# quitedob/yolo-sod

Measured on AMD Instinct MI355X. Metric: images/sec @640×640 bs=32, 1→8 MI355X; mAP@0.5:0.95 parity vs CPU ref, higher is better.
Workload: dtype f32

## Files before the change

include/yolosod_hip.h:

```cpp
#ifndef YOLOSOD_HIP_H
#define YOLOSOD_HIP_H
#include <stddef.h>
#include <stdint.h>

#ifdef __cplusplus
extern "C" {
#endif

int yolosod_abi_version(void);
const char* yolosod_last_error(void);
int yolosod_init(int device);

size_t yolosod_se_workspace(int B, int C, int H, int W);
int yolosod_se_forward(const float* x, float* y, int B, int C, int H, int W, const float* fc1_w, const float* fc1_b,
                       const float* fc2_w, const float* fc2_b, int hidden, void* workspace, size_t workspace_bytes,
                       void* stream);

size_t yolosod_cbam_workspace(int B, int C, int H, int W);
int yolosod_cbam_forward(const float* x, float* y, int B, int C, int H, int W, const float* fc0_w,
                         const float* fc2_w, int hidden, const float* sa_w, void* workspace, size_t workspace_bytes,
                         void* stream);

size_t yolosod_ca_workspace(int B, int C, int H, int W);
int yolosod_ca_forward(const float* x, float* y, int B, int C, int H, int W, const float* conv1_w,
// ... 29 lines not shown
                         size_t workspace_bytes, void* stream);
size_t yolosod_swin_prep_bytes(int C, int num_heads, int mlp_hidden);
size_t yolosod_swin_prepared_workspace(int B, int C, int H, int W, int num_heads, int window, int mlp_hidden);
int yolosod_swin_prepare(int C, int num_heads, int mlp_hidden, const float* ln1_w, const float* ln1_b,
                         const float* in_proj_w, const float* in_proj_b, const float* out_proj_w, const float* ln2_w,
                         const float* ln2_b, const float* mlp1_w, const float* mlp1_b, const float* mlp2_w,
                         const float* pw_w, const float* bn_w, const float* bn_b, const float* bn_mean,
                         const float* bn_var, float bn_eps, void* prep, size_t prep_bytes, void* stream);
int yolosod_swin_forward_prepared(const float* x, float* y, int B, int C, int H, int W, int num_heads, int window,
                                  const float* dw_w, float ln1_eps, const float* out_proj_b, float ln2_eps,
                                  int mlp_hidden, const float* mlp2_b, const void* prep, size_t prep_bytes,
                                  void* workspace, size_t workspace_bytes, void* stream);

int yolosod_plane_parts(long HW, long* seg);
int yolosod_bias_act_stats(const float* y, long y_bstride, float* out, long out_bstride, const float* bias,
                           const float* res, long res_bstride, int B, int C, long HW, int act, int parts, long seg,
                           float* psum, float* pmax, void* stream);
int yolosod_se_forward_pre(const float* x, float* y, int B, int C, int H, int W, const float* fc1_w,
                           const float* fc1_b, const float* fc2_w, const float* fc2_b, int hidden, const float* psum,
                           void* workspace, size_t workspace_bytes, void* stream);
int yolosod_cbam_forward_pre(const float* x, float* y, int B, int C, int H, int W, const float* fc0_w,
                             const float* fc2_w, int hidden, const float* sa_w, const float* psum, const float* pmax,
                             void* workspace, size_t workspace_bytes, void* stream);
int yolosod_bias_act_capool(const float* y, long y_bstride, float* out, long out_bstride, const float* bias,
                            const float* res, long res_bstride, int B, int C, int H, int W, int act, float* yin,
                            void* stream);
int yolosod_upsample2x(const void* x, void* out, long out_bstride, int B, int C, int h, int w, int elem_bytes,
                       void* stream);
size_t yolosod_stem_workspace(int B, int Cout, int H, int W);
int yolosod_stem_conv(const float* x, const float* w, const float* bias, float* out, int B, int Cout, int H, int W,
                      int parts, long seg, float* psum, void* workspace, size_t workspace_bytes, void* stream);
int yolosod_ca_forward_pre(const float* x, float* y, int B, int C, int H, int W, const float* conv1_w,
                           const float* conv1_b, int mip, const float* bn_w, const float* bn_b, const float* bn_mean,
                           const float* bn_var, float bn_eps, const float* convh_w, const float* convh_b,
                           const float* convw_w, const float* convw_b, const float* yin, void* workspace,
                           size_t workspace_bytes, void* stream);

size_t yolosod_mamba_glu_workspace(int B, int C, int H, int W, int ch, int reduction);
int yolosod_mamba_glu_forward(const float* x, float* y, int B, int C, int H, int W, int ch, int reduction,
                              const float* in_w, const float* in_bn_w, const float* in_bn_b, const float* in_bn_mean,
                              const float* in_bn_var, float in_bn_eps, const float* pw1_w, const float* dw_w,
                              const float* bn_w, const float* bn_b, const float* bn_mean, const float* bn_var,
                              float bn_eps, const float* pw2_w, const float* out_w, const float* out_bn_w,
                              const float* out_bn_b, const float* out_bn_mean, const float* out_bn_var,
                              float out_bn_eps, void* workspace, size_t workspace_bytes, void* stream);

int yolosod_detect_decode(int nl, const float* const* maps, const int* heights, const int* widths,
                          const float* strides, int B, int nc, int reg_max, float* y, void* stream);

int yolosod_detect_head(int nl, const float* const* box_feat, const float* const* cls_feat, int c2, int c3,
                        const float* const* box_w, const float* const* box_b, const float* const* cls_w,
                        const float* const* cls_b, const int* heights, const int* widths, const float* strides, int B,
                        int nc, int reg_max, float* y, void* stream);

size_t yolosod_nms_workspace(int B, int nc, int A, int multi_label);
size_t yolosod_nms_workspace_v2(int B, int nc, int A, int multi_label, int max_det);
int yolosod_nms(float* pred, int B, int nc, int A, float conf_thres, double iou_thres, const int* classes,
                int n_classes, int agnostic, int multi_label, int max_det, int max_nms, float max_wh, int in_place,
                float* out, int* counts, int* out_index, void* workspace, size_t workspace_bytes, void* stream);
int yolosod_nms_merged(float* pred, int B, int nc, int A, float conf_thres, double iou_thres, const int* classes,
                       int n_classes, int agnostic, int multi_label, int max_det, int max_nms, float max_wh,
                       int in_place, float* out, int* counts, int* out_index, int* n_merged, void* workspace,
                       size_t workspace_bytes, void* stream);

int yolosod_letterbox_ingest(const int64_t* desc, int B, void* out, long out_bstride, int out_h, int out_w,
                             int out_bf16, int pad_value, void* stream);
int yolosod_scale_boxes(float* det, const int* counts, int B, int D, const float* geom, void* stream);
int yolosod_tile_merge(const float* y, int n, int nc, int A, const int32_t* desc, int rows, float* merged, int F,
                       int S, float cut_margin, void* stream);
int yolosod_tta_views(const void* x, int B, int C, int H, int W, int bf16, const int64_t* desc, int V, int max_ph,
                      int max_pw, void* stream);
int yolosod_tta_merge(const float* y, int B, int nc, int A, int src_lo, int n, float* cat, int A_tot, int dst,
                      float scale, int flip, float img_w, float img_h, void* stream);
int yolosod_tile_merge_tta(const float* y, int n, int nc, int A, int src_lo, int n_k, const int32_t* desc, int rows,
                           float* merged, int F, int S, int A_tot, int dst, float scale, int flip, float img_w,
                           float img_h, float cut_margin, void* stream);
int yolosod_match_predictions(const float* det, const int* counts, int B, int D, const float* labels,
                              const int* label_off, const float* iouv, int T, uint8_t* tp, void* stream);

int yolosod_bias_act(const float* y, long y_bstride, float* out, long out_bstride, const float* bias,
                     const float* res, long res_bstride, int B, int C, long HW, int act, void* stream);

int yolosod_bias_act_dual(const float* y, long y_bstride, float* out, long out_bstride, const float* bias,
                          const float* res, long res_bstride, float* out2, long out2_bstride, int c2lo, int B, int C,
                          long HW, int act, void* stream);

size_t yolosod_conv3x3_prep_bytes(int cin);
int yolosod_conv3x3_prepare(const float* w, int cin, void* prep, size_t prep_bytes, void* stream);
int yolosod_conv3x3_silu(const float* x, float* y, int B, int cin, int H, int W, const float* bias, const void* prep,
                         size_t prep_bytes, void* stream);
size_t yolosod_conv3x3_prep_bytes_ex(int cin, int cout);
int yolosod_conv3x3_prepare_ex(const float* w, int cin, int cout, void* prep, size_t prep_bytes, void* stream);
int yolosod_conv3x3_silu_ex(const float* x, float* y, long y_bstride, const float* res, long res_bstride, int B,
                            int cin, int cout, int H, int W, const float* bias, const void* prep, size_t prep_bytes,
                            void* stream);
int yolosod_conv3x3_silu_xs(const float* x, long x_bstride, float* y, long y_bstride, const float* res, long res_bstride,
                            int B, int cin, int cout, int H, int W, const float* bias, const void* prep,
                            size_t prep_bytes, void* stream);
int yolosod_bottleneck3x3_silu_xs(const float* x, long x_bstride, float* y, long y_bstride, const float* res,
                                  long res_bstride, int B, int H, int W, const float* bias1, const void* prep1,
                                  size_t prep1_bytes, const float* bias2, const void* prep2, size_t prep2_bytes,
                                  void* stream);

int yolosod_conv3x3_head_xs(const float* x, long x_bstride, int B, int H, int W, const float* bias, const void* prep,
                            size_t prep_bytes, const void* head_prep, const float* head_bias, int mode, int nc,
                            float stride, float* y, int A, int a_off, void* stream);
size_t yolosod_detect_head_prep_bytes(int rows);
int yolosod_detect_head_prepare(const float* w, int rows, void* prep, size_t prep_bytes, void* stream);

int yolosod_conv1x1_thin(const float* x, long x_bs, const float* w, const float* bias, float* out, long out_bs,
                         const float* res, long res_bs, float* out2, long out2_bs, int c2lo, int B, int Cin, int Cout,
                         long HW, void* stream);

int yolosod_sppf_pool(float* z, long z_bstride, int B, int C, int H, int W, void* stream);

int yolosod_conv1x1_thin_cat(const float* x, long x_bs, const float* x2, long x2_bs, int k1, const float* w,
                             const float* bias, float* out, long out_bs, float* out2, long out2_bs, int c2lo, int B,
                             int Cin, int Cout, long HW, int up_w, void* stream);

int yolosod_conv1x1_thin_stats(const float* x, long x_bs, const float* w, const float* bias, float* out, long out_bs,
                               int B, int Cin, int Cout, long HW, int parts, float* psum, float* pmax, float* tile_ws,
                               void* stream);

int yolosod_conv1x1(const float* x, long x_bs, const float* w, const float* bias, float* out, long out_bs,
                    const float* res, long res_bs, int B, int Cin, int Cout, long HW, int act, void* stream);

int yolosod_gemm_f32(const float* A, long a_bs, int lda, const float* B, long b_bs, int ldb, int b_kcontig, float* C,
                     long c_bs, int ldc, int M, int N, int K, int batch, const float* bias, int bias_mode, int act,
                     const float* res, void* stream);
int yolosod_layernorm(const float* x, float* y, long rows, int C, const float* w, const float* b, float eps,
                      void* stream);
int yolosod_attention(const float* qkv, float* out, long n_seq, int L, int C, int heads, void* stream);

void yolosod_debug_set_swin_fused(int on);
int yolosod_debug_set_swin_x3(int on);
int yolosod_debug_set_a2_pool_px(int px);
int yolosod_debug_set_head_x2(int on);
int yolosod_debug_set_a2_x2(int on);
int yolosod_debug_set_a2_fused(int on);
int yolosod_debug_set_a2_pool_wide(int on);
int yolosod_se_gate(const float* x, int B, int C, int H, int W, const float* fc1_w, const float* fc1_b,
                    const float* fc2_w, const float* fc2_b, int hidden, const float* psum, float* gate, void* workspace,
                    size_t workspace_bytes, void* stream);
int yolosod_cbam_gates(const float* x, int B, int C, int H, int W, const float* fc0_w, const float* fc2_w, int hidden,
                       const float* sa_w, const float* psum, const float* pmax, float* ca, float* sa, void* workspace,
                       size_t workspace_bytes, void* stream);
size_t yolosod_conv3x3s2_prep_bytes(int cin, int cout);
int yolosod_conv3x3s2_prepare(const float* w, int cin, int cout, void* prep, size_t prep_bytes, void* stream);
int yolosod_conv3x3s2_silu(const float* x, float* y, int B, int cin, int cout, int H, int W, const float* bias,
                           const float* gc, const float* gp, const void* prep, size_t prep_bytes, void* stream);
int yolosod_conv3x3s2_silu_out(const float* x, float* y, long y_bstride, int B, int cin, int cout, int H, int W,
                               const float* bias, const float* gc, const float* gp, const void* prep,
                               size_t prep_bytes, void* stream);
size_t yolosod_conv1x1x2_prep_bytes(int cin, int cout);
int yolosod_conv1x1x2_prepare(const float* w, int cin, int cout, void* prep, size_t prep_bytes, void* stream);
int yolosod_conv1x1x2_silu(const float* x, long x_bstride, float* y, long y_bstride, float* y2, long y2_bstride,
                           int c2lo, int B, int cin, int cout, int HW, const float* bias, const void* prep,
                           size_t prep_bytes, void* stream);
int yolosod_conv1x1x2_silu_cat(const float* x, long x_bstride, const float* x2, long x2_bstride, int k1, float* y,
                               long y_bstride, float* y2, long y2_bstride, int c2lo, int B, int cin, int cout, int HW,
                               const float* bias, const void* prep, size_t prep_bytes, int up_w, void* stream);
int yolosod_conv1x1x2_silu_stats(const float* x, long x_bstride, float* y, long y_bstride, int B, int cin, int cout,
                                 int HW, const float* bias, const void* prep, size_t prep_bytes, int stats, int parts,
                                 float* psum, float* pmax, float* tile_ws, void* stream);
int yolosod_debug_set_conv1x1x2_form(int form);
int yolosod_debug_conv1x1x2_form(int B, int cout, int H, int W);
int yolosod_debug_set_conv3x3s2_form(int form);
int yolosod_debug_conv3x3s2_form(int B, int cout, int H, int W);
int yolosod_debug_set_conv3x3_form(int form);
int yolosod_debug_conv3x3_form(int B, int cout, int H, int W);
int yolosod_debug_conv3x3_form_ex(int B, int cin, int cout, int H, int W);
int yolosod_debug_bottleneck3x3_fused(int B, int H, int W);
int yolosod_debug_set_bottleneck3x3_fuse(int mode);
int yolosod_debug_conv3x3_head_fused(int B, int H, int W);
int yolosod_debug_set_conv3x3_head_fuse(int mode);
void yolosod_debug_set_gemm_x2(int on);
int yolosod_debug_set_swin_tokln(int on);
int yolosod_debug_split_f16(const float* v, uint32_t* h, uint32_t* l, long npair, void* stream);
int yolosod_split_range_flag(int reset, void* stream);

#include <stdint.h>

int yolosod_se_forward_bf16(const uint16_t* x, uint16_t* y, int B, int C, int H, int W, const float* fc1_w,
                            const float* fc1_b, const float* fc2_w, const float* fc2_b, int hidden, const float* psum,
                            void* workspace, size_t workspace_bytes, void* stream);
int yolosod_cbam_forward_bf16(const uint16_t* x, uint16_t* y, int B, int C, int H, int W, const float* fc0_w,
                              const float* fc2_w, int hidden, const float* sa_w, const float* psum, const float* pmax,
                              void* workspace, size_t workspace_bytes, void* stream);
int yolosod_ca_forward_bf16(const uint16_t* x, uint16_t* y, int B, int C, int H, int W, const float* conv1_w,
                            const float* conv1_b, int mip, const float* bn_w, const float* bn_b, const float* bn_mean,
                            const float* bn_var, float bn_eps, const float* convh_w, const float* convh_b,
                            const float* convw_w, const float* convw_b, const float* yin, void* workspace,
                            size_t workspace_bytes, void* stream);
size_t yolosod_swin_workspace_bf16(int B, int C, int H, int W, int num_heads, int window, int mlp_hidden);
int yolosod_swin_forward_bf16(const uint16_t* x, uint16_t* y, int B, int C, int H, int W, int num_heads, int window,
                              const float* dw_w, const float* ln1_w, const float* ln1_b, float ln1_eps,
                              const uint16_t* in_proj_w, const float* in_proj_b, const uint16_t* out_proj_w,
                              const float* out_proj_b, const float* ln2_w, const float* ln2_b, float ln2_eps,
                              const uint16_t* mlp1_w, const float* mlp1_b, int mlp_hidden, const uint16_t* mlp2_w,
                              const float* mlp2_b, const uint16_t* pw_w, const float* bn_w, const float* bn_b,
                              const float* bn_mean, const float* bn_var, float bn_eps, void* workspace,
                              size_t workspace_bytes, void* stream);
size_t yolosod_a2_workspace_bf16(int B, int C, int H, int W, int num_areas);
int yolosod_a2_forward_bf16(const uint16_t* x, uint16_t* y, int B, int C, int H, int W, int num_areas, int num_heads,
                            const uint16_t* proj_w, const float* proj_b, const float* ln_w, const float* ln_b,
                            float ln_eps, const uint16_t* in_proj_w, const float* in_proj_b, const uint16_t* oproj_w,
                            const float* oproj_b, void* workspace, size_t workspace_bytes, void* stream);
int yolosod_detect_head_levels(int nl, int l0, int l1, const void* const* box_feat, const void* const* cls_feat, int c2,
                               int c3, const float* const* box_w, const float* const* box_b, const float* const* cls_w,
                               const float* const* cls_b, const int* heights, const int* widths, const float* strides,
                               int B, int nc, int reg_max, float* y, int bf16, void* stream);
int yolosod_detect_head_bf16(int nl, const uint16_t* const* box_feat, const uint16_t* const* cls_feat, int c2, int c3,
                             const float* const* box_w, const float* const* box_b, const float* const* cls_w,
                             const float* const* cls_b, const int* heights, const int* widths, const float* strides,
                             int B, int nc, int reg_max, float* y, void* stream);
int yolosod_bias_act_bf16(const uint16_t* y, long y_bstride, uint16_t* out, long out_bstride, const float* bias,
                          const uint16_t* res, long res_bstride, uint16_t* out2, long out2_bstride, int c2lo, int B,
                          int C, long HW, int act, void* stream);
int yolosod_bias_act_stats_bf16(const uint16_t* y, long y_bstride, uint16_t* out, long out_bstride, const float* bias,
                                const uint16_t* res, long res_bstride, int B, int C, long HW, int act, int parts,
                                long seg, float* psum, float* pmax, void* stream);
int yolosod_bias_act_capool_bf16(const uint16_t* y, long y_bstride, uint16_t* out, long out_bstride,
                                 const float* bias, const uint16_t* res, long res_bstride, int B, int C, int H, int W,
                                 int act, float* yin, void* stream);
int yolosod_gemm_bf16(const uint16_t* A, long a_bs, int lda, const uint16_t* B, long b_bs, int ldb, int b_kcontig,
                      uint16_t* C, long c_bs, int ldc, int M, int N, int K, int batch, const float* bias,
                      int bias_mode, int act, const uint16_t* res, void* stream);
int yolosod_attention_bf16(const uint16_t* qkv, uint16_t* out, long n_seq, int L, int C, int heads, void* stream);

#ifdef __cplusplus
}
#endif
#endif
```

yolo-sod_amd/_hip.py:

```python
from __future__ import annotations

import ctypes
import os
from pathlib import Path

import torch

from .utils.metrics import IOU_THRESHOLDS

LIB_PATH = Path(__file__).resolve().parent / "lib" / "libyolosod_hip.so"

_c_float_p = ctypes.c_void_p
_vp = ctypes.c_void_p
_i = ctypes.c_int
_l = ctypes.c_long
_f = ctypes.c_float
_d = ctypes.c_double
_sz = ctypes.c_size_t

SIGNATURES = {
    "yolosod_abi_version": (_i, []),
    "yolosod_last_error": (ctypes.c_char_p, []),
    "yolosod_se_workspace": (_sz, [_i, _i, _i, _i]),
    "yolosod_se_forward": (_i, [_vp, _vp, _i, _i, _i, _i, _vp, _vp, _vp, _vp, _i, _vp, _sz, _vp]),
    "yolosod_cbam_workspace": (_sz, [_i, _i, _i, _i]),
    "yolosod_cbam_forward": (_i, [_vp, _vp, _i, _i, _i, _i, _vp, _vp, _i, _vp, _vp, _sz, _vp]),
    "yolosod_ca_workspace": (_sz, [_i, _i, _i, _i]),
    "yolosod_ca_forward": (_i, [_vp, _vp, _i, _i, _i, _i, _vp, _vp, _i, _vp, _vp, _vp, _vp, _f, _vp, _vp, _vp,
                                _vp, _vp, _sz, _vp]),
    "yolosod_a2_workspace": (_sz, [_i, _i, _i, _i, _i]),
    "yolosod_a2_forward": (_i, [_vp, _vp, _i, _i, _i, _i, _i, _i, _vp, _vp, _vp, _vp, _f, _vp, _vp, _vp, _vp, _vp,
                                _vp, _vp, _sz, _vp]),
    "yolosod_swin_workspace": (_sz, [_i, _i, _i, _i, _i, _i]),
    "yolosod_swin_workspace_v2": (_sz, [_i, _i, _i, _i, _i, _i, _i]),
    "yolosod_swin_forward": (_i, [_vp, _vp, _i, _i, _i, _i, _i, _i, _vp, _vp, _vp, _f, _vp, _vp, _vp, _vp, _vp, _vp,
                                  _f, _vp, _vp, _i, _vp, _vp, _vp, _vp, _vp, _vp, _vp, _f, _vp, _sz, _vp]),
    "yolosod_detect_decode": (_i, [_i, _vp, _vp, _vp, _vp, _i, _i, _i, _vp, _vp]),
    "yolosod_detect_head": (_i, [_i, _vp, _vp, _i, _i, _vp, _vp, _vp, _vp, _vp, _vp, _vp, _i, _i, _i, _vp, _vp]),
    "yolosod_nms_workspace": (_sz, [_i, _i, _i, _i]),
    "yolosod_nms_workspace_v2": (_sz, [_i, _i, _i, _i, _i]),
    "yolosod_nms": (_i, [_vp, _i, _i, _i, _f, _d, _vp, _i, _i, _i, _i, _i, _f, _i, _vp, _vp, _vp, _vp, _sz, _vp]),
    "yolosod_nms_merged": (_i, [_vp, _i, _i, _i, _f, _d, _vp, _i, _i, _i, _i, _i, _f, _i, _vp, _vp, _vp, _vp, _vp, _sz,
                                _vp]),
    "yolosod_gemm_f32": (_i, [_vp, _l, _i, _vp, _l, _i, _i, _vp, _l, _i, _i, _i, _i, _i, _vp, _i, _i, _vp, _vp]),
    "yolosod_layernorm": (_i, [_vp, _vp, _l, _i, _vp, _vp, _f, _vp]),
    "yolosod_attention": (_i, [_vp, _vp, _l, _i, _i, _i, _vp]),
    "yolosod_bias_act": (_i, [_vp, _l, _vp, _l, _vp, _vp, _l, _i, _i, _l, _i, _vp]),
    "yolosod_upsample2x": (_i, [_vp, _vp, _l, _i, _i, _i, _i, _i, _vp]),
    "yolosod_letterbox_ingest": (_i, [_vp, _i, _vp, _l, _i, _i, _i, _i, _vp]),
    "yolosod_scale_boxes": (_i, [_vp, _vp, _i, _i, _vp, _vp]),
    "yolosod_tile_merge": (_i, [_vp, _i, _i, _i, _vp, _i, _vp, _i, _i, _f, _vp]),
    "yolosod_tile_merge_tta": (_i, [_vp, _i, _i, _i, _i, _i, _vp, _i, _vp, _i, _i, _i, _i, _f, _i, _f, _f, _f, _vp]),
    "yolosod_match_predictions": (_i, [_vp, _vp, _i, _i, _vp, _vp, _vp, _i, _vp, _vp]),
    "yolosod_tta_views": (_i, [_vp, _i, _i, _i, _i, _i, _vp, _i, _i, _i, _vp]),
    "yolosod_tta_merge": (_i, [_vp, _i, _i, _i, _i, _i, _vp, _i, _i, _f, _i, _f, _f, _vp]),
    "yolosod_stem_workspace": (_sz, [_i, _i, _i, _i]),
    "yolosod_stem_conv": (_i, [_vp, _vp, _vp, _vp, _i, _i, _i, _i, _i, _l, _vp, _vp, _sz, _vp]),
    "yolosod_conv1x1_thin_stats": (_i, [_vp, _l, _vp, _vp, _vp, _l, _i, _i, _i, _l, _i, _vp, _vp, _vp, _vp]),
    "yolosod_conv1x1_thin": (_i, [_vp, _l, _vp, _vp, _vp, _l, _vp, _l, _vp, _l, _i, _i, _i, _i, _l, _vp]),
    "yolosod_bias_act_dual": (_i, [_vp, _l, _vp, _l, _vp, _vp, _l, _vp, _l, _i, _i, _i, _l, _i, _vp]),
    "yolosod_bias_act_capool": (_i, [_vp, ctypes.c_long, _vp, ctypes.c_long, _vp, _vp, ctypes.c_long, _i, _i, _i, _i,
                                     _i, _vp, _vp]),
    "yolosod_ca_forward_pre": (_i, [_vp, _vp, _i, _i, _i, _i, _vp, _vp, _i, _vp, _vp, _vp, _vp, _f, _vp, _vp, _vp, _vp,
                                    _vp, _vp, ctypes.c_size_t, _vp]),
    "yolosod_bias_act_stats": (_i, [_vp, _l, _vp, _l, _vp, _vp, _l, _i, _i, _l, _i, _i, _l, _vp, _vp, _vp]),
    "yolosod_plane_parts": (_i, [_l, ctypes.POINTER(ctypes.c_long)]),
    "yolosod_se_forward_pre": (_i, [_vp, _vp, _i, _i, _i, _i, _vp, _vp, _vp, _vp, _i, _vp, _vp, _sz, _vp]),
    "yolosod_cbam_forward_pre": (_i, [_vp, _vp, _i, _i, _i, _i, _vp, _vp, _i, _vp, _vp, _vp, _vp, _sz, _vp]),
    "yolosod_conv1x1": (_i, [_vp, _l, _vp, _vp, _vp, _l, _vp, _l, _i, _i, _i, _l, _i, _vp]),
    "yolosod_conv3x3_prep_bytes": (_sz, [_i]),
    "yolosod_conv3x3_prepare": (_i, [_vp, _i, _vp, _sz, _vp]),
    "yolosod_conv3x3_silu": (_i, [_vp, _vp, _i, _i, _i, _i, _vp, _vp, _sz, _vp]),
    "yolosod_conv1x1x2_prep_bytes": (_sz, [_i, _i]),
    "yolosod_conv1x1x2_prepare": (_i, [_vp, _i, _i, _vp, _sz, _vp]),
    "yolosod_conv1x1x2_silu": (_i, [_vp, _l, _vp, _l, _vp, _l, _i, _i, _i, _i, _i, _vp, _vp, _sz, _vp]),
    "yolosod_conv1x1x2_silu_cat": (_i, [_vp, _l, _vp, _l, _i, _vp, _l, _vp, _l, _i, _i, _i, _i, _i, _vp, _vp, _sz,
                                        _i, _vp]),
    "yolosod_conv1x1x2_silu_stats": (_i, [_vp, _l, _vp, _l, _i, _i, _i, _i, _vp, _vp, _sz, _i, _i, _vp, _vp, _vp, _vp]),
    "yolosod_sppf_pool": (_i, [_vp, _l, _i, _i, _i, _i, _vp]),
    "yolosod_conv1x1_thin_cat": (_i, [_vp, _l, _vp, _l, _i, _vp, _vp, _vp, _l, _vp, _l, _i, _i, _i, _i, _l, _i, _vp]),
    "yolosod_conv3x3_prep_bytes_ex": (_sz, [_i, _i]),
    "yolosod_conv3x3_prepare_ex": (_i, [_vp, _i, _i, _vp, _sz, _vp]),
    "yolosod_conv3x3_silu_ex": (_i, [_vp, _vp, _l, _vp, _l, _i, _i, _i, _i, _i, _vp, _vp, _sz, _vp]),
    "yolosod_conv3x3_silu_xs": (_i, [_vp, _l, _vp, _l, _vp, _l, _i, _i, _i, _i, _i, _vp, _vp, _sz, _vp]),
    "yolosod_debug_set_swin_fused": (None, [_i]),
    "yolosod_debug_set_swin_x3": (_i, [_i]),
    "yolosod_debug_set_head_x2": (_i, [_i]),
    "yolosod_debug_set_a2_x2": (_i, [_i]),
    "yolosod_debug_set_gemm_x2": (None, [_i]),
    "yolosod_debug_split_f16": (_i, [_vp, _vp, _vp, _l, _vp]),
    "yolosod_swin_prep_bytes": (_sz, [_i, _i, _i]),
    "yolosod_split_range_flag": (_i, [_i, _vp]),
    "yolosod_swin_prepare": (_i, [_i, _i, _i] + [_vp] * 15 + [_f, _vp, _sz, _vp]),
    "yolosod_swin_forward_prepared": (_i, [_vp, _vp, _i, _i, _i, _i, _i, _i, _vp, _f, _vp, _f, _i, _vp, _vp, _sz,
                                           _vp, _sz, _vp]),
    "yolosod_swin_prepared_workspace": (_sz, [_i, _i, _i, _i, _i, _i, _i]),
    "yolosod_a2_prep_bytes": (_sz, [_i, _i, _i, _i]),
    "yolosod_a2_prepare": (_i, [_i, _vp, _vp, _vp, _vp, _vp, _vp, _sz, _vp]),
    "yolosod_a2_forward_prepared": (_i, [_vp, _vp, _i, _i, _i, _i, _i, _i, _vp, _vp, _vp, _vp, _f, _vp, _vp, _vp,
                                         _vp, _vp, _sz, _vp, _sz, _vp]),
    "yolosod_init": (_i, [_i]),
    "yolosod_debug_set_a2_fused": (_i, [_i]),
    "yolosod_debug_set_a2_pool_wide": (_i, [_i]),
    "yolosod_debug_set_conv3x3_form": (_i, [_i]),
    "yolosod_debug_conv3x3_form": (_i, [_i, _i, _i, _i]),
    "yolosod_debug_conv3x3_form_ex": (_i, [_i, _i, _i, _i, _i]),
    "yolosod_bottleneck3x3_silu_xs": (_i, [_vp, _l, _vp, _l, _vp, _l, _i, _i, _i, _vp, _vp, _sz, _vp, _vp, _sz, _vp]),
    "yolosod_conv3x3_head_xs": (_i, [_vp, _l, _i, _i, _i, _vp, _vp, _sz, _vp, _vp, _i, _i, _f, _vp, _i, _i, _vp]),
    "yolosod_detect_head_prep_bytes": (_sz, [_i]),
    "yolosod_detect_head_prepare": (_i, [_vp, _i, _vp, _sz, _vp]),
    "yolosod_debug_conv3x3_head_fused": (_i, [_i, _i, _i]),
    "yolosod_debug_set_conv3x3_head_fuse": (_i, [_i]),
    "yolosod_debug_bottleneck3x3_fused": (_i, [_i, _i, _i]),
    "yolosod_debug_set_bottleneck3x3_fuse": (_i, [_i]),
    "yolosod_debug_set_conv1x1x2_form": (_i, [_i]),
    "yolosod_debug_conv1x1x2_form": (_i, [_i, _i, _i, _i]),
    "yolosod_debug_set_conv3x3s2_form": (_i, [_i]),
    "yolosod_debug_conv3x3s2_form": (_i, [_i, _i, _i, _i]),
    "yolosod_se_gate": (_i, [_vp, _i, _i, _i, _i, _vp, _vp, _vp, _vp, _i, _vp, _vp, _vp, _sz, _vp]),
    "yolosod_cbam_gates": (_i, [_vp, _i, _i, _i, _i, _vp, _vp, _i, _vp, _vp, _vp, _vp, _vp, _vp, _sz, _vp]),
    "yolosod_conv3x3s2_prep_bytes": (_sz, [_i, _i]),
    "yolosod_conv3x3s2_prepare": (_i, [_vp, _i, _i, _vp, _sz, _vp]),
    "yolosod_conv3x3s2_silu": (_i, [_vp, _vp, _i, _i, _i, _i, _i, _vp, _vp, _vp, _vp, _sz, _vp]),
    "yolosod_conv3x3s2_silu_out": (_i, [_vp, _vp, _l, _i, _i, _i, _i, _i, _vp, _vp, _vp, _vp, _sz, _vp]),
    "yolosod_debug_set_swin_tokln": (_i, [_i]),
    "yolosod_debug_set_a2_pool_px": (_i, [_i]),
    "yolosod_mamba_glu_workspace": (_sz, [_i, _i, _i, _i, _i, _i]),
    "yolosod_mamba_glu_forward": (_i, [_vp, _vp, _i, _i, _i, _i, _i, _i, _vp, _vp, _vp, _vp, _vp, _f, _vp, _vp,
                                       _vp, _vp, _vp, _vp, _f, _vp, _vp, _vp, _vp, _vp, _vp, _f, _vp, _sz, _vp]),
    "yolosod_se_forward_bf16": (_i, [_vp, _vp, _i, _i, _i, _i, _vp, _vp, _vp, _vp, _i, _vp, _vp, _sz, _vp]),
    "yolosod_cbam_forward_bf16": (_i, [_vp, _vp, _i, _i, _i, _i, _vp, _vp, _i, _vp, _vp, _vp, _vp, _sz, _vp]),
    "yolosod_ca_forward_bf16": (_i, [_vp, _vp, _i, _i, _i, _i, _vp, _vp, _i, _vp, _vp, _vp, _vp, _f, _vp, _vp, _vp,
                                     _vp, _vp, _vp, _sz, _vp]),
    "yolosod_bias_act_bf16": (_i, [_vp, _l, _vp, _l, _vp, _vp, _l, _vp, _l, _i, _i, _i, _l, _i, _vp]),
    "yolosod_bias_act_stats_bf16": (_i, [_vp, _l, _vp, _l, _vp, _vp, _l, _i, _i, _l, _i, _i, _l, _vp, _vp, _vp]),
    "yolosod_bias_act_capool_bf16": (_i, [_vp, _l, _vp, _l, _vp, _vp, _l, _i, _i, _i, _i, _i, _vp, _vp]),
    "yolosod_swin_workspace_bf16": (_sz, [_i, _i, _i, _i, _i, _i, _i]),
    "yolosod_swin_forward_bf16": (_i, [_vp, _vp, _i, _i, _i, _i, _i, _i, _vp, _vp, _vp, _f, _vp, _vp, _vp, _vp, _vp,
                                       _vp, _f, _vp, _vp, _i, _vp, _vp, _vp, _vp, _vp, _vp, _vp, _f, _vp, _sz, _vp]),
    "yolosod_a2_workspace_bf16": (_sz, [_i, _i, _i, _i, _i]),
    "yolosod_a2_forward_bf16": (_i, [_vp, _vp, _i, _i, _i, _i, _i, _i, _vp, _vp, _vp, _vp, _f, _vp, _vp, _vp, _vp,
                                     _vp, _sz, _vp]),
    "yolosod_detect_head_bf16": (_i, [_i, _vp, _vp, _i, _i, _vp, _vp, _vp, _vp, _vp, _vp, _vp, _i, _i, _i, _vp,
                                      _vp]),
    "yolosod_detect_head_levels": (_i, [_i, _i, _i, _vp, _vp, _i, _i, _vp, _vp, _vp, _vp, _vp, _vp, _vp, _i, _i,
                                        _i, _vp, _i, _vp]),
    "yolosod_gemm_bf16": (_i, [_vp, _l, _i, _vp, _l, _i, _i, _vp, _l, _i, _i, _i, _i, _i, _vp, _i, _i, _vp, _vp]),
    "yolosod_attention_bf16": (_i, [_vp, _vp, _l, _i, _i, _i, _vp]),
}

_LIB = None


def load_library() -> ctypes.CDLL:
    global _LIB
    if _LIB is None:
        if not LIB_PATH.exists():
            raise RuntimeError(
                f"yolosod_amd: HIP library {LIB_PATH} is missing - run __graft_entry__.build() "
                "(or python yolo-sod_amd/build.py). There is no CPU fallback.")
        path = os.environ.get("YOLOSOD_LIB_AB") or str(LIB_PATH)
        lib = ctypes.CDLL(path)
        for name, (res, args) in SIGNATURES.items():
            if path != str(LIB_PATH) and name.startswith("yolosod_debug_") and not hasattr(lib, name):
                continue
            fn = getattr(lib, name)
            fn.restype = res
            fn.argtypes = args
        _LIB = lib
    return _LIB


OPS_LIB_PATH = LIB_PATH.parent / "yolosod_torch_ops.so"
_OPS = None


def ops():
    global _OPS
    if _OPS is None:
        load_library()
        if not OPS_LIB_PATH.exists():
            raise RuntimeError(f"yolosod_amd: torch-op library {OPS_LIB_PATH} is missing - run "
                               "__graft_entry__.build() (or python yolo-sod_amd/build.py). There is no CPU fallback.")
        if not hasattr(torch.ops.yolosod, "se_fwd"):
            torch.ops.load_library(str(OPS_LIB_PATH))
        _OPS = torch.ops.yolosod
    return _OPS


class _OpTimer:

    def __init__(self, select=None):
        self.records = []
        self.select = select

    def durations_ms(self):
        torch.cuda.synchronize()
        out = []
        for key, e0, e1 in self.records:
            out.append((key, e0.elapsed_time(e1)))
        return out


_TIMER: _OpTimer | None = None


class op_timer:

    def __init__(self, select=None):
        self.select = select

    def __enter__(self):
        global _TIMER
        self.t = _OpTimer(self.select)
        _TIMER = self.t
        return self.t

    def __exit__(self, *exc):
        global _TIMER
        _TIMER = None
        return False


_INIT_DEVS = set()


def _init_device(dev) -> None:
    idx = torch.device(dev).index
    idx = torch.cuda.current_device() if idx is None else idx
    if idx not in _INIT_DEVS:
        _check(load_library().yolosod_init(int(idx)), "init")
        _INIT_DEVS.add(idx)


def _launch(key, dev, fn, *args):
    _init_device(dev)
    with torch.cuda.device(dev):
        t = _TIMER
        if t is None or (t.select is not None and not t.select(key)):
            return fn(*args)
        e0 = torch.cuda.Event(enable_timing=True)
        e1 = torch.cuda.Event(enable_timing=True)
        e0.record()
        rc = fn(*args)
        e1.record()
        t.records.append((key, e0, e1))
        return rc


def _check(rc: int, what: str) -> None:
    if rc != 0:
        msg = load_library().yolosod_last_error().decode(errors="replace")
        raise RuntimeError(f"yolosod_amd.{what} failed (rc={rc}): {msg}")


def _dev(t: torch.Tensor, name: str, dtype=torch.float32) -> int:
    if not isinstance(t, torch.Tensor):
        raise TypeError(f"{name}: expected a tensor")
    if t.device.type != "cuda":
        raise RuntimeError(f"{name}: HIP kernel requires a GPU tensor (got device {t.device}); no CPU fallback")
    if t.dtype != dtype:
        raise RuntimeError(f"{name}: expected {dtype}, got {t.dtype}")
    if not t.is_contiguous():
        raise RuntimeError(f"{name}: expected a contiguous tensor")
    return t.data_ptr()


def _p(t: torch.Tensor, name: str, numel: int | None = None, dtype=torch.float32) -> int:
    if numel is not None and t.numel() != numel:
        raise RuntimeError(f"{name}: expected {numel} elements, got {t.numel()}")
    return _dev(t, name, dtype)


_BF16 = torch.bfloat16


def _act_dtype(x: torch.Tensor) -> bool:
# ... 637 lines not shown
def bottleneck3x3_fused(B, H, W) -> bool:
    return bool(load_library().yolosod_debug_bottleneck3x3_fused(int(B), int(H), int(W)))


def bottleneck3x3_silu(x, bias1, prep1, bias2, prep2, out=None, res=None, op="bottleneck3x3"):
    lib = load_library()
    B, C, H, W = x.shape
    if C != 32:
        raise RuntimeError(f"bottleneck3x3: {C} channels (32 only)")
    if out is None:
        y = torch.empty((B, 32, H, W), dtype=torch.float32, device=x.device)
    else:
        _img_view(out, (B, 32, H, W), "bottleneck3x3: out")
        y = out
    if res is not None:
        _img_view(res, (B, 32, H, W), "bottleneck3x3: res")
    b1 = bias1.detach().float().contiguous()
    b2 = bias2.detach().float().contiguous()

    def run():
        blk1, blk2 = prep1(), prep2()
        _img_view(x, (B, 32, H, W), "bottleneck3x3: x")
        return lib.yolosod_bottleneck3x3_silu_xs(x.data_ptr(), x.stride(0), y.data_ptr(), y.stride(0),
                                                 None if res is None else res.data_ptr(),
                                                 0 if res is None else res.stride(0), B, H, W, _dev(b1, "bias1"),
                                                 blk1.data_ptr(), blk1.numel(), _dev(b2, "bias2"), blk2.data_ptr(),
                                                 blk2.numel(), _stream(x.device))

    _check(_launch((op, tuple(x.shape), 32 if res is None else (32, "res")), x.device, run), "bottleneck3x3")
    return y


class CatView:

    def __init__(self, parts, up0=False):
        a, b = parts
        sp = (2 * a.shape[2], 2 * a.shape[3]) if up0 else tuple(a.shape[2:])
        if a.shape[0] != b.shape[0] or sp != tuple(b.shape[2:]) or a.dtype != b.dtype or a.device != b.device:
            raise ValueError("CatView: parts must agree in batch, spatial size, dtype and device")
        self.parts = (a, b)
        self.up0 = bool(up0)
        self.shape = torch.Size((a.shape[0], a.shape[1] + b.shape[1], b.shape[2], b.shape[3]))
        self.device, self.dtype = a.device, a.dtype

    def dim(self):
        return 4

    def materialize(self):
        a, b = self.parts
        if self.up0:
            a = torch.nn.functional.interpolate(a, scale_factor=2, mode="nearest")
        return torch.cat((a, b), 1)


def sppf_pool(z, c):
    B, C4, H, W = z.shape
    if (C4 != 4 * c or z.dtype != torch.float32 or z.device.type != "cuda"
            or z.stride()[1:] != (H * W, W, 1)):
        raise RuntimeError("sppf_pool: z must be a [B, 4c, H, W] fp32 GPU tensor with contiguous images")
    lib = load_library()
    _check(_launch(("sppf_pool", (B, c, H, W), None), z.device, lib.yolosod_sppf_pool, z.data_ptr(), z.stride(0), B,
                   int(c), H, W, _stream(z.device)), "sppf_pool")
    return z


def _imgs_contig(t) -> bool:
    B, C, H, W = t.shape
    return t.stride()[1:] == (H * W, W, 1) and t.stride(0) % 4 == 0 and t.data_ptr() % 16 == 0


def conv1x1x2_ok(x, conv) -> bool:
    if isinstance(x, CatView):
        if not (all(_imgs_contig(t) for t in x.parts) and x.parts[0].shape[1] % 128 == 0):
            return False
    elif not (x.dim() == 4 and _imgs_contig(x)):
        return False
    return (x.device.type == "cuda" and x.dtype == torch.float32
            and conv.kernel_size == (1, 1) and conv.stride == (1, 1) and conv.padding == (0, 0) and conv.groups == 1
            and x.shape[1] == conv.in_channels and (x.shape[2] * x.shape[3]) % 4 == 0
            and int(load_library().yolosod_conv1x1x2_prep_bytes(int(conv.in_channels), int(conv.out_channels))) > 0)


def conv1x1x2_prepare(w):
    lib = load_library()
    return _split_prepare("conv1x1x2", lib.yolosod_conv1x1x2_prep_bytes, lib.yolosod_conv1x1x2_prepare,
                          w.reshape(int(w.shape[0]), int(w.shape[1])))


def conv1x1x2_silu(x, bias, prep, cout, out=None, out2=None, c2lo=0, op="conv1x1x2", stats=None):
    lib = load_library()
    B, Cin, H, W = x.shape
    if stats is not None and (stats not in ("sum", "summax", "capool") or out2 is not None or isinstance(x, CatView)):
        raise RuntimeError(f"conv1x1x2: stats={stats!r} takes one input tensor, no out2")
    if out is None:
        y = torch.empty((B, cout, H, W), dtype=torch.float32, device=x.device)
    else:
        _img_view(out, (B, cout, H, W), "conv1x1x2: out")
        y = out
    if out2 is not None:
        _img_view(out2, (B, cout - c2lo, H, W), "conv1x1x2: out2")
    b = bias.detach().float().contiguous()
    if stats in ("sum", "summax"):
        HW = H * W
        parts, _ = plane_parts(HW)
        psum = torch.empty(B * cout * parts, dtype=torch.float32, device=x.device)
        pmax = torch.empty_like(psum) if stats == "summax" else None
        tws = torch.empty(2 * B * cout * ((HW + 63) // 64), dtype=torch.float32, device=x.device)

        def run_stats():
            blk = prep()
            return lib.yolosod_conv1x1x2_silu_stats(x.data_ptr(), x.stride(0), y.data_ptr(), y.stride(0), B, Cin, cout,
                                                    HW, _dev(b, "bias"), blk.data_ptr(), blk.numel(),
                                                    2 if stats == "summax" else 1, parts, psum.data_ptr(),
                                                    None if pmax is None else pmax.data_ptr(), tws.data_ptr(),
                                                    _stream(x.device))

        _check(_launch(("conv1x1x2_stats", tuple(x.shape), (cout, stats)), x.device, run_stats), "conv1x1x2_stats")
        y._ys_plane_stats = PlaneStats(psum, pmax, parts, y.shape)
        return y

    x0, x1 = x.parts if isinstance(x, CatView) else (x, None)

    def run():
        blk = prep()
        return lib.yolosod_conv1x1x2_silu_cat(x0.data_ptr(), x0.stride(0), None if x1 is None else x1.data_ptr(),
                                              0 if x1 is None else x1.stride(0), int(x0.shape[1]), y.data_ptr(),
                                              y.stride(0), None if out2 is None else out2.data_ptr(),
                                              0 if out2 is None else out2.stride(0), int(c2lo), B, Cin, cout, H * W,
                                              _dev(b, "bias"), blk.data_ptr(), blk.numel(),
                                              W if x1 is not None and x.up0 else 0, _stream(x.device))

    extra = (cout, out2 is not None) + (("cat",) if x1 is not None else ())
    if stats == "capool":
        op, extra = "conv1x1x2_stats", (cout, stats)
    _check(_launch((op, tuple(x.shape), extra), x.device, run), "conv1x1x2")
    return y


def conv3x3s2_ok(x, conv) -> bool:
    return (x.device.type == "cuda" and x.dtype == torch.float32 and x.is_contiguous() and x.dim() == 4
            and conv.kernel_size == (3, 3) and conv.stride == (2, 2) and conv.padding == (1, 1)
            and conv.dilation == (1, 1) and conv.groups == 1
            and (conv.out_channels == 64 or (conv.out_channels % 128 == 0 and conv.out_channels <= 512))
            and conv.in_channels % 32 == 0 and x.shape[1] == conv.in_channels and ((x.shape[3] + 1) // 2) % 4 == 0
            and x.numel() * 4 < 2 ** 32
            and int(load_library().yolosod_conv3x3s2_prep_bytes(int(conv.in_channels), int(conv.out_channels))) > 0)


def conv3x3s2_prepare(w):
    lib = load_library()
    return _split_prepare("conv3x3s2", lib.yolosod_conv3x3s2_prep_bytes, lib.yolosod_conv3x3s2_prepare, w)


def conv3x3s2_silu(x, bias, prep, cout, gate_c=None, gate_p=None, key=None, out=None):
    lib = load_library()
    B, Cin, H, W = x.shape
    Ho, Wo = (H + 1) // 2, (W + 1) // 2
    if out is None:
        y = torch.empty((B, cout, Ho, Wo), dtype=torch.float32, device=x.device)
    else:
        y = out
        if (tuple(y.shape) != (B, cout, Ho, Wo) or y.dtype != torch.float32 or y.device != x.device
                or y.stride()[1:] != (Ho * Wo, Wo, 1) or y.data_ptr() % 16 or y.stride(0) % 4):
            raise RuntimeError(f"conv3x3s2: out {tuple(y.shape)} / {y.stride()} is not a [{B}, {cout}, {Ho}, {Wo}] "
                               "fp32 view with contiguous 16-byte aligned images")
    b = bias.detach().float().contiguous()
    gc = None if gate_c is None else gate_c.float().contiguous()
    gp = None if gate_p is None else gate_p.float().contiguous()
    if gc is not None and (tuple(gc.shape) != (B, Cin) or gc.data_ptr() % 16):
        raise RuntimeError(f"conv3x3s2: channel gate {tuple(gc.shape)} (16-byte aligned [{B}, {Cin}] expected)")
    if gp is not None and gp.numel() != B * H * W:
        raise RuntimeError(f"conv3x3s2: spatial gate of {gp.numel()} values ({B * H * W} expected)")

    def run():
        blk = prep()
        return lib.yolosod_conv3x3s2_silu_out(_dev(x, "x"), y.data_ptr(), y.stride(0), B, Cin, cout, H, W,
                                              _dev(b, "bias"), None if gc is None else _dev(gc, "gate_c"),
                                              None if gp is None else _dev(gp, "gate_p"), blk.data_ptr(), blk.numel(),
                                              _stream(x.device))

    if key is None:
        key = ("conv3x3s2", tuple(x.shape), (cout, gc is not None, gp is not None))
    _check(_launch(key, x.device, run), "conv3x3s2")
    return y


INGEST_MAX_DIM = 16384


def letterbox_ingest(images, out_shape, geoms, dtype=torch.float32, out=None, pad_value=114):
    lib = load_library()
    B = len(images)
    out_h, out_w = int(out_shape[0]), int(out_shape[1])
    if B < 1 or len(geoms) != B:
        raise RuntimeError(f"letterbox_ingest: {B} frames with {len(geoms)} geometries")
    if dtype not in (torch.float32, _BF16):
        raise RuntimeError(f"letterbox_ingest: output dtype must be float32 or bfloat16, got {dtype}")
    if out_w % 4 or not (0 < out_h <= INGEST_MAX_DIM and 0 < out_w <= INGEST_MAX_DIM):
        raise RuntimeError(f"letterbox_ingest: canvas {out_h}x{out_w} unsupported (width % 4 == 0, <= {INGEST_MAX_DIM})")
    rows = []
    dev = None
    for i, (t, g) in enumerate(zip(images, geoms)):
        if not isinstance(t, torch.Tensor):
            raise TypeError(f"letterbox_ingest: frame {i}: expected a tensor")
        if t.dtype != torch.uint8:
            raise RuntimeError(f"letterbox_ingest: frame {i}: expected uint8, got {t.dtype}")
        if t.dim() != 3 or t.shape[2] != 3:
            raise RuntimeError(f"letterbox_ingest: frame {i}: expected [h, w, 3] (BGR), got {tuple(t.shape)}")
        h, w = int(t.shape[0]), int(t.shape[1])
        if not (0 < h <= INGEST_MAX_DIM and 0 < w <= INGEST_MAX_DIM):
            raise RuntimeError(f"letterbox_ingest: frame {i}: {h}x{w} outside 1..{INGEST_MAX_DIM}")
        if t.stride(2) != 1:
            raise RuntimeError(f"letterbox_ingest: frame {i}: channel stride {t.stride(2)} (1 expected)")
        if w > 1 and t.stride(1) != 3:
            raise RuntimeError(f"letterbox_ingest: frame {i}: pixel stride {t.stride(1)} (3 expected)")
        pitch = int(t.stride(0)) if h > 1 else 3 * w
        if pitch < 3 * w:
            raise RuntimeError(f"letterbox_ingest: frame {i}: row pitch {pitch} < 3 * {w}")
        if t.device.type != "cuda":
            raise RuntimeError(f"letterbox_ingest: frame {i}: HIP kernel requires a GPU tensor (got device "
                               f"{t.device}); no CPU fallback")
        if dev is None:
            dev = t.device
        elif t.device != dev:
            raise RuntimeError(f"letterbox_ingest: frame {i} on {t.device}, frame 0 on {dev}")
        nh, nw, top, left = (int(v) for v in g[:4])
        if nh < 1 or nw < 1 or top < 0 or left < 0 or top + nh > out_h or left + nw > out_w:
            raise RuntimeError(f"letterbox_ingest: frame {i}: geometry {tuple(g)} leaves the {out_h}x{out_w} canvas")
        rows.append([t.data_ptr(), h, w, pitch, nh, nw, top, left])
    if out is None:
        out = torch.empty((B, 3, out_h, out_w), dtype=dtype, device=dev)
    elif (out.dtype != dtype or out.device != dev or tuple(out.shape) != (B, 3, out_h, out_w)
          or out.stride()[1:] != (out_h * out_w, out_w, 1) or out.stride(0) % 4 or out.stride(0) < 3 * out_h * out_w
          or out.data_ptr() % 16):
        raise RuntimeError(f"letterbox_ingest: out must be a {dtype} [{B}, 3, {out_h}, {out_w}] tensor on {dev} with "
                           "contiguous 16-byte aligned images and a batch stride that is a multiple of 4")
    desc = torch.tensor(rows, dtype=torch.int64).pin_memory().to(dev, non_blocking=True)
    key = ("ingest", (B, 3, out_h, out_w), 2 if dtype == _BF16 else None)
    _check(_launch(key, dev, lib.yolosod_letterbox_ingest, desc.data_ptr(), B, out.data_ptr(), out.stride(0) if B > 1
                   else 3 * out_h * out_w, out_h, out_w, int(dtype == _BF16), int(pad_value), _stream(dev)),
           "letterbox_ingest")
    return out


def scale_boxes_padded(out, counts, geom):
    lib = load_library()
    if out.dim() != 3 or out.shape[2] != 6:
        raise RuntimeError(f"scale_boxes_padded: out must be [B, D, 6], got {tuple(out.shape)}")
    B, D = int(out.shape[0]), int(out.shape[1])
    if tuple(counts.shape) != (B,) or tuple(geom.shape) != (B, 5):
        raise RuntimeError(f"scale_boxes_padded: counts {tuple(counts.shape)} / geom {tuple(geom.shape)} do not match "
                           f"{B} images")
    _check(_launch(("scale_boxes", (B, D, 6), None), out.device, lib.yolosod_scale_boxes, _dev(out, "out"),
                   _dev(counts, "counts", torch.int32), B, D, _dev(geom, "geom"), _stream(out.device)),
           "scale_boxes")
    return out


TILE_MERGE_MAX_NC = 64


def tile_merge(y, rows, merged, A, cut_margin=None):
    lib = load_library()
    for t, name in ((y, "y"), (merged, "merged")):
        if not isinstance(t, torch.Tensor):
            raise TypeError(f"tile_merge: {name}: expected a tensor")
        if t.device.type != "cuda":
            raise RuntimeError(f"tile_merge: {name}: HIP kernel requires a GPU tensor (got device {t.device}); "
                               "no CPU fallback")
        if t.dtype != torch.float32:
            raise RuntimeError(f"tile_merge: {name}: expected float32, got {t.dtype}")
        if t.dim() != 3:
            raise RuntimeError(f"tile_merge: {name}: expected 3 dimensions, got shape {tuple(t.shape)}")
        if not t.is_contiguous():
            raise RuntimeError(f"tile_merge: {name}: expected a contiguous tensor")
    if merged.device != y.device:
        raise RuntimeError(f"tile_merge: y on {y.device}, merged on {merged.device}")
    n, no, A = int(y.shape[0]), int(y.shape[1]), int(A)
    nc = no - 4
    if A < 1 or int(y.shape[2]) != A:
        raise RuntimeError(f"tile_merge: y has {int(y.shape[2])} anchors, A = {A}")
    if n < 1 or not 1 <= nc <= TILE_MERGE_MAX_NC:
        raise RuntimeError(f"tile_merge: y {tuple(y.shape)} unsupported (n >= 1, 1..{TILE_MERGE_MAX_NC} classes)")
    F, SA = int(merged.shape[0]), int(merged.shape[2])
    if F < 1 or int(merged.shape[1]) != no or SA < A or SA % A:
        raise RuntimeError(f"tile_merge: merged {tuple(merged.shape)} is not [F, {no}, S * {A}]")
    S = SA // A
    if S * A * nc >= 1 << 32:
        raise RuntimeError(f"tile_merge: S * A * nc = {S} * {A} * {nc} >= 2^32")
    desc = _tile_merge_desc("tile_merge", rows, n, F, S)
    cm = -1.0 if cut_margin is None else float(cut_margin)
    if cm != cm:
        raise RuntimeError("tile_merge: cut_margin is NaN")
    dev = y.device
    d = torch.from_numpy(desc).pin_memory().to(dev, non_blocking=True)
    _check(_launch(("tile_merge", (n, no, A), (F, S)), dev, lib.yolosod_tile_merge, y.data_ptr(), n, nc, A,
                   d.data_ptr(), len(desc), merged.data_ptr(), F, S, cm, _stream(dev)), "tile_merge")
    return merged


def _tile_merge_desc(who, rows, n, F, S):
    import numpy as np
    rows = list(rows)
    if not 1 <= len(rows) <= 65535:
        raise RuntimeError(f"{who}: {len(rows)} descriptor rows (1..65535)")
    desc = np.zeros((len(rows), 16), dtype=np.int32)
    fl = desc.view(np.float32)
    named = set()
    for i, r in enumerate(rows):
        if len(r) != 11 or len(r[10]) != 4:
            raise RuntimeError(f"{who}: row {i}: expected (src, frame, slot, gain, pad_x, pad_y, off_x, off_y, "
                               "tile_w, tile_h, (left, right, top, bottom))")
        src, frame, slot = int(r[0]), int(r[1]), int(r[2])
        if not -1 <= src < n:
            raise RuntimeError(f"{who}: row {i}: src {src} outside [-1, {n})")
        if not 0 <= frame < F:
            raise RuntimeError(f"{who}: row {i}: frame {frame} outside [0, {F})")
        if not 0 <= slot < S:
            raise RuntimeError(f"{who}: row {i}: slot {slot} outside [0, {S})")
        if (frame, slot) in named:
            raise RuntimeError(f"{who}: row {i}: slot {slot} of frame {frame} is named twice")
        named.add((frame, slot))
        gain = float(r[3])
        if src >= 0 and not (gain > 0.0 and gain < float("inf")):
            raise RuntimeError(f"{who}: row {i}: gain {gain}")
        desc[i, :3] = (src, frame, slot)
        desc[i, 3] = sum(1 << k for k in range(4) if r[10][k])
        fl[i, 4:11] = [float(v) for v in r[3:10]]
    return desc


def tile_merge_tta(y, rows, merged, A_tot, branch, canvas_hw, cut_margin=None):
    lib = load_library()
    for t, name in ((y, "y"), (merged, "merged")):
        if not isinstance(t, torch.Tensor):
# ... 254 lines not shown
```

yolo-sod_amd/csrc/conv3x3s2.hip:

```cpp
#include "split_conv.h"

namespace ys {
namespace c3s2 {

constexpr float WSC = SPLIT_WSC;
constexpr int TH = 4, TW = 32;
constexpr int HC = 2 * TW + 1;
constexpr int PS = 32 + 8;

struct Args {
  const float* x;
  const h16_t* wp;
  const float* bias;
  const float* gc;
  const float* gp;
  float* y;
  long ybs;
  int B, cin, H, W, Ho, Wo, tiles_x, tiles_y, ntiles;
  int ncb_all;
  unsigned* range_flag;
  const unsigned* prep_flag;
};

constexpr int ES = TW + 4;
template <int GATE, int THk, int NTk>
__global__ __launch_bounds__(NTk, 512 / NTk) void conv3x3s2_rw_kernel(Args p) {
  constexpr int HRk = 2 * THk + 1, NPXk = HRk * HC, PLk = NPXk * PS, NQUADk = NPXk * 8;
  constexpr int NITk = (NQUADk + NTk - 1) / NTk, NGPk = (NPXk + NTk - 1) / NTk;
  static_assert(NITk <= 32, "okb bits");
  __shared__ __attribute__((aligned(16))) h16_t Pl[2 * PLk];
  __shared__ __attribute__((aligned(16))) float Ep[THk * 64 * ES];
  __shared__ __attribute__((aligned(16))) float gcs[32];
  __shared__ float gps[(GATE & 2) ? NPXk : 1];
  const int tid = threadIdx.x, lane = tid & 63, wid = __builtin_amdgcn_readfirstlane(tid >> 6);
  const int l15 = lane & 15, g = lane >> 4;
  const int H = p.H, W = p.W, HWi = H * W;
  const int rp = wid >> 2, cb = wid & 3;
  float rng = 0.f;

  const int nj = gridDim.x >> 3, j = blockIdx.x >> 3, xcd = blockIdx.x & 7;
  const int per = (p.ntiles + 7) >> 3;
  const int t_beg = xcd * per + j, t_end = min((xcd + 1) * per, p.ntiles);
  if (t_beg >= t_end) return;
  const int n_it = (t_end - t_beg + nj - 1) / nj;

  auto rsrc = [&](const void* base, unsigned bytes) {
    const unsigned long long a = (unsigned long long)base;
    return __builtin_amdgcn_make_buffer_rsrc(
        (void*)(((unsigned long long)__builtin_amdgcn_readfirstlane((unsigned)(a >> 32)) << 32) |
                (unsigned)__builtin_amdgcn_readfirstlane((unsigned)a)),
        (short)0, __builtin_amdgcn_readfirstlane(bytes), 0x00020000);
  };
  const __amdgpu_buffer_rsrc_t rx = rsrc(p.x, 0xffffffffu);
  const __amdgpu_buffer_rsrc_t rw = rsrc(p.wp, (unsigned)(9L * 4 * 2 * 1024));

  f16x8_t wr[9][2];
#pragma unroll
  for (int t = 0; t < 9; ++t)
#pragma unroll
    for (int pl = 0; pl < 2; ++pl)
      wr[t][pl] = __builtin_bit_cast(
          f16x8_t, __builtin_amdgcn_raw_buffer_load_b128(rw, (unsigned)(lane * 16), ((t * 4 + cb) * 2 + pl) * 1024, 0));
  int pk[NITk], el0[NITk];
#pragma unroll
  for (int i = 0; i < NITk; ++i) {
    const int e = min(tid + NTk * i, NQUADk - 1);
    const int quad = e / NPXk, px = e - quad * NPXk;
    const int hy = px / HC, hx = px - hy * HC;
    pk[i] = (quad << 16) | (hy << 8) | hx;
    el0[i] = 4 * quad * HWi + hy * W + hx;
  }
  struct Tile {
    int b, ty, tx;
  };
  auto tile_of = [&](int it) __attribute__((always_inline)) {
    const int t = t_beg + it * nj;
    Tile tl;
    tl.tx = t % p.tiles_x;
    tl.ty = (t / p.tiles_x) % p.tiles_y;
    tl.b = t / (p.tiles_x * p.tiles_y);
    return tl;
  };
  f32x4 sv[NITk];
  float gcv = 0.f, gpv[NGPk];
  unsigned okb_ld = 0;
  auto load_tile = [&](const Tile& tl) __attribute__((always_inline)) {
    const int iy0 = 2 * THk * tl.ty - 1, ix0 = 2 * TW * tl.tx - 1;
    const __amdgpu_buffer_rsrc_t ri = rsrc(p.x + (long)tl.b * 32 * HWi, (unsigned)(32 * HWi * 4));
    const int toff = iy0 * W + ix0;
    const bool interior = iy0 >= 0 && ix0 >= 0 && iy0 + HRk <= H && ix0 + HC <= W;
    unsigned okb = 0xffffffffu;
    if (!interior) {
      okb = 0;
#pragma unroll
      for (int i = 0; i < NITk; ++i) {
        const int hy = (pk[i] >> 8) & 255, hx = pk[i] & 255;
        okb |= ((unsigned)(iy0 + hy) < (unsigned)H && (unsigned)(ix0 + hx) < (unsigned)W) ? (1u << i) : 0u;
      }
    }
#pragma unroll
    for (int i = 0; i < NITk; ++i) {
      const unsigned vo = (unsigned)((el0[i] + toff) * 4);
#pragma unroll
      for (int c = 0; c < 4; ++c)
        sv[i][c] = __builtin_bit_cast(float, __builtin_amdgcn_raw_buffer_load_b32(ri, vo + c * HWi * 4, 0, 0));
    }
    okb_ld = okb;
    if constexpr ((GATE & 1) != 0) gcv = p.gc[tl.b * 32 + (tid & 31)];
    if constexpr ((GATE & 2) != 0) {
#pragma unroll
      for (int k = 0; k < NGPk; ++k) {
        const int px = min(tid + NTk * k, NPXk - 1);
        const int hy = px / HC, hx = px - hy * HC;
        gpv[k] = p.gp[(long)tl.b * HWi + min(max(iy0 + hy, 0), H - 1) * W + min(max(ix0 + hx, 0), W - 1)];
      }
    }
  };
  int bpx[4];
#pragma unroll
  for (int k = 0; k < 4; ++k) bpx[k] = 2 * (2 * rp + (k >> 1)) * HC + 2 * ((k & 1) * 16 + l15);
  const int nw = __builtin_amdgcn_readfirstlane(p.Wo);
  const float bo = p.bias[16 * cb + l15];
  auto store_tile = [&](const Tile& tl) __attribute__((always_inline)) {
#pragma unroll
    for (int m = 0; m < THk * 512 / NTk; ++m) {
      const int idx = tid + NTk * m;
      const int r = idx >> 9, ch = (idx >> 3) & 63, px4 = idx & 7;
      const int ox = tl.tx * TW + 4 * px4, oy = tl.ty * THk + r;
      const f32x4 v = *reinterpret_cast<const f32x4*>(Ep + (r * 64 + ch) * ES + 4 * px4);
      if (oy < p.Ho && ox < nw)
        __builtin_nontemporal_store(v, reinterpret_cast<f32x4*>(p.y + (long)tl.b * p.ybs + ((long)ch * p.Ho + oy) * nw + ox));
    }
  };

  Tile cur = tile_of(0), prev = cur;
  load_tile(cur);
  for (int it = 0; it < n_it; ++it) {
    const unsigned okb = okb_ld;
    __syncthreads();
    if constexpr (GATE != 0) {
      if constexpr ((GATE & 1) != 0)
        if (tid < 32) gcs[tid] = gcv;
      if constexpr ((GATE & 2) != 0) {
#pragma unroll
        for (int k = 0; k < NGPk; ++k)
          if (tid + NTk * k < NPXk) gps[tid + NTk * k] = gpv[k];
      }
      __syncthreads();
    }
#pragma unroll
    for (int i = 0; i < NITk; ++i) {
      const int e = tid + NTk * i;
      if (e < NQUADk) {
        const int quad = pk[i] >> 16, px = e - quad * NPXk;
        f32x4 v = sv[i];
        if constexpr ((GATE & 1) != 0) v = v * *reinterpret_cast<const f32x4*>(gcs + 4 * quad);
        if constexpr ((GATE & 2) != 0) v = v * gps[px];
        if (!((okb >> i) & 1u)) v = f32x4{0.f, 0.f, 0.f, 0.f};
        uint2 hh, ll;
        split4x(v, hh, ll);
        rng = range_acc(rng, v);
        h16_t* d = Pl + px * PS + 4 * quad;
        *reinterpret_cast<uint2*>(d) = hh;
        *reinterpret_cast<uint2*>(d + PLk) = ll;
      }
    }
    if (it > 0) store_tile(prev);
    __syncthreads();
    prev = cur;
    if (it + 1 < n_it) cur = tile_of(it + 1);
    load_tile(cur);
    __builtin_amdgcn_sched_barrier(0);
    f32x4 acc[4];
#pragma unroll
    for (int k = 0; k < 4; ++k) acc[k] = f32x4{0.f, 0.f, 0.f, 0.f};
#pragma unroll
    for (int t = 0; t < 9; ++t) {
      const int toff = (t / 3) * HC + (t % 3);
#pragma unroll
      for (int k = 0; k < 4; ++k) {
        const h16_t* src = Pl + (bpx[k] + toff) * PS + 8 * g;
        const f16x8_t xh = *reinterpret_cast<const f16x8_t*>(src);
        const f16x8_t xl = *reinterpret_cast<const f16x8_t*>(src + PLk);
        f32x4 c = __builtin_amdgcn_mfma_f32_16x16x32_f16(xh, wr[t][1], acc[k], 0, 0, 0);
        c = __builtin_amdgcn_mfma_f32_16x16x32_f16(xl, wr[t][0], c, 0, 0, 0);
        acc[k] = __builtin_amdgcn_mfma_f32_16x16x32_f16(xh, wr[t][0], c, 0, 0, 0);
      }
    }
#pragma unroll
    for (int k = 0; k < 4; ++k) {
      f32x4 v;
#pragma unroll
      for (int e = 0; e < 4; ++e) v[e] = silu_fast_(acc[k][e] * (1.0f / WSC) + bo);
      *reinterpret_cast<f32x4*>(Ep + ((2 * rp + (k >> 1)) * 64 + 16 * cb + l15) * ES + 16 * (k & 1) + 4 * g) = v;
    }
  }
  __syncthreads();
  store_tile(prev);
  range_report(p.range_flag, rng);
  if (p.prep_flag && p.range_flag && blockIdx.x == 0 && threadIdx.x == 0 && *p.prep_flag) *p.range_flag = 1u;
}

template <int G>
struct Geo;
template <>
struct Geo<0> {
  static constexpr int BW = 16, TBX = 2, TBY = 2, RS = 65;
};
template <>
struct Geo<1> {
  static constexpr int BW = 8, TBX = 5, TBY = 1, RS = 88;
};
template <>
struct Geo<2> {
  static constexpr int BW = 4, TBX = 5, TBY = 1, RS = 44;
};
template <int G>
struct GeoD : Geo<G> {
  using B = Geo<G>;
  static constexpr int BH = 16 / B::BW, NBLK = B::TBX * B::TBY;
  static constexpr int TW = B::TBX * B::BW, TH = B::TBY * BH, HC = 2 * TW + 1, HR = 2 * TH + 1, NPX = HR * HC;
  static constexpr int PL = HR * B::RS * PS;
  static constexpr int NQUAD = NPX * 8, NIT = (NQUAD + 255) / 256;
  static_assert(B::RS >= HC && NIT <= 32 && HC < 256 && HR < 256, "conv3x3s2 geometry");
};

#ifndef YS_S2_READ_AHEAD
#define YS_S2_READ_AHEAD 1
#endif

template <int NCB, int GATE, int G>
__global__ __launch_bounds__(256, (NCB == 8 || G != 0) ? 2 : 3) void conv3x3s2_t2_kernel(Args p) {
  using Ge = GeoD<G>;
  constexpr int BW = Ge::BW, BH = Ge::BH, TBX = Ge::TBX, NBLK = Ge::NBLK, RS = Ge::RS;
  constexpr int THk = Ge::TH, TW = Ge::TW, HC = Ge::HC;
  constexpr int NTk = 256, HRk = Ge::HR, NPXk = Ge::NPX, PLk = Ge::PL, NQUADk = Ge::NQUAD;
  constexpr int NITk = Ge::NIT, NGPk = (NPXk + NTk - 1) / NTk, CBW = NCB / 4;
  static_assert(NCB == 4 || NCB == 8, "Cout 64 or 128");
  constexpr bool RA = YS_S2_READ_AHEAD != 0 && !(NCB == 4 && G == 0);
  __shared__ __attribute__((aligned(16))) h16_t Pl[2 * PLk];
  __shared__ __attribute__((aligned(16))) float gcs[32];
  __shared__ float gps[(GATE & 2) ? NPXk : 1];
  __shared__ float bsh[512];
  const int tid = threadIdx.x, lane = tid & 63, wid = __builtin_amdgcn_readfirstlane(tid >> 6);
  const int l15 = lane & 15, g = lane >> 4;
  const int H = p.H, W = p.W, HWi = H * W, nq = p.cin >> 5;
  float rng = 0.f;
  for (int o = tid; o < 16 * p.ncb_all; o += 256) bsh[o] = p.bias[o];

  const int nj = gridDim.x >> 3, j = blockIdx.x >> 3, xcd = blockIdx.x & 7;
  const int ngrp = p.ncb_all / NCB;
  const int nitems = p.ntiles * ngrp;
  const int per = (nitems + 7) >> 3;
  const int t_beg = xcd * per + j, t_end = min((xcd + 1) * per, nitems);
  if (t_beg >= t_end) return;
  const int n_it = ((t_end - t_beg + nj - 1) / nj) * nq;

  auto rsrc = [&](const void* base, unsigned bytes) {
    const unsigned long long a = (unsigned long long)base;
    return __builtin_amdgcn_make_buffer_rsrc(
        (void*)(((unsigned long long)__builtin_amdgcn_readfirstlane((unsigned)(a >> 32)) << 32) |
                (unsigned)__builtin_amdgcn_readfirstlane((unsigned)a)),
        (short)0, __builtin_amdgcn_readfirstlane(bytes), 0x00020000);
  };
  const __amdgpu_buffer_rsrc_t rw = rsrc(p.wp, (unsigned)(9L * nq * p.ncb_all * 2 * 1024));
  int pk[NITk], el0[NITk];
#pragma unroll
  for (int i = 0; i < NITk; ++i) {
    const int e = min(tid + NTk * i, NQUADk - 1);
    const int quad = e / NPXk, px = e - quad * NPXk;
    const int hy = px / HC, hx = px - hy * HC;
    pk[i] = (quad << 16) | (hy << 8) | hx;
    el0[i] = 4 * quad * HWi + hy * W + hx;
  }
  struct It {
    int b, ty, tx, q, grp;
  };
  auto it_of = [&](int it) __attribute__((always_inline)) {
    const int tg = t_beg + (it / nq) * nj;
    const int t = tg / ngrp;
    It r;
    r.grp = tg - t * ngrp;
    r.q = it - (it / nq) * nq;
    r.tx = t % p.tiles_x;
    r.ty = (t / p.tiles_x) % p.tiles_y;
    r.b = t / (p.tiles_x * p.tiles_y);
    return r;
  };
  f32x4 sv[NITk];
  float gcv = 0.f, gpv[NGPk];
  unsigned okb_ld = 0;
  auto load_part = [&](const It& r, int k0, int k1) __attribute__((always_inline)) {
    const int iy0 = 2 * THk * r.ty - 1, ix0 = 2 * TW * r.tx - 1;
    const __amdgpu_buffer_rsrc_t ri =
        rsrc(p.x + ((long)r.b * p.cin + 32 * r.q) * HWi, (unsigned)((p.cin - 32 * r.q) * HWi * 4));
    const int toff = iy0 * W + ix0;
    if (k0 == 0) {
      const bool interior = iy0 >= 0 && ix0 >= 0 && iy0 + HRk <= H && ix0 + HC <= W;
      unsigned okb = 0xffffffffu;
      if (!interior) {
        okb = 0;
#pragma unroll
        for (int i = 0; i < NITk; ++i) {
          const int hy = (pk[i] >> 8) & 255, hx = pk[i] & 255;
          okb |= ((unsigned)(iy0 + hy) < (unsigned)H && (unsigned)(ix0 + hx) < (unsigned)W) ? (1u << i) : 0u;
        }
      }
      okb_ld = okb;
    }
#pragma unroll
    for (int i = 0; i < NITk; ++i) {
      if (4 * i + 3 < k0 || 4 * i >= k1) continue;
      const unsigned vo = (unsigned)((el0[i] + toff) * 4);
#pragma unroll
      for (int c = 0; c < 4; ++c)
        if (4 * i + c >= k0 && 4 * i + c < k1)
          sv[i][c] = __builtin_bit_cast(float, __builtin_amdgcn_raw_buffer_load_b32(ri, vo + c * HWi * 4, 0, 0));
    }
  };
  auto load_gates = [&](const It& r) __attribute__((always_inline)) {
    if constexpr ((GATE & 1) != 0) gcv = p.gc[r.b * p.cin + 32 * r.q + (tid & 31)];
    if constexpr ((GATE & 2) != 0) {
      const int iy0 = 2 * THk * r.ty - 1, ix0 = 2 * TW * r.tx - 1;
#pragma unroll
      for (int k = 0; k < NGPk; ++k) {
        const int px = min(tid + NTk * k, NPXk - 1);
        const int hy = px / HC, hx = px - hy * HC;
        gpv[k] = p.gp[(long)r.b * HWi + min(max(iy0 + hy, 0), H - 1) * W + min(max(ix0 + hx, 0), W - 1)];
      }
    }
  };
  auto wfrag = [&](int t, int q, int cb, int pl) __attribute__((always_inline)) {
    const int st = __builtin_amdgcn_readfirstlane((((t * nq + q) * p.ncb_all + cb) * 2 + pl) * 1024);
    return __builtin_bit_cast(f16x8_t, __builtin_amdgcn_raw_buffer_load_b128(rw, (unsigned)(lane * 16), st, 0));
  };
  int bpx[NBLK];
#pragma unroll
  for (int k = 0; k < NBLK; ++k) bpx[k] = 2 * ((k / TBX) * BH + l15 / BW) * RS + 2 * ((k % TBX) * BW + l15 % BW);
  f32x4 acc[NBLK][CBW];
#pragma unroll
  for (int k = 0; k < NBLK; ++k)
#pragma unroll
    for (int u = 0; u < CBW; ++u) acc[k][u] = f32x4{0.f, 0.f, 0.f, 0.f};
  const int nw = __builtin_amdgcn_readfirstlane(p.Wo);
  constexpr int NLD = 4 * NITk;
  constexpr int PER_TAP = (NLD + 7) / 8;

// ... 13 lines not shown
          if (tid + NTk * k < NPXk) gps[tid + NTk * k] = gpv[k];
      }
      __syncthreads();
    }
#pragma unroll
    for (int i = 0; i < NITk; ++i) {
      const int e = tid + NTk * i;
      if (e < NQUADk) {
        const int quad = pk[i] >> 16, px = e - quad * NPXk;
        f32x4 v = sv[i];
        if constexpr ((GATE & 1) != 0) v = v * *reinterpret_cast<const f32x4*>(gcs + 4 * quad);
        if constexpr ((GATE & 2) != 0) v = v * gps[px];
        if (!((okb >> i) & 1u)) v = f32x4{0.f, 0.f, 0.f, 0.f};
        uint2 hh, ll;
        split4x(v, hh, ll);
        rng = range_acc(rng, v);
        const int pxl = RS == HC ? px : ((pk[i] >> 8) & 255) * RS + (pk[i] & 255);
        h16_t* d = Pl + pxl * PS + 4 * quad;
        *reinterpret_cast<uint2*>(d) = hh;
        *reinterpret_cast<uint2*>(d + PLk) = ll;
      }
    }
    __syncthreads();
    if (it + 1 < n_it) cur = it_of(it + 1);
    const int cb0 = r.grp * NCB + CBW * wid;
    f16x8_t wa[CBW][2], wn[CBW][2];
#pragma unroll
    for (int u = 0; u < CBW; ++u) {
      wa[u][0] = wfrag(0, r.q, cb0 + u, 0);
      wa[u][1] = wfrag(0, r.q, cb0 + u, 1);
    }
    auto rd = [&](int t, int k, f16x8_t& h, f16x8_t& l) __attribute__((always_inline)) {
      const h16_t* src = Pl + (bpx[k] + (t / 3) * RS + (t % 3)) * PS + 8 * g;
      h = *reinterpret_cast<const f16x8_t*>(src);
      l = *reinterpret_cast<const f16x8_t*>(src + PLk);
    };
    f16x8_t nh, nl;
    if constexpr (RA) rd(0, 0, nh, nl);
    __builtin_amdgcn_sched_barrier(0);
#pragma unroll
    for (int t = 0; t < 9; ++t) {
      const int tn = t + 1 < 9 ? t + 1 : t;
#pragma unroll
      for (int u = 0; u < CBW; ++u) {
        wn[u][0] = wfrag(tn, r.q, cb0 + u, 0);
        wn[u][1] = wfrag(tn, r.q, cb0 + u, 1);
      }
      if (t < 8) load_part(cur, PER_TAP * t, min(PER_TAP * t + PER_TAP, NLD));
      else load_gates(cur);
      __builtin_amdgcn_sched_barrier(0);
#pragma unroll
      for (int k = 0; k < NBLK; ++k) {
        f16x8_t xh, xl;
        if constexpr (RA) {
          xh = nh, xl = nl;
          if (k < NBLK - 1) rd(t, k + 1, nh, nl);
          else if (t < 8) rd(t + 1, 0, nh, nl);
        } else {
          rd(t, k, xh, xl);
        }
#pragma unroll
        for (int u = 0; u < CBW; ++u) {
          f32x4 c = __builtin_amdgcn_mfma_f32_16x16x32_f16(xh, wa[u][1], acc[k][u], 0, 0, 0);
          c = __builtin_amdgcn_mfma_f32_16x16x32_f16(xl, wa[u][0], c, 0, 0, 0);
          acc[k][u] = __builtin_amdgcn_mfma_f32_16x16x32_f16(xh, wa[u][0], c, 0, 0, 0);
        }
      }
      if constexpr (RA) {
#pragma unroll
        for (int k = 0; k < NBLK; ++k) {
          if (k < NBLK - 1 || t < 8) __builtin_amdgcn_sched_group_barrier(0x100, 2, 0);
          __builtin_amdgcn_sched_group_barrier(0x008, 3 * CBW, 0);
        }
      }
#pragma unroll
      for (int u = 0; u < CBW; ++u) {
        wa[u][0] = wn[u][0];
        wa[u][1] = wn[u][1];
      }
    }
    if (r.q == nq - 1) {
      float bo[CBW];
#pragma unroll
      for (int u = 0; u < CBW; ++u) bo[u] = bsh[16 * (cb0 + u) + l15];
      f32x4 v[NBLK][CBW];
#pragma unroll
      for (int k = 0; k < NBLK; ++k)
#pragma unroll
        for (int u = 0; u < CBW; ++u)
#pragma unroll
          for (int e = 0; e < 4; ++e) v[k][u][e] = silu_fast_(acc[k][u][e] * (1.0f / WSC) + bo[u]);
#pragma unroll
      for (int k = 0; k < NBLK; ++k) {
        const int oy = r.ty * THk + (k / TBX) * BH + (4 * g) / BW, ox = r.tx * TW + (k % TBX) * BW + (4 * g) % BW;
#pragma unroll
        for (int u = 0; u < CBW; ++u) {
          const int o = 16 * (cb0 + u) + l15;
          if (oy < p.Ho && ox < nw)
            __builtin_nontemporal_store(
                v[k][u], reinterpret_cast<f32x4*>(p.y + (long)r.b * p.ybs + ((long)o * p.Ho + oy) * nw + ox));
          acc[k][u] = f32x4{0.f, 0.f, 0.f, 0.f};
        }
      }
    }
  }
  range_report(p.range_flag, rng);
  if (p.prep_flag && p.range_flag && blockIdx.x == 0 && threadIdx.x == 0 && *p.prep_flag) *p.range_flag = 1u;
}

}
}

using namespace ys;

YS_EXPORT size_t yolosod_conv3x3s2_prep_bytes(int cin, int cout) {
  if (cin <= 0 || cin % 32 || cin > 2048 || !(cout == 64 || (cout % 128 == 0 && cout <= 512))) return 0;
  return split_prep_bytes((size_t)2 * cout * cin * 9);
}

static int g_s2_form = 0;
YS_EXPORT int yolosod_debug_set_conv3x3s2_form(int form) {
  const int old = g_s2_form;
  if (form >= 0 && form < 12) g_s2_form = form;
  return old;
}

static const int S2_GEO_TW[3] = {c3s2::GeoD<0>::TW, c3s2::GeoD<1>::TW, c3s2::GeoD<2>::TW};
static const int S2_GEO_TH[3] = {c3s2::GeoD<0>::TH, c3s2::GeoD<1>::TH, c3s2::GeoD<2>::TH};

static int s2_pick_geo(int Ho, int Wo) {
  static const int nblk[3] = {c3s2::GeoD<0>::NBLK, c3s2::GeoD<1>::NBLK, c3s2::GeoD<2>::NBLK};
  return pick_geo(Ho, Wo, S2_GEO_TW, S2_GEO_TH, nblk);
}

static int s2_form(int B, int cout, int Ho, int Wo) {
  const int fgeo = g_s2_form & 3, fgrp = (g_s2_form >> 2) & 3;
  const int geo = fgeo ? fgeo - 1 : s2_pick_geo(Ho, Wo);
  const bool g64 = cout == 64 || fgrp == 2;
  return geo + 1 + 4 * (g64 ? 2 : 1);
}

YS_EXPORT int yolosod_debug_conv3x3s2_form(int B, int cout, int H, int W) {
  if (B <= 0 || H <= 0 || W <= 0 || ((W + 1) / 2) % 4 || !(cout == 64 || (cout % 128 == 0 && cout <= 512))) return 0;
  return s2_form(B, cout, (H + 1) / 2, (W + 1) / 2);
}

YS_EXPORT int yolosod_conv3x3s2_prepare(const float* w, int cin, int cout, void* prep, size_t prep_bytes,
                                        void* stream) {
  YS_CHECK_ARG(yolosod_conv3x3s2_prep_bytes(cin, cout) > 0, "conv3x3s2_prepare: (cin=%d, cout=%d) unsupported", cin,
               cout);
  return split_prepare<9>("conv3x3s2_prepare", w, cin, cin, cout, prep, prep_bytes, stream);
}

YS_EXPORT int yolosod_conv3x3s2_silu_out(const float* x, float* y, long y_bstride, int B, int cin, int cout, int H,
                                         int W, const float* bias, const float* gc, const float* gp, const void* prep,
                                         size_t prep_bytes, void* stream) {
  YS_CHECK_ARG(x && y && bias && prep, "conv3x3s2: null pointer");
  YS_CHECK_ARG(B >= 0 && H > 0 && W > 0 && yolosod_conv3x3s2_prep_bytes(cin, cout) > 0, "conv3x3s2: bad shape");
  const int Ho = (H + 1) / 2, Wo = (W + 1) / 2;
  YS_CHECK_ARG(Wo % 4 == 0, "conv3x3s2: output width %d not a multiple of 4", Wo);
  YS_CHECK_ARG(y_bstride >= (long)cout * Ho * Wo, "conv3x3s2: output batch stride %ld < %ld", y_bstride,
               (long)cout * Ho * Wo);
  YS_CHECK_ARG(((uintptr_t)y & 15) == 0 && y_bstride % 4 == 0, "conv3x3s2: output not 16-byte aligned");
  YS_CHECK_ARG((long)B * cin * H * W * 4 < (1L << 32) && (long)cin * H * W < (1L << 31),
               "conv3x3s2: input too large for 32-bit buffer offsets");
  YS_CHECK_ARG(!gc || ((uintptr_t)gc & 15) == 0, "conv3x3s2: channel gate must be 16-byte aligned");
  if (B == 0) return 0;
  SplitPrep sp;
  YS_CHECK_ARG(split_prep_carve(prep, prep_bytes, (size_t)2 * cout * cin * 9, &sp),
               "conv3x3s2: prepared block too small");
  const int tx = (Wo + c3s2::TW - 1) / c3s2::TW, ty = (Ho + c3s2::TH - 1) / c3s2::TH;
  const long ntiles = (long)B * tx * ty;
  YS_CHECK_ARG(ntiles < (1L << 30), "conv3x3s2: too many tiles");
  c3s2::Args a{x, sp.wp, bias, gc, gp, y, y_bstride, B, cin, H, W, Ho, Wo, tx, ty, (int)ntiles, cout / 16,
               range_flag_dev(), sp.flag};
  const int gate = (gc ? 1 : 0) | (gp ? 2 : 0);
  hipStream_t st = (hipStream_t)stream;
  using KP = void (*)(c3s2::Args);
  if (cout == 64 && cin == 32) {
    a.tiles_y = (Ho + 1) / 2;
    const long nt2 = (long)B * a.tiles_y * tx;
    a.ntiles = (int)nt2;
    static const KP kp[4] = {c3s2::conv3x3s2_rw_kernel<0, 2, 256>, c3s2::conv3x3s2_rw_kernel<1, 2, 256>,
                             c3s2::conv3x3s2_rw_kernel<2, 2, 256>, c3s2::conv3x3s2_rw_kernel<3, 2, 256>};
    hipLaunchKernelGGL(kp[gate], dim3((unsigned)persistent_grid(2L * cu_count(), nt2)), dim3(256), 0, st, a);
  } else {
    const int form = s2_form(B, cout, Ho, Wo);
    const int geo = (form & 3) - 1;
    const bool g64 = (form >> 2) == 2;
    a.tiles_x = (Wo + S2_GEO_TW[geo] - 1) / S2_GEO_TW[geo];
    a.tiles_y = (Ho + S2_GEO_TH[geo] - 1) / S2_GEO_TH[geo];
    const long nt2 = (long)B * a.tiles_y * a.tiles_x;
    const long nitems = nt2 * (g64 ? cout / 64 : cout / 128);
    YS_CHECK_ARG(nitems < (1L << 30), "conv3x3s2: too many tiles");
    a.ntiles = (int)nt2;
    const long grid = persistent_grid((g64 && geo == 0 ? 3L : 2L) * cu_count(), nitems);
#define S2T2_GATES(NCB_, G_)                                                                        \
  {                                                                                                 \
    c3s2::conv3x3s2_t2_kernel<NCB_, 0, G_>, c3s2::conv3x3s2_t2_kernel<NCB_, 1, G_>,                 \
        c3s2::conv3x3s2_t2_kernel<NCB_, 2, G_>, c3s2::conv3x3s2_t2_kernel<NCB_, 3, G_>              \
  }
    static const KP kp[3][2][4] = {{S2T2_GATES(8, 0), S2T2_GATES(4, 0)},
                                   {S2T2_GATES(8, 1), S2T2_GATES(4, 1)},
                                   {S2T2_GATES(8, 2), S2T2_GATES(4, 2)}};
#undef S2T2_GATES
    hipLaunchKernelGGL(kp[geo][g64 ? 1 : 0][gate], dim3((unsigned)grid), dim3(256), 0, st, a);
  }
  YS_CHECK_LAUNCH("conv3x3s2");
  return 0;
}

YS_EXPORT int yolosod_conv3x3s2_silu(const float* x, float* y, int B, int cin, int cout, int H, int W,
                                     const float* bias, const float* gc, const float* gp, const void* prep,
                                     size_t prep_bytes, void* stream) {
  return yolosod_conv3x3s2_silu_out(x, y, (long)cout * ((H + 1) / 2) * ((W + 1) / 2), B, cin, cout, H, W, bias, gc, gp,
                                    prep, prep_bytes, stream);
}
```

yolo-sod_amd/csrc/conv_epilogue.hip:

```cpp
#include "common.h"
#include <math.h>

namespace ys {


template <int ACT, bool RES, bool DUAL = false, class T = float>
__global__ __launch_bounds__(256) void bias_act_kernel(const T* __restrict__ y, T* __restrict__ out,
                                                       const float* __restrict__ bias, const T* __restrict__ res,
                                                       int C, long HW4, long y_bs4, long o_bs4, long r_bs4,
                                                       long total4, int rev, T* __restrict__ out2 = nullptr,
                                                       int c2lo = 0, long o2_bs4 = 0) {
  for (long i0 = (long)blockIdx.x * 256 + threadIdx.x; i0 < total4; i0 += (long)gridDim.x * 256) {
    const long i = rev ? total4 - 1 - i0 : i0;
    const long b = i / ((long)C * HW4);
    const long rem = i - b * (long)C * HW4;
    const int c = (int)(rem / HW4);
    const float bc = bias[c];
    f32x4 v = ld4(y + 4 * (b * y_bs4 + rem));
    v += bc;
    if (ACT == 1) {
      v.x = silu_st<T>(v.x); v.y = silu_st<T>(v.y); v.z = silu_st<T>(v.z); v.w = silu_st<T>(v.w);
    }
    if (RES) v += ld4(res + 4 * (b * r_bs4 + rem));
    st4(out + 4 * (b * o_bs4 + rem), v);
    if (DUAL && c >= c2lo) st4(out2 + 4 * (b * o2_bs4 + rem - (long)c2lo * HW4), v);
  }
}

template <int ACT, bool RES, bool DUAL>
__global__ __launch_bounds__(256) void bias_act8_bf16_kernel(const bf16_t* __restrict__ y, bf16_t* __restrict__ out,
                                                             const float* __restrict__ bias,
                                                             const bf16_t* __restrict__ res, int C, long HW8,
                                                             long y_bs8, long o_bs8, long r_bs8, long total8, int rev,
                                                             bf16_t* __restrict__ out2, int c2lo, long o2_bs8) {
  for (long i0 = (long)blockIdx.x * 256 + threadIdx.x; i0 < total8; i0 += (long)gridDim.x * 256) {
    const long i = rev ? total8 - 1 - i0 : i0;
    const long b = i / ((long)C * HW8);
    const long rem = i - b * (long)C * HW8;
    const int c = (int)(rem / HW8);
    const float bc = bias[c];
    float f[8];
    unpack8(*reinterpret_cast<const uint4*>(y + 8 * (b * y_bs8 + rem)), f);
    float r[8];
    if (RES) unpack8(*reinterpret_cast<const uint4*>(res + 8 * (b * r_bs8 + rem)), r);
#pragma unroll
    for (int j = 0; j < 8; ++j) {
      float v = f[j] + bc;
      if (ACT == 1) v = silu_st<bf16_t>(v);
      if (RES) v += r[j];
      f[j] = v;
    }
    const uint4 o = pack8(f);
    *reinterpret_cast<uint4*>(out + 8 * (b * o_bs8 + rem)) = o;
    if (DUAL && c >= c2lo) *reinterpret_cast<uint4*>(out2 + 8 * (b * o2_bs8 + rem - (long)c2lo * HW8)) = o;
  }
}

template <int ACT, bool RES, bool MAX, class T = float, bool V8 = false>
__global__ __launch_bounds__(256) void bias_act_stats_kernel(const T* __restrict__ y, T* __restrict__ out,
                                                             const float* __restrict__ bias,
                                                             const T* __restrict__ res, int C, long HW,
                                                             long y_bs, long o_bs, long r_bs, int parts, long seg,
                                                             float* __restrict__ psum, float* __restrict__ pmax,
                                                             int rev) {
  const long bx = rev ? (long)gridDim.x - 1 - blockIdx.x : (long)blockIdx.x;
  const long plane = bx / parts;
  const int k = (int)(bx % parts);
  const long b = plane / C;
  const int c = (int)(plane - b * C);
  const long s0 = k * seg;
  const long s1 = (s0 + seg < HW) ? s0 + seg : HW;
  const float bc = bias[c];
  const T* y4 = y + b * y_bs + (long)c * HW + s0;
  const T* r4 = RES ? res + b * r_bs + (long)c * HW + s0 : nullptr;
  T* o4 = out + b * o_bs + (long)c * HW + s0;
  const long n4 = (s1 - s0) >> 2;
  const int tid = threadIdx.x;
  float s = 0.f, m = -INFINITY;
  if constexpr (V8 && sizeof(T) == 2) {
    const long n8 = (s1 - s0) >> 3;
    for (long i0 = tid; i0 < n8; i0 += 4 * 256) {
      uint4 v[4], r[4];
#pragma unroll
      for (int u = 0; u < 4; ++u) {
        const long i = i0 + u * 256;
        if (i < n8) {
          v[u] = *reinterpret_cast<const uint4*>(y4 + 8 * i);
          if (RES) r[u] = *reinterpret_cast<const uint4*>(r4 + 8 * i);
        }
      }
#pragma unroll
      for (int u = 0; u < 4; ++u) {
        const long i = i0 + u * 256;
        if (i >= n8) continue;
        float f[8], rr[8];
        unpack8(v[u], f);
        if (RES) unpack8(r[u], rr);
#pragma unroll
        for (int j = 0; j < 8; ++j) {
          float o = f[j] + bc;
          if (ACT == 1) o = silu_st<T>(o);
          if (RES) o += rr[j];
          f[j] = o;
        }
        const uint4 ob = pack8(f);
        *reinterpret_cast<uint4*>(o4 + 8 * i) = ob;
        unpack8(ob, f);
        s += ((f[0] + f[1]) + (f[2] + f[3])) + ((f[4] + f[5]) + (f[6] + f[7]));
        if (MAX)
          m = fmaxf(m, fmaxf(fmaxf(fmaxf(f[0], f[1]), fmaxf(f[2], f[3])), fmaxf(fmaxf(f[4], f[5]), fmaxf(f[6], f[7]))));
      }
    }
  } else
  for (long i0 = tid; i0 < n4; i0 += 4 * 256) {
    f32x4 v[4], r[4];
#pragma unroll
    for (int u = 0; u < 4; ++u) {
      const long i = i0 + u * 256;
      if (i < n4) {
        v[u] = ld4(y4 + 4 * i);
        if (RES) r[u] = ld4(r4 + 4 * i);
      }
    }
#pragma unroll
    for (int u = 0; u < 4; ++u) {
      const long i = i0 + u * 256;
      if (i >= n4) continue;
      f32x4 o = v[u] + bc;
      if (ACT == 1) {
        o.x = silu_st<T>(o.x); o.y = silu_st<T>(o.y); o.z = silu_st<T>(o.z); o.w = silu_st<T>(o.w);
      }
      if (RES) o += r[u];
      st4(o4 + 4 * i, o);
      if (sizeof(T) == 2) o = round_bf16(o);
      s += (o.x + o.y) + (o.z + o.w);
      if (MAX) m = fmaxf(m, fmaxf(fmaxf(o.x, o.y), fmaxf(o.z, o.w)));
    }
  }
  __shared__ float ss[4], sm[4];
  s = wave_sum(s);
  if (MAX) m = wave_max(m);
  const int w = tid >> 6;
  if ((tid & 63) == 0) {
    ss[w] = s;
    sm[w] = m;
  }
  __syncthreads();
  if (tid == 0) {
    psum[bx] = (ss[0] + ss[1]) + (ss[2] + ss[3]);
    if (MAX) pmax[bx] = fmaxf(fmaxf(sm[0], sm[1]), fmaxf(sm[2], sm[3]));
  }
}

template <int ACT, bool RES, class T = float>
__global__ __launch_bounds__(256) void bias_act_capool_kernel(const T* __restrict__ y, T* __restrict__ out,
                                                              const float* __restrict__ bias,
                                                              const T* __restrict__ res, int C, int H, int W,
                                                              int RB, long y_bs, long o_bs, long r_bs,
                                                              float* __restrict__ yin) {
  extern __shared__ __attribute__((aligned(16))) float band[];
  const long plane = blockIdx.x;
  const long b = plane / C;
  const int c = (int)(plane - b * C);
  const long HW = (long)H * W;
  const T* yp = y + b * y_bs + (long)c * HW;
  T* op = out + b * o_bs + (long)c * HW;
  const T* rp = RES ? res + b * r_bs + (long)c * HW : nullptr;
  float* o = yin + plane * (long)(H + W);
  const float bc = bias[c];
  const int tid = threadIdx.x;
  const int W4 = W >> 2, NG = 256 / W4;
  const int cq = tid % W4, rg = tid / W4;
  f32x4* band4 = reinterpret_cast<f32x4*>(band);
  f32x4 col = f32x4{0.f, 0.f, 0.f, 0.f};
  const float invW = 1.0f / (float)W;
  for (int h0 = 0; h0 < H; h0 += RB) {
    const int rb = (H - h0 < RB) ? H - h0 : RB;
    const int n4 = rb * W4;
    const long base = (long)h0 * W;
    f32x4 v[8], r[8];
#pragma unroll
    for (int u = 0; u < 8; ++u) {
      const int i = tid + 256 * u < n4 ? tid + 256 * u : n4 - 1;
      v[u] = ld4(yp + base + 4 * i);
      if (RES) r[u] = ld4(rp + base + 4 * i);
    }
#pragma unroll
    for (int u = 0; u < 8; ++u) {
      f32x4 t = v[u] + bc;
      if (ACT == 1) {
        t.x = silu_st<T>(t.x); t.y = silu_st<T>(t.y); t.z = silu_st<T>(t.z); t.w = silu_st<T>(t.w);
      }
      if (RES) t += r[u];
      v[u] = t;
    }
#pragma unroll
    for (int u = 0; u < 8; ++u) {
      const int i = tid + 256 * u;
      if (i < n4) {
        f32x4 t = v[u];
        st4(op + base + 4 * i, t);
        if (sizeof(T) == 2) t = round_bf16(t);
        band4[i] = t;
      }
    }
    __syncthreads();
    for (int rr = tid >> 2; rr < rb; rr += 64) {
      f32x4 s4 = f32x4{0.f, 0.f, 0.f, 0.f};
      for (int q = tid & 3; q < W4; q += 4) s4 += band4[rr * W4 + q];
      const float sm = quad_sum((s4.x + s4.y) + (s4.z + s4.w));
      if ((tid & 3) == 0) o[h0 + rr] = sm * invW;
    }
    if (rg < NG)
      for (int rr = rg; rr < rb; rr += NG) col += band4[rr * W4 + cq];
    __syncthreads();
  }
  float* cpart = band + (long)RB * W;
  if (rg < NG) reinterpret_cast<f32x4*>(cpart)[rg * W4 + cq] = col;
  __syncthreads();
  const float invH = 1.0f / (float)H;
  for (int w = tid; w < W; w += 256) {
    float s = 0.f;
    for (int g = 0; g < NG; ++g) s += cpart[g * W + w];
    o[H + w] = s * invH;
  }
}


template <int M, int K, bool RES, bool DUAL, bool STATS = false, bool UP = false>
__global__ __launch_bounds__(256, 2) void conv1x1_thin_kernel(const float* __restrict__ x, long x_bs,
                                                              const float* __restrict__ w,
                                                              const float* __restrict__ bias, float* __restrict__ out,
                                                              long o_bs, const float* __restrict__ res, long r_bs,
                                                              float* __restrict__ out2, long o2_bs, int c2lo, int HW,
                                                              int ntile, int rev, float* __restrict__ tsum = nullptr,
                                                              float* __restrict__ tmax = nullptr,
                                                              const float* __restrict__ x2 = nullptr, long x2_bs = 0,
                                                              int k1 = K, int up_w = 0) {
  constexpr int RB = M / 64;
  constexpr int KQ = K / 4;
  constexpr int XS = 68;
  __shared__ __attribute__((aligned(16))) float xs[K * XS];
  const int tid = threadIdx.x, lane = tid & 63, wid = tid >> 6;
  const int l15 = lane & 15, g = lane >> 4;
  const int b = rev ? gridDim.y - 1 - blockIdx.y : blockIdx.y;
  const float* xb = x + (long)b * x_bs;
  const float* xb2 = x2 ? x2 + (long)b * x2_bs - (long)k1 * HW : xb;
  float4 a[RB][KQ / 4];
#pragma unroll
  for (int rb = 0; rb < RB; ++rb) {
    const float* wr = w + (long)(wid * (M / 4) + rb * 16 + l15) * K + g * KQ;
#pragma unroll
    for (int t = 0; t < KQ / 4; ++t) a[rb][t] = *reinterpret_cast<const float4*>(wr + 4 * t);
  }
  float bv[RB][4];
#pragma unroll
  for (int rb = 0; rb < RB; ++rb)
#pragma unroll
    for (int r = 0; r < 4; ++r) bv[rb][r] = bias[wid * (M / 4) + rb * 16 + 4 * g + r];
  for (int tile = blockIdx.x; tile < ntile; tile += gridDim.x) {
    const int p0 = tile * 64;
    __syncthreads();
    if (UP) {
      const int pp = p0 + 4 * (tid & 15), yy = pp / up_w, xx = pp - yy * up_w;
      const float* xu = xb + (yy >> 1) * (up_w >> 1) + (xx >> 1);
      const int hw1 = HW >> 2;
#pragma unroll 4
      for (int e = tid; e < k1 * 16; e += 256) {
        const int row = e >> 4, c4 = e & 15;
        const float2 s2 = *reinterpret_cast<const float2*>(xu + (long)row * hw1);
        *reinterpret_cast<float4*>(xs + row * XS + 4 * c4) = make_float4(s2.x, s2.x, s2.y, s2.y);
      }
#pragma unroll 4
      for (int e = k1 * 16 + tid; e < K * 16; e += 256) {
        const int row = e >> 4, c4 = e & 15;
        *reinterpret_cast<float4*>(xs + row * XS + 4 * c4) =
            *reinterpret_cast<const float4*>(xb2 + (long)row * HW + p0 + 4 * c4);
      }
    } else {
#pragma unroll 4
      for (int e = tid; e < K * 16; e += 256) {
        const int row = e >> 4, c4 = e & 15;
        *reinterpret_cast<float4*>(xs + row * XS + 4 * c4) =
            *reinterpret_cast<const float4*>((row < k1 ? xb : xb2) + (long)row * HW + p0 + 4 * c4);
      }
    }
    __syncthreads();
    f32x4 acc[RB][4];
#pragma unroll
    for (int rb = 0; rb < RB; ++rb)
#pragma unroll
      for (int pb = 0; pb < 4; ++pb) acc[rb][pb] = f32x4{0.f, 0.f, 0.f, 0.f};
#pragma unroll
    for (int t4 = 0; t4 < KQ / 4; ++t4)
#pragma unroll
      for (int c = 0; c < 4; ++c) {
        const float* xr = xs + (g * KQ + 4 * t4 + c) * XS + l15;
        float bx[4];
#pragma unroll
        for (int pb = 0; pb < 4; ++pb) bx[pb] = xr[16 * pb];
#pragma unroll
        for (int rb = 0; rb < RB; ++rb) {
          const float av = c == 0 ? a[rb][t4].x : c == 1 ? a[rb][t4].y : c == 2 ? a[rb][t4].z : a[rb][t4].w;
#pragma unroll
          for (int pb = 0; pb < 4; ++pb) acc[rb][pb] = __builtin_amdgcn_mfma_f32_16x16x4f32(av, bx[pb], acc[rb][pb], 0, 0, 0);
        }
      }
#pragma unroll
    for (int rb = 0; rb < RB; ++rb)
#pragma unroll
      for (int r = 0; r < 4; ++r) {
        const int row = wid * (M / 4) + rb * 16 + 4 * g + r;
        float ts = 0.f, tm = -INFINITY;
#pragma unroll
        for (int pb = 0; pb < 4; ++pb) {
          const int p = p0 + pb * 16 + l15;
          float v = siluf_(acc[rb][pb][r] + bv[rb][r]);
          if (RES) v += res[(long)b * r_bs + (long)row * HW + p];
          out[(long)b * o_bs + (long)row * HW + p] = v;
          if (DUAL && row >= c2lo) out2[(long)b * o2_bs + (long)(row - c2lo) * HW + p] = v;
          if (STATS) {
            ts += v;
            tm = fmaxf(tm, v);
          }
        }
        if (STATS) {
#pragma unroll
          for (int o = 1; o < 16; o <<= 1) {
            ts += __shfl_xor(ts, o, 64);
            tm = fmaxf(tm, __shfl_xor(tm, o, 64));
          }
          if (l15 == 0) {
            const long ti = ((long)b * M + row) * ntile + tile;
            tsum[ti] = ts;
            tmax[ti] = tm;
          }
        }
      }
  }
}

__global__ __launch_bounds__(256) void thin_stats_reduce_kernel(const float* __restrict__ tsum,
                                                                const float* __restrict__ tmax, long planes, int ntile,
                                                                int parts, float* __restrict__ psum,
                                                                float* __restrict__ pmax) {
  const long plane = (long)blockIdx.x * 4 + (threadIdx.x >> 6);
  const int lane = threadIdx.x & 63;
  if (plane >= planes) return;
  float s = 0.f, m = -INFINITY;
  for (int t = lane; t < ntile; t += 64) {
    s += tsum[plane * ntile + t];
    if (tmax) m = fmaxf(m, tmax[plane * ntile + t]);
  }
  s = wave_sum(s);
  m = wave_max(m);
  for (int k = lane; k < parts; k += 64) {
    psum[plane * parts + k] = k == 0 ? s : 0.f;
    if (pmax) pmax[plane * parts + k] = k == 0 ? m : -INFINITY;
  }
}

void thin_stats_reduce_launch(const float* tsum, const float* tmax, long planes, int ntile, int parts, float* psum,
                              float* pmax, hipStream_t st) {
  hipLaunchKernelGGL(thin_stats_reduce_kernel, dim3((unsigned)((planes + 3) / 4)), dim3(256), 0, st, tsum, tmax, planes,
                     ntile, parts, psum, pmax);
}

template <class E>
__global__ __launch_bounds__(256) void upsample2x_kernel(const E* __restrict__ x, E* __restrict__ out, long ob, int C,
                                                         int h, int w, long quads) {
  const int wq = w >> 2;
  for (long q = (long)blockIdx.x * 256 + threadIdx.x; q < quads; q += (long)gridDim.x * 256) {
    const long row = q / wq;
    const int j = (int)(q - row * wq) * 4;
    const long plane = row / h;
    const int i = (int)(row - plane * h);
    const int b = (int)(plane / C), c = (int)(plane - (long)b * C);
    E* o = out + (long)b * ob + ((long)c * 2 * h + 2 * i) * (2L * w) + 2 * j;
    if (sizeof(E) == 4) {
      const uint4 v = *reinterpret_cast<const uint4*>(x + row * w + j);
      const uint4 lo = make_uint4(v.x, v.x, v.y, v.y), hi = make_uint4(v.z, v.z, v.w, v.w);
      uint4* o0 = reinterpret_cast<uint4*>(o);
      uint4* o1 = reinterpret_cast<uint4*>(o + 2L * w);
      o0[0] = lo; o0[1] = hi; o1[0] = lo; o1[1] = hi;
    } else {
      const uint2 v = *reinterpret_cast<const uint2*>(x + row * w + j);
      const uint32_t e0 = v.x & 0xffffu, e1 = v.x >> 16, e2 = v.y & 0xffffu, e3 = v.y >> 16;
      const uint4 d = make_uint4(e0 | (e0 << 16), e1 | (e1 << 16), e2 | (e2 << 16), e3 | (e3 << 16));
      *reinterpret_cast<uint4*>(o) = d;
      *reinterpret_cast<uint4*>(o + 2L * w) = d;
    }
  }
}

}

using namespace ys;

YS_EXPORT int yolosod_upsample2x(const void* x, void* out, long out_bstride, int B, int C, int h, int w, int elem_bytes,
                                 void* stream) {
  YS_CHECK_ARG(x && out, "upsample2x: null pointer");
  YS_CHECK_ARG(B >= 0 && C > 0 && h > 0 && w > 0 && (elem_bytes == 4 || elem_bytes == 2), "upsample2x: bad shape");
  YS_CHECK_ARG(w % 4 == 0 && ((uintptr_t)x & 15) == 0 && ((uintptr_t)out & 15) == 0 &&
                   (out_bstride * elem_bytes) % 16 == 0 && (4L * h * w * elem_bytes) % 16 == 0 &&
                   out_bstride >= 4L * C * h * w,
               "upsample2x: w %% 4, 16-byte alignment and a batch stride >= C*4*h*w required");
  if (B == 0) return 0;
  const long quads = (long)B * C * h * (w / 4);
  const unsigned grid = (unsigned)((quads + 255) / 256 < 8192 ? (quads + 255) / 256 : 8192);
  hipStream_t st = (hipStream_t)stream;
  if (elem_bytes == 4)
    hipLaunchKernelGGL(upsample2x_kernel<uint32_t>, dim3(grid), dim3(256), 0, st, (const uint32_t*)x, (uint32_t*)out,
                       out_bstride, C, h, w, quads);
  else
    hipLaunchKernelGGL(upsample2x_kernel<uint16_t>, dim3(grid), dim3(256), 0, st, (const uint16_t*)x, (uint16_t*)out,
                       out_bstride, C, h, w, quads);
  YS_CHECK_LAUNCH("upsample2x");
  return 0;
}

template <class T>
static int bias_act_stats_impl(const T* y, long y_bstride, T* out, long out_bstride, const float* bias, const T* res,
                               long res_bstride, int B, int C, long HW, int act, int parts, long seg, float* psum,
                               float* pmax, void* stream) {
  YS_CHECK_ARG(y && out && bias && psum, "bias_act_stats: null pointer");
  YS_CHECK_ARG(act == 0 || act == 1, "bias_act_stats: act=%d unsupported", act);
  YS_CHECK_ARG(HW % 4 == 0 && seg % 4 == 0 && y_bstride % 4 == 0 && out_bstride % 4 == 0 &&
                   (!res || res_bstride % 4 == 0),
               "bias_act_stats: HW, seg and batch strides must be multiples of 4");
  YS_CHECK_ARG(parts >= 1 && seg >= 1 && (long)parts * seg >= HW && (long)(parts - 1) * seg < HW,
               "bias_act_stats: plane plan (%d x %ld) does not cover HW=%ld", parts, seg, HW);
  YS_CHECK_ARG((((uintptr_t)y | (uintptr_t)out | (uintptr_t)(res ? res : y)) & (4 * sizeof(T) - 1)) == 0,
               "bias_act_stats: pointers must be aligned to 4 elements");
  const long blocks = (long)B * C * parts;
  if (blocks == 0) return 0;
  YS_CHECK_ARG(blocks < (1L << 31), "bias_act_stats: too many planes");
  hipStream_t st = (hipStream_t)stream;
  const bool v8 = sizeof(T) == 2 && HW % 8 == 0 && seg % 8 == 0 && y_bstride % 8 == 0 && out_bstride % 8 == 0 &&
                  (!res || res_bstride % 8 == 0) && (((uintptr_t)y | (uintptr_t)out | (uintptr_t)(res ? res : y)) & 15) == 0;
#define YS_BAS(A_, R_, M_)                                                                                         \
  do {                                                                                                             \
    if (v8)                                                                                                        \
      hipLaunchKernelGGL((bias_act_stats_kernel<A_, R_, M_, T, true>), dim3((unsigned)blocks), dim3(256), 0, st, y, \
                         out, bias, res, C, HW, y_bstride, out_bstride, res_bstride, parts, seg, psum, pmax,       \
                         mall_reverse());                                                                          \
    else                                                                                                           \
      hipLaunchKernelGGL((bias_act_stats_kernel<A_, R_, M_, T>), dim3((unsigned)blocks), dim3(256), 0, st, y, out,  \
                         bias, res, C, HW, y_bstride, out_bstride, res_bstride, parts, seg, psum, pmax,            \
                         mall_reverse());                                                                          \
  } while (0)
  const bool mx = pmax != nullptr;
  if (act == 1) {
    if (res) { if (mx) YS_BAS(1, true, true); else YS_BAS(1, true, false); }
    else { if (mx) YS_BAS(1, false, true); else YS_BAS(1, false, false); }
  } else {
    if (res) { if (mx) YS_BAS(0, true, true); else YS_BAS(0, true, false); }
    else { if (mx) YS_BAS(0, false, true); else YS_BAS(0, false, false); }
  }
#undef YS_BAS
  YS_CHECK_LAUNCH("bias_act_stats");
  return 0;
}

template <class T>
static int bias_act_impl(const T* y, long y_bstride, T* out, long out_bstride, const float* bias, const T* res,
                         long res_bstride, T* out2, long out2_bstride, int c2lo, int B, int C, long HW, int act,
                         void* stream) {
  YS_CHECK_ARG(y && out && bias, "bias_act: null pointer");
  YS_CHECK_ARG(act == 0 || act == 1, "bias_act: act=%d unsupported", act);
  YS_CHECK_ARG(!out2 || (c2lo >= 0 && c2lo < C), "bias_act_dual: c2lo=%d outside [0, C=%d)", c2lo, C);
// ... 237 lines not shown
```

yolo-sod_amd/nn/modules.py:

```python
from __future__ import annotations

import contextlib
import math
import os
from collections.abc import Sequence

import torch
import torch.nn as nn
import torch.nn.functional as F

from .. import _hip

__all__ = (
    "Conv", "DWConv", "Concat", "Bottleneck", "C2f", "SPPF", "DFL", "SE", "SE_Block", "CBAM_Block",
    "ChannelAttention", "SpatialAttention", "CA_Block", "h_sigmoid", "A2_Attn", "WindowAttention", "SwinBlock",
    "Conv1x1BN", "GLUBlock", "MambaBlock", "Detect",
)


def autopad(k, p=None, d=1):
    if d > 1:
        k = d * (k - 1) + 1 if isinstance(k, int) else [d * (x - 1) + 1 for x in k]
    if p is None:
        p = k // 2 if isinstance(k, int) else [x // 2 for x in k]
    return p


def _is_meta(x: torch.Tensor) -> bool:
    return x.device.type == "meta"


def _cached(mod: nn.Module, tag: str, srcs, make):
    key = tuple((id(t), t.data_ptr(), -1 if t.is_inference() else t._version, t.dtype, t.device) for t in srcs)
    cache = mod.__dict__.setdefault("_ys_cache", {})
    ent = cache.get(tag)
    if ent is None or ent[0] != key:
        val = make()
        dev = _cuda_device(val)
        ent = cache[tag] = (key, val, torch.cuda.current_stream(dev) if dev is not None else None)
    elif ent[2] is not None:
        cur = torch.cuda.current_stream(ent[2].device)
        if cur != ent[2]:
            _record_stream(ent[1], cur)
    return ent[1]


def _prep(conv: nn.Module, tag: str, make):
    return lambda: _cached(conv, tag, (conv.weight,), lambda: make(conv.weight))


def _cuda_device(v):
    if isinstance(v, torch.Tensor):
        return v.device if v.is_cuda else None
    if isinstance(v, (tuple, list)):
        for t in v:
            d = _cuda_device(t)
            if d is not None:
                return d
    return None


def _record_stream(v, stream):
    if isinstance(v, torch.Tensor):
        if v.is_cuda:
            v.record_stream(stream)
    elif isinstance(v, (tuple, list)):
        for t in v:
            _record_stream(t, stream)


def _f32(mod: nn.Module, tag: str, *ts):
    if all(t.dtype == torch.float32 and t.is_contiguous() for t in ts):
        return tuple(t.detach() for t in ts)
    return _cached(mod, tag, ts, lambda: tuple(t.detach().float().contiguous() for t in ts))


def _as(mod: nn.Module, tag: str, dtype, *ts):
    if all(t.dtype == dtype and t.is_contiguous() for t in ts):
        return tuple(t.detach() for t in ts)
    return _cached(mod, tag, ts, lambda: tuple(t.detach().to(dtype).contiguous() for t in ts))


def _act_code(act):
    if isinstance(act, nn.SiLU):
        return 1
    if isinstance(act, nn.Identity):
        return 0
    return None


THIN1X1 = os.environ.get("YOLOSOD_THIN1X1", "1") == "1"
CONV3X3 = os.environ.get("YOLOSOD_CONV3X3", "1")
S2_NECK = os.environ.get("YOLOSOD_S2_NECK", "1") != "0"
S1_BACKBONE_DEFAULT, S2_BACKBONE_DEFAULT = "1", "10"
S2_BACKBONE_LAYERS = (7, 10)


def _backbone_switch(value: str, layers=()):
    v = value.strip()
    if v in ("0", "1"):
        return v == "1"
    try:
        picked = frozenset(int(t) for t in v.split(","))
    except ValueError:
        picked = frozenset()
    if not picked or not picked <= frozenset(layers):
        raise ValueError(f"backbone switch {value!r}: expected 0, 1"
                         + (f" or layers out of {tuple(layers)}" if layers else ""))
    return True if picked == frozenset(layers) else picked


S2_BACKBONE = _backbone_switch(os.environ.get("YOLOSOD_S2_BACKBONE", S2_BACKBONE_DEFAULT), S2_BACKBONE_LAYERS)
S1_BACKBONE = _backbone_switch(os.environ.get("YOLOSOD_S1_BACKBONE", S1_BACKBONE_DEFAULT))
S1_NECK = os.environ.get("YOLOSOD_S1_NECK", "1") != "0"
N1_NECK = os.environ.get("YOLOSOD_N1_NECK", "1") != "0"
N1_BACKBONE_DEFAULT = "8,11,13"
N1_BACKBONE_LAYERS = (6, 8, 11, 13)
N1_BACKBONE = _backbone_switch(os.environ.get("YOLOSOD_N1_BACKBONE", N1_BACKBONE_DEFAULT), N1_BACKBONE_LAYERS)
N1_STATS_DEFAULT = "17,22,31"
N1_STATS_LAYERS = (17, 22, 31)
N1_STATS = _backbone_switch(os.environ.get("YOLOSOD_N1_STATS", N1_STATS_DEFAULT), N1_STATS_LAYERS)
C2F_SLICES = os.environ.get("YOLOSOD_C2F_SLICES", "1") != "0"
SPPF_HIP = os.environ.get("YOLOSOD_SPPF_HIP", "1") != "0"
STEM_HIP = os.environ.get("YOLOSOD_STEM_HIP", "1") != "0"


def _onoff_switch(name: str, value: str) -> bool:
    v = value.strip()
    if v not in ("0", "1"):
        raise ValueError(f"{name}={value!r}: expected 0 or 1")
    return v == "1"


BOTTLENECK_FUSE = _onoff_switch("YOLOSOD_BOTTLENECK_FUSE", os.environ.get("YOLOSOD_BOTTLENECK_FUSE", "1"))
HEAD_FUSE_DEFAULT = "1"
HEAD_FUSE = _onoff_switch("YOLOSOD_HEAD_FUSE", os.environ.get("YOLOSOD_HEAD_FUSE", HEAD_FUSE_DEFAULT))


def _s2_on(s2, layer=None):
    if not s2:
        return False
    if s2 != "backbone":
        return S2_NECK
    if layer is None or isinstance(S2_BACKBONE, bool):
        return S2_BACKBONE
    return layer in S2_BACKBONE


def _s1_on(s1) -> bool:
    return bool(s1) and (S1_BACKBONE if s1 == "backbone" else S1_NECK)


def _n1_on(n1, layer=None):
    if not n1:
        return False
    if n1 != "backbone":
        return N1_NECK
    if layer is None or isinstance(N1_BACKBONE, bool):
        return bool(N1_BACKBONE)
    return layer in N1_BACKBONE


def _n1_stats_on(stats_layer) -> bool:
    if stats_layer is None:
        return False
    if isinstance(N1_STATS, bool):
        return N1_STATS
    return stats_layer in N1_STATS


def _n1_run(conv, x, out, out2, c2lo, n1, stats=None):
    prep = _prep(conv, "c1prep", _hip.conv1x1x2_prepare)
    return _hip.conv1x1x2_silu(x, conv.bias, prep, conv.out_channels, out=out, out2=out2, c2lo=c2lo,
                               op="conv1x1x2_backbone" if n1 == "backbone" else "conv1x1x2", stats=stats)


def conv_epilogue(conv: nn.Conv2d, act_code, x, out=None, res=None, stats=None, out2=None, c2lo=0, tower=False,
                  s2=False, s1=False, n1=False, layer=None, stats_layer=None):
    if x.device.type != "cuda" or conv.bias is None or act_code is None or x.dtype not in (torch.float32,
                                                                                           torch.bfloat16):
        return None
    split = _hip.split_convs_enabled()
    if isinstance(x, _hip.CatView):
        if act_code == 1 and res is None and stats is None and conv.kernel_size == (1, 1):
            if split and _n1_on(n1, layer) and _hip.conv1x1x2_ok(x, conv) and (
                    out is None or _hip._imgs_contig(out)) and (out2 is None or _hip._imgs_contig(out2)):
                return _n1_run(conv, x, out, out2, c2lo, n1)
            if (THIN1X1 and conv.out_channels == 64 and conv.stride == (1, 1) and conv.groups == 1
                    and conv.padding == (0, 0) and _hip.conv1x1_thin_ok(x, conv.out_channels)
                    and (out is None or out.data_ptr() % 16 == 0)):
                return _hip.conv1x1_thin(x, conv.weight.detach().reshape(conv.out_channels, -1), conv.bias.detach(),
                                         out=out, out2=out2, c2lo=c2lo)
        x = x.materialize()
    if (split and act_code == 1 and out is None and res is None and stats is None and out2 is None and CONV3X3 != "0"
            and (CONV3X3 == "all" or tower) and _hip.conv3x3_ok(x, conv)):
        prep = _prep(conv, "c3prep", _hip.conv3x3_prepare)
        return _hip.conv3x3_silu(x, conv.bias, prep, conv.out_channels)
    if (split and _n1_on(n1, layer) and act_code == 1 and res is None
            and (stats is None or (n1 is True and out2 is None and stats in ("sum", "summax", "capool")
                                   and _n1_stats_on(stats_layer)))
            and _hip.conv1x1x2_ok(x, conv) and (out is None or _hip._imgs_contig(out))
            and (out2 is None or _hip._imgs_contig(out2))):
        return _n1_run(conv, x, out, out2, c2lo, n1, stats)
    if (split and _s1_on(s1) and act_code == 1 and stats is None and out2 is None and _hip.conv3x3_ok(x, conv)
            and x.shape[3] % 4 == 0 and (res is None or _hip._imgs_contig(res))):
        prep = _prep(conv, "c3prep", _hip.conv3x3_prepare)
        return _hip.conv3x3_silu(x, conv.bias, prep, conv.out_channels, out=out, res=res,
                                 op="conv3x3_backbone" if s1 == "backbone" else "conv3x3")
    if (split and _s2_on(s2, layer) and act_code == 1 and res is None and stats is None and out2 is None
            and _hip.conv3x3s2_ok(x, conv)):
        prep = _prep(conv, "c3s2prep", _hip.conv3x3s2_prepare)
        key = ("conv3x3s2_backbone", tuple(x.shape), (conv.out_channels, False, False)) if s2 == "backbone" else None
        return _hip.conv3x3s2_silu(x, conv.bias, prep, conv.out_channels, key=key, out=out)
    if (THIN1X1 and act_code == 1 and (stats is None or (stats in ("sum", "summax") and res is None and out2 is None))
            and conv.out_channels == 64 and conv.kernel_size == (1, 1) and conv.stride == (1, 1)
            and conv.groups == 1 and conv.padding == (0, 0) and _hip.conv1x1_thin_ok(x, conv.out_channels)
            and (out is None or out.data_ptr() % 16 == 0) and (res is None or res.data_ptr() % 16 == 0)):
        return _hip.conv1x1_thin(x, conv.weight.detach().reshape(conv.out_channels, -1), conv.bias.detach(),
                                 out=out, res=res, out2=out2, c2lo=c2lo, stats=stats)
    y = F.conv2d(x, conv.weight, None, conv.stride, conv.padding, conv.dilation, conv.groups)
    if (y.shape[2] * y.shape[3]) % 4 or y.dtype != x.dtype:
        y = y + conv.bias.view(1, -1, 1, 1)
        y = F.silu(y) if act_code == 1 else y
        if res is not None:
            y = y + res
        if out2 is not None:
            out2.copy_(y[:, c2lo:])
        if out is not None:
            out.copy_(y)
            return out
        return y
    (bias,) = _f32(conv, "bias", conv.bias)
    return _hip.bias_act(y, bias, act_code, out=out, res=res, stats=stats, out2=out2, c2lo=c2lo)


def catview_route(cv, c0, c1, H, W, dtype) -> bool:
    conv = cv.conv
    if (dtype != torch.float32 or not cv.is_fused() or conv.bias is None or _act_code(cv.act) != 1
            or cv.emit_stats is not None or conv.kernel_size != (1, 1) or conv.stride != (1, 1) or conv.groups != 1
            or conv.padding != (0, 0) or conv.in_channels != c0 + c1):
        return False
    if cv.n1 and N1_NECK and _hip.split_convs_enabled() and c0 % 128 == 0 and c1 % 32 == 0 and (H * W) % 4 == 0 and int(
            _hip.load_library().yolosod_conv1x1x2_prep_bytes(c0 + c1, conv.out_channels)) > 0:
        return True
    return (THIN1X1 and conv.out_channels == 64 and c0 + c1 in _hip.THIN1X1_CIN and (H * W) % 64 == 0
            and c0 % 4 == 0 and c1 % 4 == 0)


class Conv(nn.Module):

    default_act = nn.SiLU()
    emit_stats = None
    tower = False
    s2 = False
    s2_backbone = False
    layer = None
    s1 = False
    s1_backbone = False
    n1 = False
    n1_backbone = False
    n1_layer = None
    n1_stats_layer = None
    stem = False

    def __init__(self, c1, c2, k=1, s=1, p=None, g=1, d=1, act=True):
        super().__init__()
        self.conv = nn.Conv2d(c1, c2, k, s, autopad(k, p, d), groups=g, dilation=d, bias=False)
        self.bn = nn.BatchNorm2d(c2)
        self.act = self.default_act if act is True else act if isinstance(act, nn.Module) else nn.Identity()

    def forward(self, x):
        return self.act(self.bn(self.conv(x)))

    def gated_ok(self, x) -> bool:
        return (not hasattr(self, "bn") and self.conv.bias is not None and isinstance(self.act, nn.SiLU)
                and _hip.split_convs_enabled() and _hip.conv3x3s2_ok(x, self.conv))

    def forward_gated(self, x, gate_c, gate_p, key):
        cv = self.conv
        prep = _prep(cv, "c3s2prep", _hip.conv3x3s2_prepare)
        return _hip.conv3x3s2_silu(x, cv.bias, prep, cv.out_channels, gate_c, gate_p, key=key)

    def forward_fuse(self, x, out=None, res=None, out2=None, c2lo=0):
        if (self.stem and STEM_HIP and self.emit_stats == "sum" and out is None and res is None and out2 is None
                and isinstance(self.act, nn.SiLU) and _hip.stem_ok(x, self.conv)):
            return _hip.stem_conv(x, self.conv.weight.detach(), self.conv.bias.detach())
        y = conv_epilogue(self.conv, _act_code(self.act), x, out, res, self.emit_stats, out2, c2lo, self.tower,
                          "backbone" if self.s2_backbone else self.s2, self.s1_mark(),
                          "backbone" if self.n1_backbone else self.n1,
                          self.n1_layer if self.n1_backbone else self.layer, self.n1_stats_layer)
        if y is not None:
            return y
        if isinstance(x, _hip.CatView):
            x = x.materialize()
        y = self.act(self.conv(x))
        if res is not None:
            y = y + res
        if out2 is not None:
            out2.copy_(y[:, c2lo:])
        if out is not None:
            out.copy_(y)
            return out
        return y

    def is_fused(self):
        return not hasattr(self, "bn")

    def s1_mark(self):
        return "backbone" if self.s1_backbone else self.s1


class DWConv(Conv):

    def __init__(self, c1, c2, k=1, s=1, d=1, act=True):
        super().__init__(c1, c2, k, s, g=math.gcd(c1, c2), d=d, act=act)


class Concat(nn.Module):
    def __init__(self, dimension=1):
        super().__init__()
        self.d = dimension

    def forward(self, x):
        return torch.cat(x, self.d)


class Bottleneck(nn.Module):
    def __init__(self, c1, c2, shortcut=True, g=1, k=(3, 3), e=0.5):
        super().__init__()
        c_ = int(c2 * e)
        self.cv1 = Conv(c1, c_, k[0], 1)
        self.cv2 = Conv(c_, c2, k[1], 1, g=g)
        self.add = shortcut and c1 == c2

    def _one_launch(self, x, out, out2) -> bool:
        if not (BOTTLENECK_FUSE and out2 is None and x.device.type == "cuda" and x.dtype == torch.float32
                and _hip.split_convs_enabled() and x.dim() == 4 and x.shape[1] == 32 and x.shape[3] % 4 == 0):
            return False
        for cv in (self.cv1, self.cv2):
            c = cv.conv
            if not (cv.is_fused() and c.bias is not None and _act_code(cv.act) == 1 and cv.emit_stats is None
                    and _s1_on(cv.s1_mark()) and c.in_channels == 32 and c.out_channels == 32
                    and _hip.conv3x3_ok(x, c)):
                return False
        if not _hip._imgs_contig(x) or (out is not None and not _hip._imgs_contig(out)):
            return False
        return _hip.bottleneck3x3_fused(x.shape[0], x.shape[2], x.shape[3])

    def forward(self, x, out=None, out2=None):
        if self._one_launch(x, out, out2):
            c1, c2 = self.cv1.conv, self.cv2.conv
            prep1 = _prep(c1, "c3prep", _hip.conv3x3_prepare)
            prep2 = _prep(c2, "c3prep", _hip.conv3x3_prepare)
            backbone = self.cv2.s1_mark() == "backbone"
            return _hip.bottleneck3x3_silu(x, c1.bias, prep1, c2.bias, prep2, out=out, res=x if self.add else None,
                                           op="bottleneck3x3_backbone" if backbone else "bottleneck3x3")
        if self.cv2.is_fused():
            return self.cv2.forward_fuse(self.cv1(x), out=out, res=x if self.add else None, out2=out2)
        y = x + self.cv2(self.cv1(x)) if self.add else self.cv2(self.cv1(x))
        if out2 is not None:
            out2.copy_(y)
        if out is not None:
            out.copy_(y)
            return out
        return y


class C2f(nn.Module):
    def __init__(self, c1, c2, n=1, shortcut=False, g=1, e=0.5):
        super().__init__()
        self.c = int(c2 * e)
        self.cv1 = Conv(c1, 2 * self.c, 1, 1)
        self.cv2 = Conv((2 + n) * self.c, c2, 1)
        self.m = nn.ModuleList(Bottleneck(self.c, self.c, shortcut, g, k=((3, 3), (3, 3)), e=1.0) for _ in range(n))

    def forward(self, x):
        if isinstance(x, _hip.CatView) and not (x.device.type == "cuda" and self.cv1.is_fused()):
            x = x.materialize()
        if x.device.type == "cuda" and self.cv1.is_fused():
            B, _, H, W = x.shape
            n, c = len(self.m), self.c
            z = torch.empty((B, (2 + n) * c, H, W), dtype=x.dtype, device=x.device)
            if (n and _hip.split_convs_enabled() and x.dtype == torch.float32 and W % 4 == 0
                    and (C2F_SLICES or all(m.cv1.s1_backbone and m.cv2.s1_backbone for m in self.m))
                    and all(_s1_on(m.cv1.s1_mark()) and _s1_on(m.cv2.s1_mark()) and m.cv1.conv.kernel_size == (3, 3)
                            for m in self.m)):
                self.cv1.forward_fuse(x, out=z[:, : 2 * c])
                for i, m in enumerate(self.m):
                    m(z[:, (1 + i) * c:(2 + i) * c], out=z[:, (2 + i) * c:(3 + i) * c])
                return self.cv2(z)
            t = torch.empty((B, c, H, W), dtype=x.dtype, device=x.device) if n else None
            self.cv1.forward_fuse(x, out=z[:, : 2 * c], out2=t, c2lo=c)
            for i, m in enumerate(self.m):
                nxt = torch.empty_like(t) if i + 1 < n else None
                m(t, out=z[:, (2 + i) * c:(3 + i) * c], out2=nxt)
                t = nxt
            return self.cv2(z)
        y = list(self.cv1(x).chunk(2, 1))
        y.extend(m(y[-1]) for m in self.m)
        return self.cv2(torch.cat(y, 1))


class SPPF(nn.Module):
    def __init__(self, c1, c2, k=5):
        super().__init__()
        c_ = c1 // 2
        self.cv1 = Conv(c1, c_, 1, 1)
        self.cv2 = Conv(c_ * 4, c2, 1, 1)
        self.m = nn.MaxPool2d(kernel_size=k, stride=1, padding=k // 2)

    def forward(self, x):
        mp = self.m
        if (SPPF_HIP and x.device.type == "cuda" and x.dtype == torch.float32 and self.cv1.is_fused()
                and mp.kernel_size == 5 and mp.stride in (1, (1, 1)) and mp.padding == 2 and mp.dilation == 1
                and not mp.ceil_mode and x.shape[2] * x.shape[3] <= 4096):
            B, _, H, W = x.shape
            c = self.cv1.conv.out_channels
            z = torch.empty((B, 4 * c, H, W), dtype=x.dtype, device=x.device)
            self.cv1.forward_fuse(x, out=z[:, :c])
            _hip.sppf_pool(z, c)
            return self.cv2(z)
        y = [self.cv1(x)]
        y.extend(self.m(y[-1]) for _ in range(3))
        return self.cv2(torch.cat(y, 1))


class DFL(nn.Module):

    def __init__(self, c1=16):
        super().__init__()
        self.conv = nn.Conv2d(c1, 1, 1, bias=False).requires_grad_(False)
        x = torch.arange(c1, dtype=torch.float)
        self.conv.weight.data[:] = nn.Parameter(x.view(1, c1, 1, 1))
        self.c1 = c1


def fold_conv_bn(conv: nn.Conv2d, bn: nn.BatchNorm2d):
    w_conv = conv.weight.view(conv.out_channels, -1)
    w_bn = torch.diag(bn.weight.div(torch.sqrt(bn.eps + bn.running_var)))
    w = torch.mm(w_bn, w_conv).view(conv.weight.shape)
    b_conv = torch.zeros(conv.weight.shape[0], device=conv.weight.device) if conv.bias is None else conv.bias
    b_bn = bn.bias - bn.weight.mul(bn.running_mean).div(torch.sqrt(bn.running_var + bn.eps))
    b = torch.mm(w_bn, b_conv.reshape(-1, 1)).reshape(-1) + b_bn
    return w, b


def conv_weight_bias(m: Conv):
    if hasattr(m, "bn"):
        w, b = fold_conv_bn(m.conv, m.bn)
    else:
        w, b = m.conv.weight, m.conv.bias
    return w.detach().reshape(w.shape[0], -1).contiguous(), b.detach().contiguous()


class SE(nn.Module):

    def __init__(self, reduction: int = 16) -> None:
        super().__init__()
        self.reduction = reduction
        self.fc1: nn.Conv2d | None = None
        self.fc2: nn.Conv2d | None = None
        self.in_channels: int | None = None

    def _maybe_build(self, c: int, device):
        hidden = max(c // self.reduction, 4)
        if (self.fc1 is None) or (self.in_channels != c):
            self.fc1 = nn.Conv2d(c, hidden, 1, bias=True)
            self.fc2 = nn.Conv2d(hidden, c, 1, bias=True)
            self.in_channels = c
        if device is not None and torch.device(device).type != "meta":
            self.fc1.to(device=device)
            self.fc2.to(device=device)

    def forward(self, x: torch.Tensor) -> torch.Tensor:
        b, c, h, w = x.shape
        if _is_meta(x):
            if self.fc1 is None or self.in_channels != c:
                raise RuntimeError("SE: lazy weights must be materialised before a meta shape probe")
            return torch.empty_like(x)
        self._maybe_build(c, x.device)
        return _hip.se_forward(x, *_f32(self, "fc", self.fc1.weight, self.fc1.bias, self.fc2.weight, self.fc2.bias))

    def gate(self, x: torch.Tensor) -> torch.Tensor:
        self._maybe_build(x.shape[1], x.device)
        return _hip.se_gate(x, *_f32(self, "fc", self.fc1.weight, self.fc1.bias, self.fc2.weight, self.fc2.bias))


SE_Block = SE


class ChannelAttention(nn.Module):

    def __init__(self, in_planes, ratio=16):
        super().__init__()
        self.avg_pool = nn.AdaptiveAvgPool2d(1)
        self.max_pool = nn.AdaptiveMaxPool2d(1)
        self.fc = nn.Sequential(nn.Conv2d(in_planes, in_planes // ratio, 1, bias=False), nn.ReLU(),
                                nn.Conv2d(in_planes // ratio, in_planes, 1, bias=False))
        self.sigmoid = nn.Sigmoid()


class SpatialAttention(nn.Module):

    def __init__(self, kernel_size=7):
        super().__init__()
        self.conv1 = nn.Conv2d(2, 1, kernel_size, padding=kernel_size // 2, bias=False)
        self.sigmoid = nn.Sigmoid()


class CBAM_Block(nn.Module):

    def __init__(self, c1, c2=None, reduction=16):
        super().__init__()
        self.channel_attention = ChannelAttention(c1, reduction)
        self.spatial_attention = SpatialAttention()

    def forward(self, x):
        if _is_meta(x):
            return torch.empty_like(x)
        fc = self.channel_attention.fc
        if self.spatial_attention.conv1.kernel_size != (7, 7):
            raise RuntimeError("CBAM_Block: only the 7x7 spatial kernel is implemented")
        return _hip.cbam_forward(x, *_f32(self, "p", fc[0].weight, fc[2].weight,
                                          self.spatial_attention.conv1.weight))

    def gates(self, x):
        fc = self.channel_attention.fc
        if self.spatial_attention.conv1.kernel_size != (7, 7):
            raise RuntimeError("CBAM_Block: only the 7x7 spatial kernel is implemented")
        return _hip.cbam_gates(x, *_f32(self, "p", fc[0].weight, fc[2].weight, self.spatial_attention.conv1.weight))


class h_sigmoid(nn.Module):
    def __init__(self, inplace=True):
        super().__init__()
        self.relu = nn.ReLU6(inplace=inplace)

    def forward(self, x):
        return self.relu(x + 3) / 6
# ... 385 lines not shown
```

yolo-sod_amd/nn/tasks.py:

```python
from __future__ import annotations

import ast
import contextlib
import copy
import hashlib
import math
import os
import re
from pathlib import Path

import numpy as np
import torch
import torch.nn as nn
import yaml

from .. import _hip
from . import modules as M

CFG_DIR = Path(__file__).resolve().parent.parent / "cfg"

_STREAMS_ENV = os.environ.get("YOLOSOD_STREAMS")
STREAMS = int(_STREAMS_ENV) if _STREAMS_ENV is not None else 1
SIDE_STREAMS = max(1, int(os.environ.get("YOLOSOD_SIDE_STREAMS", "2")))
GATE_FUSE = os.environ.get("YOLOSOD_GATE_FUSE", "1") != "0"
# ... 33 lines not shown
    d.setdefault("scale", guess_model_scale(path))
    d["yaml_file"] = str(path)
    return d


def parse_model(d: dict, ch: int, verbose: bool = False, registry: dict | None = None):
    reg = dict(DEFAULT_REGISTRY)
    if registry:
        reg.update(registry)
    legacy = True
    max_channels = float("inf")
    nc, act, scales = (d.get(x) for x in ("nc", "activation", "scales"))
    depth, width, kpt_shape = (d.get(x, 1.0) for x in ("depth_multiple", "width_multiple", "kpt_shape"))
    if scales:
        scale = d.get("scale")
        if not scale:
            scale = tuple(scales.keys())[0]
        depth, width, max_channels = scales[scale]
    if act:
        raise NotImplementedError("custom 'activation' is not supported on this path")

    ch = [ch]
    layers, save, c2 = [], [], ch[-1]
    for i, (f, n, m, args) in enumerate(d.get("backbone", []) + d.get("neck", []) + d.get("head", [])):
        name = m
        if m.startswith("nn."):
            cls = getattr(torch.nn, m[3:])
        else:
            if m not in reg:
                raise KeyError(f"module '{m}' (layer {i}) is not provided by yolosod_amd")
            cls = reg[m]
        args = list(args)
        for j, a in enumerate(args):
            if isinstance(a, str):
                with contextlib.suppress(ValueError):
                    args[j] = locals()[a] if a in locals() else ast.literal_eval(a)
        n = n_ = max(round(n * depth), 1) if n > 1 else n
        if name in _SCALED_C1C2:
            c1, c2 = ch[f], args[0]
            if c2 != nc:
                c2 = make_divisible(min(c2, max_channels) * width, 8)
            args = [c1, c2, *args[1:]]
            if name in _REPEAT_INSERT:
                args.insert(2, n)
                n = 1
        elif name == "Concat":
            c2 = sum(ch[x] for x in f)
        elif name in _KEEP_CH:
            c2 = ch[f]
            if name in {"SwinBlock", "MambaBlock", "CA_Block", "CBAM_Block"}:
                args = [ch[f], *args]
            elif name == "A2_Attn":
                args = [ch[f], None, *args]
        elif name in _DETECT:
            f_list = f if isinstance(f, (list, tuple)) else [f]
            args.append([ch[x] for x in f_list])
            cls.legacy = legacy
        else:
            c2 = ch[f]

        m_ = nn.Sequential(*(cls(*args) for _ in range(n))) if n > 1 else cls(*args)
        t = name if not name.startswith("nn.") else f"torch.nn.modules.{name[3:]}"
        m_.np = sum(x.numel() for x in m_.parameters())
        m_.i, m_.f, m_.type = i, f, t
        m_.c_in = ch[f] if isinstance(f, int) else [ch[x] for x in f]
        if verbose:
            print(f"{i:>3}{str(f):>20}{n_:>3}{m_.np:10.0f}  {t:<45}{str(args):<30}")
        save.extend(x % i for x in ([f] if isinstance(f, int) else f) if x != -1)
        layers.append(m_)
        if i == 0:
            ch = []
        ch.append(c2)
    return nn.Sequential(*layers), sorted(save)


def initialize_weights(model: nn.Module) -> None:
    for m in model.modules():
        t = type(m)
        if t is nn.BatchNorm2d:
            m.eps = 1e-3
            m.momentum = 0.03
        elif t in {nn.Hardswish, nn.LeakyReLU, nn.ReLU, nn.ReLU6, nn.SiLU}:
            m.inplace = True


def state_dict_sha256(model: nn.Module) -> str:
    h = hashlib.sha256()
    for k, v in model.state_dict().items():
        h.update(k.encode())
        h.update(v.detach().cpu().contiguous().numpy().tobytes())
    return h.hexdigest()


class BaseModel(nn.Module):
    def forward(self, x, *args, **kwargs):
        return self.predict(x, *args, **kwargs)

    def predict(self, x, profile=False, visualize=False, augment=False, embed=None):
        if augment:
            return self._predict_augment(x)
        return self._predict_once(x)

    def _predict_augment(self, x):
        raise NotImplementedError(f"{type(self).__name__} does not support augment=True")

    def _predict_once(self, x):
        if x.device.type == "cuda" and getattr(self, "_fused", False):
            return self._predict_once_planned(x)
        y = []
        for m in self.model:
            if m.f != -1:
                x = y[m.f] if isinstance(m.f, int) else [x if j == -1 else y[j] for j in m.f]
            x = m(x)
            y.append(x if m.i in self.save else None)
        return x

    def _concat_producers(self):
        plan = getattr(self, "_cplan", None)
        if plan is not None:
            return plan
        plan = {}
        for c, m in enumerate(self.model):
            if not isinstance(m, M.Concat) or m.d != 1 or not isinstance(m.f, (list, tuple)) or -1 not in m.f:
                continue
            p = c - 1
            prod = self.model[p]
            if p in self.save or sum(1 for j in m.f if j in (-1, p)) != 1:
                continue
            if (isinstance(prod, M.Conv) and prod.is_fused() and prod.emit_stats is None) or (
                    isinstance(prod, nn.Upsample) and prod.mode == "nearest" and prod.size is None
                    and prod.scale_factor in (2, 2.0, (2, 2), (2.0, 2.0))):
                plan[p] = c
        self._cplan = plan
        return plan

    def _gate_consumers(self):
        plan = getattr(self, "_gplan", None)
        if plan is not None:
            return plan
        plan = {}
        det = self.model[-1]
        busy = set(self._concat_producers()) | (set(det.f) if isinstance(det, M.Detect) and isinstance(
            det.f, (list, tuple)) else set())
        for k in range(len(self.model) - 1):
            m, nxt = self.model[k], self.model[k + 1]
            if (isinstance(m, (M.SE, M.CBAM_Block)) and k not in self.save and k + 1 not in busy
                    and isinstance(nxt, M.Conv)
                    and not isinstance(nxt, M.DWConv) and nxt.f == -1 and nxt.conv.kernel_size == (3, 3)
                    and nxt.conv.stride == (2, 2) and nxt.conv.groups == 1 and nxt.conv.out_channels in (64, 128)):
                plan[k] = nxt
        self._gplan = plan
        return plan

    def _predict_once_planned(self, x):
        plan = self._concat_producers()
        det = self.model[-1]
        towers = lvl = main = side = None
        img_hw = tuple(x.shape[2:])
        streams = STREAMS
        if _STREAMS_ENV is None and x.dtype == torch.bfloat16:
            streams = 2
        if (streams > 0 and isinstance(det, M.Detect) and isinstance(det.f, (list, tuple)) and len(set(det.f)) == len(det.f)
                and det._fused_ok([x])):
            lvl = {j: k for k, j in enumerate(det.f)}
            towers = {}
            ready = []
            last_mafn = max((k for k, mm in enumerate(self.model)
                             if isinstance(mm, (M.SE, M.CBAM_Block, M.CA_Block, M.A2_Attn, M.SwinBlock))), default=-1)
            main = torch.cuda.current_stream(x.device)
            side = getattr(self, "_side_streams", None)
            if side is None or len(side) != SIDE_STREAMS or side[0].device != x.device:
                side = self._side_streams = [torch.cuda.Stream(device=x.device) for _ in range(SIDE_STREAMS)]
            rr = 0
            head_y = None
            lvl_in = {}
            head_hw = [_level_hw(img_hw, float(s)) for s in det.stride]
        y = []
        pend = {}
        cvpend = {}
        elided = 0
        gplan = self._gate_consumers() if GATE_FUSE else {}
        gated = None
        for m in self.model:
            if gated is not None:
                xg, gc, gp, key = gated
                gated = None
                x = m.forward_gated(xg, gc, gp, key)
                y.append(x if m.i in self.save else None)
                continue
            inp = x
            if m.f != -1:
                inp = y[m.f] if isinstance(m.f, int) else [x if j == -1 else y[j] for j in m.f]
            cons = gplan.get(m.i)
            if cons is not None and isinstance(inp, torch.Tensor) and cons.gated_ok(inp):
                if isinstance(m, M.SE):
                    gc, gp = m.gate(inp), None
                    key = ("se_conv", tuple(inp.shape), (cons.conv.out_channels, m.fc1.out_channels))
                else:
                    gc, gp = m.gates(inp)
                    key = ("cbam_conv", tuple(inp.shape),
                           (cons.conv.out_channels, m.channel_attention.fc[0].out_channels))
                gated = (inp, gc, gp, key)
                x = None
                y.append(None)
                continue
            c = plan.get(m.i)
            if c is not None and isinstance(inp, torch.Tensor) and inp.dim() == 4:
                cat = self.model[c]
                B, _, H, W = inp.shape
                if isinstance(m, nn.Upsample):
                    H, W = 2 * H, 2 * W
                    cp = inp.shape[1]
                else:
                    cv = m.conv
                    cp = cv.out_channels
                    H, W = ((n + 2 * p - d * (k - 1) - 1) // s + 1 for n, p, d, k, s in
                            zip((H, W), cv.padding, cv.dilation, cv.kernel_size, cv.stride))
                srcs = [None if j == -1 else y[j] for j in cat.f]
                chans = [cp if s is None else s.shape[1] for s in srcs]
                nxt = self.model[c + 1] if c + 1 < len(self.model) else None
                if (CATVIEW and len(srcs) == 2 and c not in self.save and isinstance(nxt, M.C2f) and nxt.f == -1
                        and all(s is None or (s.shape[0], s.shape[2], s.shape[3]) == (B, H, W) for s in srcs)
                        and M.catview_route(nxt.cv1, chans[0], chans[1], H, W, inp.dtype)):
                    up0 = False
                    if isinstance(m, nn.Upsample):
                        if (UPVIEW and cat.f[0] == -1 and inp.dtype == torch.float32 and inp.is_contiguous()
                                and inp.data_ptr() % 16 == 0 and W % 4 == 0):
                            x, up0 = inp, True
                        else:
                            x = torch.empty((B, cp, H, W), dtype=inp.dtype, device=inp.device)
                            if not (UPSAMPLE_HIP and _hip.upsample2x_into(inp, x)):
                                x = m(inp)
                    else:
                        x = m(inp)
                    cvpend[c] = (up0,)
                    y.append(None)
                    continue
                if all(s is None or (s.shape[0], s.shape[2], s.shape[3]) == (B, H, W) for s in srcs):
                    buf = torch.empty((B, sum(chans), H, W), dtype=inp.dtype, device=inp.device)
                    offs = [sum(chans[:i]) for i in range(len(chans))]
                    k = [j for j in cat.f].index(-1)
                    out = buf[:, offs[k]:offs[k] + cp]
                    if isinstance(m, nn.Upsample):
                        h, w = inp.shape[2], inp.shape[3]
                        if not (UPSAMPLE_HIP and _hip.upsample2x_into(inp, out)):
                            out.view(B, cp, h, 2, w, 2).copy_(inp[:, :, :, None, :, None].expand(B, cp, h, 2, w, 2))
                    else:
                        m.forward_fuse(inp, out=out)
                    pend[c] = (buf, offs, chans)
                    x = out
                    y.append(None)
                    continue
            cvp = cvpend.pop(m.i, None)
            if cvp is not None:
                x = _hip.CatView([x if j == -1 else y[j] for j in m.f], up0=cvp[0])
                elided += 1
            elif m.i in pend:
                buf, offs, chans = pend.pop(m.i)
                elided += 1
                for j, o, n in zip(m.f, offs, chans):
                    if j != -1:
                        buf[:, o:o + n].copy_(y[j])
                x = buf
            elif m is det and towers is not None and len(towers) == det.nl:
                feats = [towers[k] for k in range(det.nl)]
                for sd in side:
                    main.wait_stream(sd)
                if head_y is None:
                    x = det.forward_towers(feats)
                else:
                    ins = [lvl_in[k] for k in range(det.nl)]
                    if [tuple(t.shape[2:]) for t in ins] == head_hw:
                        x = det.forward_levels(head_y, feats, ins)
                    else:
                        x = det.forward_towers([f if f is not None else det.tower_features(k, ins[k])
                                                for k, f in enumerate(feats)])
            else:
                x = m(inp)
            if towers is not None and m is not det:
                if m.i in lvl:
                    ready.append((lvl[m.i], x))
                if ready and (streams != 2 or m.i >= last_mafn):
                    for k, xk in ready:
                        lvl_in[k] = xk
                        if (None not in head_hw and tuple(xk.shape[2:]) == head_hw[k]
                                and det.head_fuse_level(k, xk)):
                            if head_y is None:
                                head_off = [sum(h * w for h, w in head_hw[:j]) for j in range(det.nl + 1)]
                                head_y = torch.empty((xk.shape[0], 4 + det.nc, head_off[-1]), dtype=torch.float32,
                                                     device=xk.device)
                            for mode in (1, 2):
                                sd = side[rr % len(side)]
                                rr += 1
                                sd.wait_stream(main)
                                xk.record_stream(sd)
                                head_y.record_stream(sd)
                                with torch.cuda.stream(sd):
                                    det.tower_into(head_y, k, mode, xk, head_off[k])
                            towers[k] = None
                            continue
                        feats = []
                        for tower in (det.cv2[k], det.cv3[k]):
                            sd = side[rr % len(side)]
                            rr += 1
                            sd.wait_stream(main)
                            xk.record_stream(sd)
                            with torch.cuda.stream(sd):
                                f = tower[:-1](xk).contiguous()
                            f.record_stream(main)
                            feats.append(f)
                        towers[k] = tuple(feats)
                    ready = []
            y.append(x if m.i in self.save else None)
        self._last_elided = elided
        return x

    def is_fused(self, thresh=10):
        bn = tuple(v for k, v in nn.__dict__.items() if "Norm" in k)
        return sum(isinstance(v, bn) for v in self.modules()) < thresh

    def fuse(self, verbose=False):
        if not self.is_fused():
            for m in self.model.modules():
                if isinstance(m, M.Conv) and hasattr(m, "bn"):
                    m.conv = _fuse_conv_and_bn(m.conv, m.bn)
                    delattr(m, "bn")
                    m.forward = m.forward_fuse
        self._fused = True
        self._cplan = None
        return self


def _level_hw(img_hw, stride):
    h, w = img_hw
    n = int(round(math.log2(stride))) if stride >= 1 else -1
    if n < 0 or 2.0 ** n != stride:
        return None
    for _ in range(n):
        h, w = (h + 1) // 2, (w + 1) // 2
    return h, w


def _fuse_conv_and_bn(conv: nn.Conv2d, bn: nn.BatchNorm2d) -> nn.Conv2d:
    fused = nn.Conv2d(conv.in_channels, conv.out_channels, kernel_size=conv.kernel_size, stride=conv.stride,
                      padding=conv.padding, dilation=conv.dilation, groups=conv.groups,
                      bias=True).requires_grad_(False).to(conv.weight.device)
    with torch.no_grad():
        w, b = M.fold_conv_bn(conv, bn)
        fused.weight.copy_(w)
        fused.bias.copy_(b)
    return fused


def probe_manifest_path(yaml_file) -> Path:
    return CFG_DIR / (Path(yaml_file).stem + ".probe.npz")


class DetectionModel(BaseModel):

    def __init__(self, cfg="yolov12-sod-fusion-v5-simple.yaml", ch=3, nc=None, verbose=False, registry=None,
                 probe_stats: bool = True):
        super().__init__()
        self.yaml = cfg if isinstance(cfg, dict) else yaml_model_load(cfg)
        ch = self.yaml["ch"] = self.yaml.get("ch", ch)
        if nc and nc != self.yaml["nc"]:
            self.yaml["nc"] = nc
        self.model, self.save = parse_model(copy.deepcopy(self.yaml), ch=ch, verbose=verbose, registry=registry)
        self.names = {i: f"{i}" for i in range(self.yaml["nc"])}
        self.inplace = self.yaml.get("inplace", True)

        for i, m in enumerate(self.model):
            if i and m.f == -1 and isinstance(m, (M.SE, M.CBAM_Block, M.CA_Block)):
                prod = self.model[i - 1]
                conv = prod if isinstance(prod, M.Conv) else getattr(prod, "cv2", None)
                if isinstance(conv, M.Conv):
                    conv.emit_stats = ("summax" if isinstance(m, M.CBAM_Block) else
                                       "capool" if isinstance(m, M.CA_Block) else "sum")

        m0 = self.model[0]
        if (isinstance(m0, M.Conv) and not isinstance(m0, M.DWConv) and m0.emit_stats == "sum"
                and m0.conv.in_channels == 3 and m0.conv.kernel_size == (3, 3) and m0.conv.stride == (2, 2)
                and m0.conv.groups == 1):
            m0.stem = True

        n_backbone = len(self.yaml.get("backbone", []))
        for i, m in enumerate(self.model):
            if (isinstance(m, M.Conv) and not isinstance(m, M.DWConv)
                    and m.conv.kernel_size == (3, 3) and m.conv.stride == (2, 2) and m.conv.groups == 1):
                if i >= n_backbone:
                    m.s2 = True
                elif i and m.f == -1 and not isinstance(self.model[i - 1], (M.SE, M.CBAM_Block)):
                    m.s2_backbone = True
                    m.layer = i
            if isinstance(m, M.C2f):
                for bt in m.m:
                    for cv in (bt.cv1, bt.cv2):
                        if cv.conv.kernel_size == (3, 3) and cv.conv.stride == (1, 1) and cv.conv.groups == 1:
                            if i >= n_backbone:
                                cv.s1 = True
                            else:
                                cv.s1_backbone = True
            if i >= n_backbone:
                for cv in ([m] if isinstance(m, M.Conv) and not isinstance(m, M.DWConv) else
                           [m.cv1, m.cv2] if isinstance(m, M.C2f) else []):
                    if cv.conv.kernel_size == (1, 1) and cv.conv.groups == 1 and cv.conv.out_channels % 128 == 0:
                        cv.n1 = True
                        if cv.emit_stats is not None:
                            cv.n1_stats_layer = i
            elif isinstance(m, (M.C2f, M.SPPF)):
                for cv in (m.cv1, m.cv2):
                    if cv.conv.kernel_size == (1, 1) and cv.conv.groups == 1 and cv.conv.out_channels % 128 == 0:
                        cv.n1_backbone = True
                        cv.n1_layer = i

        for m in self.model:
            if isinstance(m, M.SE):
                m._maybe_build(m.c_in, None)

        det = self.model[-1]
        if not isinstance(det, M.Detect):
            raise NotImplementedError("only Detect-headed models are supported")
        det.stride = self._probe_strides(ch)
        self.stride = det.stride
        det.bias_init()
        initialize_weights(self)
        if probe_stats:
            self._load_probe_stats()

    def tta_plan(self, shape, scales=None, flips=None):
# ... 75 lines not shown
```

yolo-sod_amd/perf.py:

```python
from __future__ import annotations

import os

F32 = 4

PEAK_HBM_GBS = 8000.0
PEAK_FP32_MFMA_TFLOPS = 157.3
PEAK_BF16_MFMA_TFLOPS = 2516.6


def elem_size(key) -> int:
    return key[3] if len(key) > 3 else F32


def peak_tflops(key) -> float:
    return PEAK_BF16_MFMA_TFLOPS if elem_size(key) == 2 else PEAK_FP32_MFMA_TFLOPS


def _on(name: str) -> bool:
    return os.environ.get(name, "1") != "0"


def method_peak_tflops(key) -> float:
    if elem_size(key) == 4:
        op = key[0]
        split = ((op == "swin" and key[1][1] in (64, 256) and _on("YOLOSOD_SWIN_X3"))
                 or (op == "a2" and _on("YOLOSOD_A2_X2")) or (op == "head" and _on("YOLOSOD_HEAD_X2"))
                 or op in FUSED_CONV)
        if split:
            return PEAK_BF16_MFMA_TFLOPS / 3
    return peak_tflops(key)


FUSED_CONV = {"se_conv": "se", "cbam_conv": "cbam"}
GATE_ONLY = {"se_gate": "se_conv", "cbam_gate": "cbam_conv"}
PATH_OPS = frozenset({"se", "cbam", "ca", "a2", "swin", "mamba", "decode", "head", "nms", *FUSED_CONV})


def swin_geom(H, W, ws=7):
    if H <= ws and W <= ws:
        return H, W, H, W
    wh, ww = min(ws, H), min(ws, W)
    return wh, ww, H + (wh - H % wh) % wh, W + (ww - W % ww) % ww


def op_cost(key):
    b, f = _op_cost(key[:3], elem_size(key))
    return b, f


def _op_cost(key, E):
    op, shape, extra = key
    if op in FUSED_CONV:
        B, C, H, W = shape
        cout, hid = extra
        Ho, Wo = (H + 1) // 2, (W + 1) // 2
        act = B * C * H * W * E + B * cout * Ho * Wo * E + (B * H * W * F32 if op == "cbam_conv" else 0)
        w = (cout * C * 9 + cout + 2 * C * hid + C + hid + (98 if op == "cbam_conv" else 0)) * F32
        flops = 2 * B * Ho * Wo * cout * C * 9 + B * C * H * W * (1 if op == "se_conv" else 2)
        return act + w, flops
    if op in ("se", "cbam", "ca"):
        B, C, H, W = shape
        hid = extra
        act = 2 * B * C * H * W * E
        w = (2 * C * hid + C + hid) * F32
        flops = B * C * H * W * (2 if op == "se" else 6)
        return act + w, flops
    if op == "a2":
        B, C, H, W = shape
        A, heads = extra
        L = A * W
        act = 2 * B * C * H * W * E
        w = (2 * (C * C + C) + 4 * C * C + 4 * C + 2 * C) * F32
        conv = 2 * 2 * C * C * H * W
        mha = 2 * L * C * 3 * C + 2 * L * C * C + 2 * 2 * L * L * C
        return act + w, B * (conv + mha)
    if op == "swin":
        B, C, H, W = shape
        heads, ws, hid = extra
        wh, ww, Hp, Wp = swin_geom(H, W, ws)
        L = wh * ww
        tok_p = Hp * Wp
        act = 2 * B * C * H * W * E
        w = (9 * C + 4 * C * C + 3 * C + C + 2 * C * hid + hid + C + C * C + 6 * C) * F32
        dense = tok_p * (2 * C * 3 * C + 2 * C * C + 2 * 2 * C * hid) + H * W * 2 * C * C
        attn = tok_p * 2 * 2 * L * C
        dw = H * W * 2 * 9 * C
        return act + w, B * (dense + attn + dw)
    if op == "mamba":
        B, C, H, W = shape
        ch, r = extra
        hd = 2 * ch
        hw, hwh = H * W, (H // r) * (W // r)
        act = 2 * B * C * hw * E
        w = (ch * C + 2 * hd * ch + 9 * hd + ch * hd + C * ch + 4 * (ch + hd + C)) * F32
        flops = 2 * ch * C * hw + hwh * (2 * 2 * hd * ch + 2 * 9 * hd + 2 * ch * hd + 2 * C * ch)
        return act + w, B * flops
    if op == "decode":
        B, A = shape
        nc = extra
        return B * A * ((64 + nc) + (4 + nc)) * F32, B * A * (64 * 4 + nc * 4)
    if op == "head":
        B, A = shape
        nc, c2, c3 = extra
        return (B * A * ((c2 + c3) * E + (4 + nc) * F32) + (64 * c2 + nc * c3 + 64 + nc) * F32,
                B * A * (2 * (64 * c2 + nc * c3) + 64 * 4 + nc * 4))
    if op == "nms":
        B, nc, A = shape
        return B * A * (4 + nc) * F32, 0
    raise KeyError(op)


def bound_of(key, method: bool = True) -> str:
    nbytes, flops = op_cost(key)
    peak = method_peak_tflops(key) if method else peak_tflops(key)
    return "mfma" if flops / (peak * 1e12) > nbytes / (PEAK_HBM_GBS * 1e9) else "hbm"


def t_min_ms(key, method: bool = False) -> float:
    nbytes, flops = op_cost(key)
    peak = method_peak_tflops(key) if method else peak_tflops(key)
    return max(nbytes / (PEAK_HBM_GBS * 1e9), flops / (peak * 1e12)) * 1e3



PRODUCER_GATE = {"sum": "se", "summax": "cbam", "capool": "ca"}


def _numel(shape) -> int:
    n = 1
    for d in shape:
        n *= d
    return n


def producer_of(key):
    op, shape, extra = key[:3]
    tail, E = tuple(key[3:]), elem_size(key)
    if op == "bias_act" and isinstance(extra, str) and extra.split("+")[0] in PRODUCER_GATE:
        st, res = extra.split("+")[0], extra.endswith("+res")
        plain = ("bias_act", tuple(shape), "res" if res else None) + tail
        return PRODUCER_GATE[st], tuple(shape), plain, _numel(shape) * E * (3 if res else 2)
    if op == "conv1x1_thin" and isinstance(extra, tuple) and len(extra) == 2 and extra[1] in ("sum", "summax"):
        B, cin, H, W = shape
        cout = extra[0]
        plain = ("conv1x1_thin", tuple(shape), (cout, False, False)) + tail
        return PRODUCER_GATE[extra[1]], (B, cout, H, W), plain, B * H * W * (cin + cout) * E
    if op == "conv1x1x2_stats" and isinstance(extra, tuple) and len(extra) == 2 and extra[1] in PRODUCER_GATE:
        B, cin, H, W = shape
        cout = extra[0]
        plain = ("conv1x1x2", tuple(shape), (cout, False)) + tail
        return PRODUCER_GATE[extra[1]], (B, cout, H, W), plain, B * H * W * (cin + cout) * E
    if op == "stem" and isinstance(extra, tuple) and len(extra) == 2 and extra[1] in PRODUCER_GATE:
        B, cin, H, W = shape
        cout = extra[0]
        plain = ("stem", tuple(shape), (cout, None)) + tail
        nbytes = B * (cin * H * W + cout * (H // 2) * (W // 2)) * E
        return PRODUCER_GATE[extra[1]], (B, cout, H // 2, W // 2), plain, nbytes
    return None


class PathSelect:

    def __init__(self):
        self.plain = set()

    def __call__(self, key):
        if key[0] in PATH_OPS or key[0] in GATE_ONLY:
            return True
        p = producer_of(key)
        if p is not None:
            self.plain.add(p[2])
            return True
        return key in self.plain


def aggregate(calls):
    agg = {}
    for key, ms in calls:
        a = agg.setdefault(key, [0.0, 0])
        a[0] += ms
        a[1] += 1
    return agg


def producer_billing(agg):
    out = {}
    for key, (tot, n) in agg.items():
        p = producer_of(key)
        if p is None:
            continue
        gate, gshape, plain, pbytes = p
        t_st = tot / n
        if plain in agg:
            t_pl = agg[plain][0] / agg[plain][1]
            basis = f"its in-model plain variant, {agg[plain][1]} launches"
        else:
            t_pl = pbytes / (PEAK_HBM_GBS * 1e9) * 1e3
            basis = "plain pass at the HBM roof (no plain variant of this shape in the model)"
        out[(gate, gshape)] = (max(0.0, t_st - t_pl),
                               f"{key[0]}{tuple(key[1])} {key[2]}: {t_st:.4f} ms in-model vs {t_pl:.4f} ms ({basis})")
    return out


def summarize(calls, steps):
    agg = aggregate(calls)
    billed = producer_billing(agg)
    gate_ms = {}
    for key, (tot, n) in agg.items():
        if key[0] in GATE_ONLY:
            k2 = (GATE_ONLY[key[0]], tuple(key[1]))
            gate_ms[k2] = gate_ms.get(k2, 0.0) + tot
    ops, backbone = [], []
    for key, (tot, n) in agg.items():
        if key[0] in GATE_ONLY:
            continue
        if key[0] not in PATH_OPS:
            backbone.append({"op": key[0], "shape": list(key[1]), "extra": str(key[2]), "launches": n,
                             "total_ms_per_step": round(tot / steps, 4)})
            continue
        nbytes, flops = op_cost(key)
        kern = tot / n + gate_ms.get((key[0], tuple(key[1])), 0.0) / n
        ext, src = billed.get((FUSED_CONV.get(key[0], key[0]), tuple(key[1])), (0.0, None))
        avg = kern + ext
        bound = bound_of(key)
        tm, tm_d = t_min_ms(key, method=True), t_min_ms(key)
        o = {"op": key[0], "shape": list(key[1]), "dtype": "bf16" if elem_size(key) == 2 else "f32",
             "launches": n, "avg_ms": round(avg, 4), "kernels_ms": round(kern, 4),
             "total_ms_per_step": round(avg * n / steps, 4),
             "GBps": round(nbytes / (avg * 1e-3) / 1e9, 1), "TFLOPs": round(flops / (avg * 1e-3) / 1e12, 2),
             "bound": bound, "peak": method_peak_tflops(key) if bound == "mfma" else PEAK_HBM_GBS,
             "t_min_ms": round(tm, 4), "frac": round(tm / avg, 3), "frac_vs_dtype_peak": round(tm_d / avg, 3),
             "bytes": nbytes, "flops": flops, "key": key}
        if src:
            o["producer_extra_ms"] = round(ext, 4)
            o["producer"] = src
        ops.append(o)
    ops.sort(key=lambda o: -o["total_ms_per_step"])
    t_meas = sum(o["total_ms_per_step"] for o in ops)
    t_min = sum(t_min_ms(o["key"], method=True) * o["launches"] / steps for o in ops)
    t_min_d = sum(t_min_ms(o["key"]) * o["launches"] / steps for o in ops)
    path = {"t_min_ms": round(t_min, 4), "t_meas_ms": round(t_meas, 4),
            "frac": round(t_min / t_meas, 4) if t_meas else None,
            "definition": "sum over hot-path ops of max(bytes / 8 TB/s, flops / matrix ceiling of the method the op "
                          "computes with: fp16 peak / 3 = 838.9 TF/s for the fp32 ops on fp16 two-term splits, 2516.6 "
                          "for bf16, 157.3 for exact fp32 MFMA) / measured; a producing epilogue's extra time for a "
                          "gate's statistics (in-model producer minus its in-model plain variant of the same shape) is "
                          "billed to the gate",
            "frac_vs_dtype_peak": round(t_min_d / t_meas, 4) if t_meas else None}
    path["mafn"] = mafn_path(ops, steps)
    return ops, sorted(backbone, key=lambda o: -o["total_ms_per_step"]), path



def _split_fused(key):
    op, shape, extra = key[:3]
    B, C, H, W = shape
    cout, hid = extra
    E = elem_size(key)
    Ho, Wo = (H + 1) // 2, (W + 1) // 2
    conv_b = (B * C * H * W + B * cout * Ho * Wo) * E + (cout * C * 9 + cout) * F32
    conv_f = 2 * B * Ho * Wo * cout * C * 9
    t_conv = max(conv_b / (PEAK_HBM_GBS * 1e9), conv_f / (PEAK_BF16_MFMA_TFLOPS / 3 * 1e12)) * 1e3
    return (FUSED_CONV[op], tuple(shape), hid) + tuple(key[3:]), t_conv


def mafn_path(ops, steps):
    t_min = t_meas = 0.0
    nbytes = 0
    parts = []
    for o in ops:
        key, n = o["key"], o["launches"]
        if key[0] in FUSED_CONV:
            k8, t_conv = _split_fused(key)
            meas = max(o["avg_ms"] - t_conv, 0.0)
        elif key[0] == "head":
            B, A = key[1]
            nc = key[2][0]
            k8, meas = ("decode", (B, A), nc) + tuple(key[3:]), o["avg_ms"]
        else:
            k8, meas = key, o["avg_ms"]
        b, _ = op_cost(k8)
        tm = t_min_ms(k8, method=True)
        nbytes += b * n / steps
        t_min += tm * n / steps
        t_meas += meas * n / steps
        parts.append(f"{k8[0]}{tuple(k8[1])}: {meas:.4f} ms")
    floor = nbytes / (PEAK_HBM_GBS * 1e9) * 1e3
    return {"bytes_per_step": int(nbytes), "t_hbm_floor_ms": round(floor, 4), "t_min_ms": round(t_min, 4),
            "t_meas_ms": round(t_meas, 4), "frac": round(t_min / t_meas, 4) if t_meas else None,
            "frac_vs_hbm_floor": round(floor / t_meas, 4) if t_meas else None,
            "definition": "SURVEY 8(d): MAFN instances + decode + NMS scan; gate-fused SE/CBAM billed without their "
                          "consumer conv (its t_min subtracted, its FLOPs excluded)", "instances": parts}



CSV_FIELDS = ("config", "steps", "seq", "op", "shape", "extra", "esize", "ms")


def calls_to_rows(config, steps, calls):
    return [{"config": config, "steps": steps, "seq": i, "op": k[0], "shape": "x".join(map(str, k[1])),
             "extra": repr(k[2]), "esize": k[3] if len(k) > 3 else "", "ms": f"{ms:.6f}"}
            for i, (k, ms) in enumerate(calls)]


def rows_to_calls(rows):
    import ast
    out = []
    for r in rows:
        key = (r["op"], tuple(int(d) for d in r["shape"].split("x")), ast.literal_eval(r["extra"]))
        if r["esize"] != "":
            key = key + (int(r["esize"]),)
        out.append((key, float(r["ms"])))
    return out
```

Baseline: 4573.

## Fuse C2f cv1 1x1 conv into the stride-2 3x3 conv epilogue

Adds a templated tail to the persistent stride-2 3x3 conv kernel. It applies the following C2f block's 64->64 1x1 conv plus SiLU on the output tile held in shared memory, using fp32 MFMA, and writes straight into the C2f concat buffer. A model-level plan detects Conv(32->64, s2) followed by C2f and routes both through the fused path. This removes one full activation write and read plus a kernel launch. In exchange the kernel uses more registers and LDS, adds extra syncs, and some paths recompute indices.

```diff
diff --git a/include/yolosod_hip.h b/include/yolosod_hip.h
--- a/include/yolosod_hip.h
+++ b/include/yolosod_hip.h
@@ -205,6 +205,11 @@
 int yolosod_conv3x3s2_silu_out(const float* x, float* y, long y_bstride, int B, int cin, int cout, int H, int W,
                                const float* bias, const float* gc, const float* gp, const void* prep,
                                size_t prep_bytes, void* stream);
+int yolosod_conv3x3s2_cv1_out(const float* x, float* y, long y_bstride, int B, int cin, int cout, int H, int W,
+                              const float* bias, const float* gc, const float* gp, const void* prep,
+                              size_t prep_bytes, const float* w1x1, const float* b1x1, int cout1x1, void* stream);
+int yolosod_debug_s2_cv1_fused(int B, int H, int W);
+int yolosod_debug_set_s2_cv1_fuse(int mode);
 size_t yolosod_conv1x1x2_prep_bytes(int cin, int cout);
 int yolosod_conv1x1x2_prepare(const float* w, int cin, int cout, void* prep, size_t prep_bytes, void* stream);
 int yolosod_conv1x1x2_silu(const float* x, long x_bstride, float* y, long y_bstride, float* y2, long y2_bstride,
diff --git a/yolo-sod_amd/_hip.py b/yolo-sod_amd/_hip.py
--- a/yolo-sod_amd/_hip.py
+++ b/yolo-sod_amd/_hip.py
@@ -123,6 +123,9 @@
     "yolosod_conv3x3s2_prepare": (_i, [_vp, _i, _i, _vp, _sz, _vp]),
     "yolosod_conv3x3s2_silu": (_i, [_vp, _vp, _i, _i, _i, _i, _i, _vp, _vp, _vp, _vp, _sz, _vp]),
     "yolosod_conv3x3s2_silu_out": (_i, [_vp, _vp, _l, _i, _i, _i, _i, _i, _vp, _vp, _vp, _vp, _sz, _vp]),
+    "yolosod_conv3x3s2_cv1_out": (_i, [_vp, _vp, _l, _i, _i, _i, _i, _i, _vp, _vp, _vp, _vp, _sz, _vp, _vp, _i, _vp]),
+    "yolosod_debug_set_s2_cv1_fuse": (_i, [_i]),
+    "yolosod_debug_s2_cv1_fused": (_i, [_i, _i, _i]),
     "yolosod_debug_set_swin_tokln": (_i, [_i]),
     "yolosod_debug_set_a2_pool_px": (_i, [_i]),
     "yolosod_mamba_glu_workspace": (_sz, [_i, _i, _i, _i, _i, _i]),
@@ -1066,10 +1069,19 @@
     return _split_prepare("conv3x3s2", lib.yolosod_conv3x3s2_prep_bytes, lib.yolosod_conv3x3s2_prepare, w)
 
 
-def conv3x3s2_silu(x, bias, prep, cout, gate_c=None, gate_p=None, key=None, out=None):
+def s2_cv1_fused(B, H, W) -> bool:
+    return bool(load_library().yolosod_debug_s2_cv1_fused(int(B), int(H), int(W)))
+
+
+def conv3x3s2_silu(x, bias, prep, cout, gate_c=None, gate_p=None, key=None, out=None, cv1=None):
     lib = load_library()
     B, Cin, H, W = x.shape
     Ho, Wo = (H + 1) // 2, (W + 1) // 2
+    if cv1 is not None:
+        w1, b1 = (t.detach().float().contiguous() for t in cv1)
+        if (Cin, cout) != (32, 64) or tuple(w1.shape) != (64, 64) or tuple(b1.shape) != (64,):
+            raise RuntimeError(f"conv3x3s2 + cv1: {Cin} -> {cout} -> {tuple(w1.shape)} unsupported "
+                               "(32 -> 64 -> 64 only)")
     if out is None:
         y = torch.empty((B, cout, Ho, Wo), dtype=torch.float32, device=x.device)
     else:
@@ -1088,13 +1100,18 @@
 
     def run():
         blk = prep()
-        return lib.yolosod_conv3x3s2_silu_out(_dev(x, "x"), y.data_ptr(), y.stride(0), B, Cin, cout, H, W,
-                                              _dev(b, "bias"), None if gc is None else _dev(gc, "gate_c"),
-                                              None if gp is None else _dev(gp, "gate_p"), blk.data_ptr(), blk.numel(),
-                                              _stream(x.device))
+        args = (_dev(x, "x"), y.data_ptr(), y.stride(0), B, Cin, cout, H, W, _dev(b, "bias"),
+                None if gc is None else _dev(gc, "gate_c"), None if gp is None else _dev(gp, "gate_p"),
+                blk.data_ptr(), blk.numel())
+        if cv1 is not None:
+            return lib.yolosod_conv3x3s2_cv1_out(*args, _dev(w1, "cv1 weight"), _dev(b1, "cv1 bias"), 64,
+                                                 _stream(x.device))
+        return lib.yolosod_conv3x3s2_silu_out(*args, _stream(x.device))
 
     if key is None:
         key = ("conv3x3s2", tuple(x.shape), (cout, gc is not None, gp is not None))
+    if cv1 is not None:
+        key = (key[0], key[1], tuple(key[2]) + ("cv1",)) + tuple(key[3:])
     _check(_launch(key, x.device, run), "conv3x3s2")
     return y
 
diff --git a/yolo-sod_amd/csrc/conv1x1_thin_math.h b/yolo-sod_amd/csrc/conv1x1_thin_math.h
--- /dev/null
+++ b/yolo-sod_amd/csrc/conv1x1_thin_math.h
@@ -0,0 +1,35 @@
+#pragma once
+#include "common.h"
+
+namespace ys {
+namespace thinm {
+
+template <int K>
+__device__ __forceinline__ void load_a(const float* __restrict__ w, int row0, int g, int l15, float4 (&a)[K / 16]) {
+  const float* wr = w + (long)(row0 + l15) * K + g * (K / 4);
+#pragma unroll
+  for (int t = 0; t < K / 16; ++t) a[t] = *reinterpret_cast<const float4*>(wr + 4 * t);
+}
+
+__device__ __forceinline__ void load_bias(const float* __restrict__ bias, int row0, int g, float (&bv)[4]) {
+#pragma unroll
+  for (int r = 0; r < 4; ++r) bv[r] = bias[row0 + 4 * g + r];
+}
+
+template <int N>
+__device__ __forceinline__ float a_of(const float4 (&a)[N], int t4, int c) {
+  return c == 0 ? a[t4].x : c == 1 ? a[t4].y : c == 2 ? a[t4].z : a[t4].w;
+}
+
+template <int RB, int PB>
+__device__ __forceinline__ void step(f32x4 (&acc)[RB][PB], const float (&av)[RB], const float (&bx)[PB]) {
+#pragma unroll
+  for (int rb = 0; rb < RB; ++rb)
+#pragma unroll
+    for (int pb = 0; pb < PB; ++pb) acc[rb][pb] = __builtin_amdgcn_mfma_f32_16x16x4f32(av[rb], bx[pb], acc[rb][pb], 0, 0, 0);
+}
+
+__device__ __forceinline__ float out_of(float acc, float bias) { return siluf_(acc + bias); }
+
+}
+}
diff --git a/yolo-sod_amd/csrc/conv3x3s2.hip b/yolo-sod_amd/csrc/conv3x3s2.hip
--- a/yolo-sod_amd/csrc/conv3x3s2.hip
+++ b/yolo-sod_amd/csrc/conv3x3s2.hip
@@ -1,4 +1,5 @@
 #include "split_conv.h"
+#include "conv1x1_thin_math.h"
 
 namespace ys {
 namespace c3s2 {
@@ -21,15 +22,31 @@
   unsigned* range_flag;
   const unsigned* prep_flag;
 };
+struct ArgsCv1 : Args {
+  const float* w1;
+  const float* b1;
+};
+template <class A>
+struct HasTail {
+  static constexpr bool value = false;
+};
+template <>
+struct HasTail<ArgsCv1> {
+  static constexpr bool value = true;
+};
 
 constexpr int ES = TW + 4;
-template <int GATE, int THk, int NTk>
-__global__ __launch_bounds__(NTk, 512 / NTk) void conv3x3s2_rw_kernel(Args p) {
+constexpr int ep_off(int rc, int epad) { return rc * ES + (rc >> 4) * epad; }
+template <int GATE, int THk, int NTk, class A = Args>
+__global__ __launch_bounds__(NTk, 512 / NTk) void conv3x3s2_rw_kernel(A p) {
+  constexpr bool TAIL = HasTail<A>::value;
   constexpr int HRk = 2 * THk + 1, NPXk = HRk * HC, PLk = NPXk * PS, NQUADk = NPXk * 8;
   constexpr int NITk = (NQUADk + NTk - 1) / NTk, NGPk = (NPXk + NTk - 1) / NTk;
+  constexpr int EPAD = TAIL ? 16 : 0;
   static_assert(NITk <= 32, "okb bits");
+  static_assert(!TAIL || (THk == 2 && NTk == 256), "the cv1 tail: four waves on a 64-pixel tile");
   __shared__ __attribute__((aligned(16))) h16_t Pl[2 * PLk];
-  __shared__ __attribute__((aligned(16))) float Ep[THk * 64 * ES];
+  __shared__ __attribute__((aligned(16))) float Ep[THk * 4 * (16 * ES + EPAD)];
   __shared__ __attribute__((aligned(16))) float gcs[32];
   __shared__ float gps[(GATE & 2) ? NPXk : 1];
   const int tid = threadIdx.x, lane = tid & 63, wid = __builtin_amdgcn_readfirstlane(tid >> 6);
@@ -61,15 +78,32 @@
     for (int pl = 0; pl < 2; ++pl)
       wr[t][pl] = __builtin_bit_cast(
           f16x8_t, __builtin_amdgcn_raw_buffer_load_b128(rw, (unsigned)(lane * 16), ((t * 4 + cb) * 2 + pl) * 1024, 0));
-  int pk[NITk], el0[NITk];
-#pragma unroll
-  for (int i = 0; i < NITk; ++i) {
-    const int e = min(tid + NTk * i, NQUADk - 1);
+  constexpr bool LEAN = TAIL && (GATE & 2) != 0;
+  int pk[LEAN ? 1 : NITk], el0[LEAN ? 1 : NITk];
+  auto pk_of = [&](int t, int i) __attribute__((always_inline)) {
+    const int e = min(t + NTk * i, NQUADk - 1);
     const int quad = e / NPXk, px = e - quad * NPXk;
     const int hy = px / HC, hx = px - hy * HC;
-    pk[i] = (quad << 16) | (hy << 8) | hx;
-    el0[i] = 4 * quad * HWi + hy * W + hx;
+    return (quad << 16) | (hy << 8) | hx;
+  };
+  auto el_of = [&](int k) __attribute__((always_inline)) {
+    return 4 * (k >> 16) * HWi + ((k >> 8) & 255) * W + (k & 255);
+  };
+  if constexpr (!LEAN) {
+#pragma unroll
+    for (int i = 0; i < NITk; ++i) {
+      const int e = min(tid + NTk * i, NQUADk - 1);
+      const int quad = e / NPXk, px = e - quad * NPXk;
+      const int hy = px / HC, hx = px - hy * HC;
+      pk[i] = (quad << 16) | (hy << 8) | hx;
+      el0[i] = 4 * quad * HWi + hy * W + hx;
+    }
   }
+  auto tid_now = [&]() __attribute__((always_inline)) {
+    int t = tid;
+    if constexpr (LEAN) asm volatile("" : "+v"(t));
+    return t;
+  };
   struct Tile {
     int b, ty, tx;
   };
@@ -90,17 +124,20 @@
     const int toff = iy0 * W + ix0;
     const bool interior = iy0 >= 0 && ix0 >= 0 && iy0 + HRk <= H && ix0 + HC <= W;
     unsigned okb = 0xffffffffu;
+    const int tn = tid_now();
     if (!interior) {
       okb = 0;
 #pragma unroll
       for (int i = 0; i < NITk; ++i) {
-        const int hy = (pk[i] >> 8) & 255, hx = pk[i] & 255;
+        const int pki = LEAN ? pk_of(tn, i) : pk[LEAN ? 0 : i];
+        const int hy = (pki >> 8) & 255, hx = pki & 255;
         okb |= ((unsigned)(iy0 + hy) < (unsigned)H && (unsigned)(ix0 + hx) < (unsigned)W) ? (1u << i) : 0u;
       }
     }
 #pragma unroll
     for (int i = 0; i < NITk; ++i) {
-      const unsigned vo = (unsigned)((el0[i] + toff) * 4);
+      const int el = LEAN ? el_of(pk_of(tn, i)) : el0[LEAN ? 0 : i];
+      const unsigned vo = (unsigned)((el + toff) * 4);
 #pragma unroll
       for (int c = 0; c < 4; ++c)
         sv[i][c] = __builtin_bit_cast(float, __builtin_amdgcn_raw_buffer_load_b32(ri, vo + c * HWi * 4, 0, 0));
@@ -121,13 +158,21 @@
   for (int k = 0; k < 4; ++k) bpx[k] = 2 * (2 * rp + (k >> 1)) * HC + 2 * ((k & 1) * 16 + l15);
   const int nw = __builtin_amdgcn_readfirstlane(p.Wo);
   const float bo = p.bias[16 * cb + l15];
+  float4 a1[TAIL ? 4 : 1];
+  float bv1[4];
+  if constexpr (TAIL) {
+    thinm::load_a<64>(p.w1, 16 * wid, g, l15, a1);
+    thinm::load_bias(p.b1, 16 * wid, g, bv1);
+  }
   auto store_tile = [&](const Tile& tl) __attribute__((always_inline)) {
 #pragma unroll
     for (int m = 0; m < THk * 512 / NTk; ++m) {
       const int idx = tid + NTk * m;
       const int r = idx >> 9, ch = (idx >> 3) & 63, px4 = idx & 7;
       const int ox = tl.tx * TW + 4 * px4, oy = tl.ty * THk + r;
-      const f32x4 v = *reinterpret_cast<const f32x4*>(Ep + (r * 64 + ch) * ES + 4 * px4);
+      const float* src = TAIL ? Ep + ep_off(tid >> 3, EPAD) + 4 * px4 + m * ep_off(NTk >> 3, EPAD)
+                              : Ep + (r * 64 + ch) * ES + 4 * px4;
+      const f32x4 v = *reinterpret_cast<const f32x4*>(src);
       if (oy < p.Ho && ox < nw)
         __builtin_nontemporal_store(v, reinterpret_cast<f32x4*>(p.y + (long)tl.b * p.ybs + ((long)ch * p.Ho + oy) * nw + ox));
     }
@@ -148,11 +193,12 @@
       }
       __syncthreads();
     }
+    const int ts = tid_now();
 #pragma unroll
     for (int i = 0; i < NITk; ++i) {
       const int e = tid + NTk * i;
       if (e < NQUADk) {
-        const int quad = pk[i] >> 16, px = e - quad * NPXk;
+        const int quad = (LEAN ? pk_of(ts, i) : pk[LEAN ? 0 : i]) >> 16, px = e - quad * NPXk;
         f32x4 v = sv[i];
         if constexpr ((GATE & 1) != 0) v = v * *reinterpret_cast<const f32x4*>(gcs + 4 * quad);
         if constexpr ((GATE & 2) != 0) v = v * gps[px];
@@ -192,7 +238,31 @@
       f32x4 v;
 #pragma unroll
       for (int e = 0; e < 4; ++e) v[e] = silu_fast_(acc[k][e] * (1.0f / WSC) + bo);
-      *reinterpret_cast<f32x4*>(Ep + ((2 * rp + (k >> 1)) * 64 + 16 * cb + l15) * ES + 16 * (k & 1) + 4 * g) = v;
+      *reinterpret_cast<f32x4*>(Ep + ep_off((2 * rp + (k >> 1)) * 64 + 16 * cb + l15, EPAD) + 16 * (k & 1) + 4 * g) = v;
+    }
+    if constexpr (TAIL) {
+      __syncthreads();
+      f32x4 t1[1][4];
+#pragma unroll
+      for (int pb = 0; pb < 4; ++pb) t1[0][pb] = f32x4{0.f, 0.f, 0.f, 0.f};
+#pragma unroll
+      for (int t4 = 0; t4 < 4; ++t4)
+#pragma unroll
+        for (int c = 0; c < 4; ++c) {
+          float bx[4];
+#pragma unroll
+          for (int pb = 0; pb < 4; ++pb)
+            bx[pb] = Ep[ep_off((pb >> 1) * 64 + 16 * g + 4 * t4 + c, EPAD) + 16 * (pb & 1) + l15];
+          const float av[1] = {thinm::a_of(a1, t4, c)};
+          thinm::step(t1, av, bx);
+        }
+      __syncthreads();
+#pragma unroll
+      for (int pb = 0; pb < 4; ++pb)
+#pragma unroll
+        for (int r = 0; r < 4; ++r)
+          Ep[ep_off((pb >> 1) * 64 + 16 * wid + 4 * g + r, EPAD) + 16 * (pb & 1) + l15] =
+              thinm::out_of(t1[0][pb][r], bv1[r]);
     }
   }
   __syncthreads();
@@ -512,9 +582,9 @@
   return split_prepare<9>("conv3x3s2_prepare", w, cin, cin, cout, prep, prep_bytes, stream);
 }
 
-YS_EXPORT int yolosod_conv3x3s2_silu_out(const float* x, float* y, long y_bstride, int B, int cin, int cout, int H,
-                                         int W, const float* bias, const float* gc, const float* gp, const void* prep,
-                                         size_t prep_bytes, void* stream) {
+static int conv3x3s2_run(const float* x, float* y, long y_bstride, int B, int cin, int cout, int H, int W,
+                         const float* bias, const float* gc, const float* gp, const void* prep, size_t prep_bytes,
+                         const float* w1, const float* b1, void* stream) {
   YS_CHECK_ARG(x && y && bias && prep, "conv3x3s2: null pointer");
   YS_CHECK_ARG(B >= 0 && H > 0 && W > 0 && yolosod_conv3x3s2_prep_bytes(cin, cout) > 0, "conv3x3s2: bad shape");
   const int Ho = (H + 1) / 2, Wo = (W + 1) / 2;
@@ -543,7 +613,13 @@
     a.ntiles = (int)nt2;
     static const KP kp[4] = {c3s2::conv3x3s2_rw_kernel<0, 2, 256>, c3s2::conv3x3s2_rw_kernel<1, 2, 256>,
                              c3s2::conv3x3s2_rw_kernel<2, 2, 256>, c3s2::conv3x3s2_rw_kernel<3, 2, 256>};
-    hipLaunchKernelGGL(kp[gate], dim3((unsigned)persistent_grid(2L * cu_count(), nt2)), dim3(256), 0, st, a);
+    using KP1 = void (*)(c3s2::ArgsCv1);
+    static const KP1 kp1[4] = {
+        c3s2::conv3x3s2_rw_kernel<0, 2, 256, c3s2::ArgsCv1>, c3s2::conv3x3s2_rw_kernel<1, 2, 256, c3s2::ArgsCv1>,
+        c3s2::conv3x3s2_rw_kernel<2, 2, 256, c3s2::ArgsCv1>, c3s2::conv3x3s2_rw_kernel<3, 2, 256, c3s2::ArgsCv1>};
+    const dim3 grid((unsigned)persistent_grid(2L * cu_count(), nt2));
+    if (w1) hipLaunchKernelGGL(kp1[gate], grid, dim3(256), 0, st, c3s2::ArgsCv1{a, w1, b1});
+    else hipLaunchKernelGGL(kp[gate], grid, dim3(256), 0, st, a);
   } else {
     const int form = s2_form(B, cout, Ho, Wo);
     const int geo = (form & 3) - 1;
@@ -570,6 +646,37 @@
   return 0;
 }
 
+YS_EXPORT int yolosod_conv3x3s2_silu_out(const float* x, float* y, long y_bstride, int B, int cin, int cout, int H,
+                                         int W, const float* bias, const float* gc, const float* gp, const void* prep,
+                                         size_t prep_bytes, void* stream) {
+  return conv3x3s2_run(x, y, y_bstride, B, cin, cout, H, W, bias, gc, gp, prep, prep_bytes, nullptr, nullptr, stream);
+}
+
+static const long S2_CV1_MIN_BYTES = 8L * 32 * 160 * 160 * 4;
+static int g_s2_cv1_fuse = -1;
+YS_EXPORT int yolosod_debug_set_s2_cv1_fuse(int mode) {
+  const int old = g_s2_cv1_fuse;
+  if (mode >= -1 && mode <= 1) g_s2_cv1_fuse = mode;
+  return old;
+}
+
+YS_EXPORT int yolosod_debug_s2_cv1_fused(int B, int H, int W) {
+  const int Ho = (H + 1) / 2, Wo = (W + 1) / 2;
+  if (B <= 0 || H <= 0 || W <= 0 || Wo % 4 || g_s2_cv1_fuse == 0) return 0;
+  return g_s2_cv1_fuse == 1 || (long)B * 32 * Ho * Wo * 4 >= S2_CV1_MIN_BYTES;
+}
+
+YS_EXPORT int yolosod_conv3x3s2_cv1_out(const float* x, float* y, long y_bstride, int B, int cin, int cout, int H,
+                                        int W, const float* bias, const float* gc, const float* gp, const void* prep,
+                                        size_t prep_bytes, const float* w1x1, const float* b1x1, int cout1x1,
+                                        void* stream) {
+  YS_CHECK_ARG(w1x1 && b1x1, "conv3x3s2_cv1: null pointer");
+  YS_CHECK_ARG(cin == 32 && cout == 64 && cout1x1 == 64,
+               "conv3x3s2_cv1: (cin=%d, cout=%d, 1x1 cout=%d) unsupported: 32 -> 64 -> 64 only", cin, cout, cout1x1);
+  YS_CHECK_ARG(((uintptr_t)w1x1 & 15) == 0, "conv3x3s2_cv1: 1x1 weights must be 16-byte aligned");
+  return conv3x3s2_run(x, y, y_bstride, B, cin, cout, H, W, bias, gc, gp, prep, prep_bytes, w1x1, b1x1, stream);
+}
+
 YS_EXPORT int yolosod_conv3x3s2_silu(const float* x, float* y, int B, int cin, int cout, int H, int W,
                                      const float* bias, const float* gc, const float* gp, const void* prep,
                                      size_t prep_bytes, void* stream) {
diff --git a/yolo-sod_amd/csrc/conv_epilogue.hip b/yolo-sod_amd/csrc/conv_epilogue.hip
--- a/yolo-sod_amd/csrc/conv_epilogue.hip
+++ b/yolo-sod_amd/csrc/conv_epilogue.hip
@@ -1,4 +1,5 @@
 #include "common.h"
+#include "conv1x1_thin_math.h"
 #include <math.h>
 
 namespace ys {
@@ -247,17 +248,12 @@
   const float* xb = x + (long)b * x_bs;
   const float* xb2 = x2 ? x2 + (long)b * x2_bs - (long)k1 * HW : xb;
   float4 a[RB][KQ / 4];
+  float bv[RB][4];
 #pragma unroll
   for (int rb = 0; rb < RB; ++rb) {
-    const float* wr = w + (long)(wid * (M / 4) + rb * 16 + l15) * K + g * KQ;
-#pragma unroll
-    for (int t = 0; t < KQ / 4; ++t) a[rb][t] = *reinterpret_cast<const float4*>(wr + 4 * t);
-  }
-  float bv[RB][4];
-#pragma unroll
-  for (int rb = 0; rb < RB; ++rb)
-#pragma unroll
-    for (int r = 0; r < 4; ++r) bv[rb][r] = bias[wid * (M / 4) + rb * 16 + 4 * g + r];
+    thinm::load_a<K>(w, wid * (M / 4) + rb * 16, g, l15, a[rb]);
+    thinm::load_bias(bias, wid * (M / 4) + rb * 16, g, bv[rb]);
+  }
   for (int tile = blockIdx.x; tile < ntile; tile += gridDim.x) {
     const int p0 = tile * 64;
     __syncthreads();
@@ -299,12 +295,10 @@
         float bx[4];
 #pragma unroll
         for (int pb = 0; pb < 4; ++pb) bx[pb] = xr[16 * pb];
-#pragma unroll
-        for (int rb = 0; rb < RB; ++rb) {
-          const float av = c == 0 ? a[rb][t4].x : c == 1 ? a[rb][t4].y : c == 2 ? a[rb][t4].z : a[rb][t4].w;
-#pragma unroll
-          for (int pb = 0; pb < 4; ++pb) acc[rb][pb] = __builtin_amdgcn_mfma_f32_16x16x4f32(av, bx[pb], acc[rb][pb], 0, 0, 0);
-        }
+        float av[RB];
+#pragma unroll
+        for (int rb = 0; rb < RB; ++rb) av[rb] = thinm::a_of(a[rb], t4, c);
+        thinm::step(acc, av, bx);
       }
 #pragma unroll
     for (int rb = 0; rb < RB; ++rb)
@@ -315,7 +309,7 @@
 #pragma unroll
         for (int pb = 0; pb < 4; ++pb) {
           const int p = p0 + pb * 16 + l15;
-          float v = siluf_(acc[rb][pb][r] + bv[rb][r]);
+          float v = thinm::out_of(acc[rb][pb][r], bv[rb][r]);
           if (RES) v += res[(long)b * r_bs + (long)row * HW + p];
           out[(long)b * o_bs + (long)row * HW + p] = v;
           if (DUAL && row >= c2lo) out2[(long)b * o2_bs + (long)(row - c2lo) * HW + p] = v;
diff --git a/yolo-sod_amd/nn/modules.py b/yolo-sod_amd/nn/modules.py
--- a/yolo-sod_amd/nn/modules.py
+++ b/yolo-sod_amd/nn/modules.py
@@ -135,6 +135,21 @@
 BOTTLENECK_FUSE = _onoff_switch("YOLOSOD_BOTTLENECK_FUSE", os.environ.get("YOLOSOD_BOTTLENECK_FUSE", "1"))
 HEAD_FUSE_DEFAULT = "1"
 HEAD_FUSE = _onoff_switch("YOLOSOD_HEAD_FUSE", os.environ.get("YOLOSOD_HEAD_FUSE", HEAD_FUSE_DEFAULT))
+THIN_FUSE_PARTS = ("cv1",)
+THIN_FUSE_DEFAULT = "1"
+
+
+def _parts_switch(name: str, value: str, parts) -> frozenset:
+    v = value.strip()
+    if v in ("0", "1"):
+        return frozenset(parts) if v == "1" else frozenset()
+    picked = frozenset(t.strip() for t in v.split(","))
+    if not picked or not picked <= frozenset(parts):
+        raise ValueError(f"{name}={value!r}: expected 0, 1 or parts out of {tuple(parts)}")
+    return picked
+
+
+THIN_FUSE = _parts_switch("YOLOSOD_THIN_FUSE", os.environ.get("YOLOSOD_THIN_FUSE", THIN_FUSE_DEFAULT), THIN_FUSE_PARTS)
 
 
 def _s2_on(s2, layer=None):
@@ -276,10 +291,33 @@
         return (not hasattr(self, "bn") and self.conv.bias is not None and isinstance(self.act, nn.SiLU)
                 and _hip.split_convs_enabled() and _hip.conv3x3s2_ok(x, self.conv))
 
-    def forward_gated(self, x, gate_c, gate_p, key):
+    def forward_gated(self, x, gate_c, gate_p, key, out=None, cv1=None):
         cv = self.conv
         prep = _prep(cv, "c3s2prep", _hip.conv3x3s2_prepare)
-        return _hip.conv3x3s2_silu(x, cv.bias, prep, cv.out_channels, gate_c, gate_p, key=key)
+        if cv1 is not None:
+            c1 = cv1.conv
+            cv1 = (c1.weight.detach().reshape(c1.out_channels, -1), c1.bias.detach())
+        return _hip.conv3x3s2_silu(x, cv.bias, prep, cv.out_channels, gate_c, gate_p, key=key, out=out, cv1=cv1)
+
+    def s2_cv1_ok(self, x, c2f, gated: bool) -> bool:
+        cv, c1 = self.conv, c2f.cv1
+        if not ("cv1" in THIN_FUSE and THIN1X1 and x.dim() == 4 and x.dtype == torch.float32
+                and cv.in_channels == 32 and cv.out_channels == 64 and self.emit_stats is None):
+            return False
+        if not (gated or (self.is_fused() and cv.bias is not None and isinstance(self.act, nn.SiLU)
+                          and _hip.split_convs_enabled()
+                          and _s2_on("backbone" if self.s2_backbone else self.s2, self.layer)
+                          and _hip.conv3x3s2_ok(x, cv))):
+            return False
+        k = c1.conv
+        if not (c1.is_fused() and k.bias is not None and _act_code(c1.act) == 1 and c1.emit_stats is None
+                and k.kernel_size == (1, 1) and k.stride == (1, 1) and k.padding == (0, 0) and k.groups == 1
+                and k.in_channels == 64 and k.out_channels == 64 and 2 * c2f.c == 64 and k.weight.dtype == torch.float32
+                and not c1.n1 and not c1.n1_backbone):
+            return False
+        B, _, H, W = x.shape
+        Ho, Wo = (H + 1) // 2, (W + 1) // 2
+        return ((Ho * Wo) % 64 == 0 and c2f.slices_ok(torch.float32, Wo) and _hip.s2_cv1_fused(B, H, W))
 
     def forward_fuse(self, x, out=None, res=None, out2=None, c2lo=0):
         if (self.stem and STEM_HIP and self.emit_stats == "sum" and out is None and res is None and out2 is None
@@ -374,17 +412,28 @@
         self.cv2 = Conv((2 + n) * self.c, c2, 1)
         self.m = nn.ModuleList(Bottleneck(self.c, self.c, shortcut, g, k=((3, 3), (3, 3)), e=1.0) for _ in range(n))
 
-    def forward(self, x):
+    def slices_ok(self, dtype, W) -> bool:
+        return bool(len(self.m) and _hip.split_convs_enabled() and dtype == torch.float32 and W % 4 == 0
+                    and (C2F_SLICES or all(m.cv1.s1_backbone and m.cv2.s1_backbone for m in self.m))
+                    and all(_s1_on(m.cv1.s1_mark()) and _s1_on(m.cv2.s1_mark()) and m.cv1.conv.kernel_size == (3, 3)
+                            for m in self.m))
+
+    def empty_z(self, B, H, W, dtype, device):
+        return torch.empty((B, (2 + len(self.m)) * self.c, H, W), dtype=dtype, device=device)
+
+    def forward(self, x, z=None):
+        if z is not None:
+            n, c = len(self.m), self.c
+            for i, m in enumerate(self.m):
+                m(z[:, (1 + i) * c:(2 + i) * c], out=z[:, (2 + i) * c:(3 + i) * c])
+            return self.cv2(z)
         if isinstance(x, _hip.CatView) and not (x.device.type == "cuda" and self.cv1.is_fused()):
             x = x.materialize()
         if x.device.type == "cuda" and self.cv1.is_fused():
             B, _, H, W = x.shape
             n, c = len(self.m), self.c
-            z = torch.empty((B, (2 + n) * c, H, W), dtype=x.dtype, device=x.device)
-            if (n and _hip.split_convs_enabled() and x.dtype == torch.float32 and W % 4 == 0
-                    and (C2F_SLICES or all(m.cv1.s1_backbone and m.cv2.s1_backbone for m in self.m))
-                    and all(_s1_on(m.cv1.s1_mark()) and _s1_on(m.cv2.s1_mark()) and m.cv1.conv.kernel_size == (3, 3)
-                            for m in self.m)):
+            z = self.empty_z(B, H, W, x.dtype, x.device)
+            if self.slices_ok(x.dtype, W):
                 self.cv1.forward_fuse(x, out=z[:, : 2 * c])
                 for i, m in enumerate(self.m):
                     m(z[:, (1 + i) * c:(2 + i) * c], out=z[:, (2 + i) * c:(3 + i) * c])
diff --git a/yolo-sod_amd/nn/tasks.py b/yolo-sod_amd/nn/tasks.py
--- a/yolo-sod_amd/nn/tasks.py
+++ b/yolo-sod_amd/nn/tasks.py
@@ -209,6 +209,24 @@
         self._gplan = plan
         return plan
 
+    def _s2_cv1_plan(self):
+        plan = getattr(self, "_s2cv1plan", None)
+        if plan is not None:
+            return plan
+        plan = {}
+        det = self.model[-1]
+        busy = set(self._concat_producers()) | (set(det.f) if isinstance(det, M.Detect) and isinstance(
+            det.f, (list, tuple)) else set())
+        for k in range(len(self.model) - 1):
+            m, nxt = self.model[k], self.model[k + 1]
+            if (isinstance(m, M.Conv) and not isinstance(m, M.DWConv) and k not in self.save and k not in busy
+                    and m.conv.kernel_size == (3, 3) and m.conv.stride == (2, 2) and m.conv.groups == 1
+                    and (m.conv.in_channels, m.conv.out_channels) == (32, 64)
+                    and isinstance(nxt, M.C2f) and nxt.f == -1 and 2 * nxt.c == 64):
+                plan[k] = nxt
+        self._s2cv1plan = plan
+        return plan
+
     def _predict_once_planned(self, x):
         plan = self._concat_producers()
         det = self.model[-1]
@@ -238,10 +256,23 @@
         elided = 0
         gplan = self._gate_consumers() if GATE_FUSE else {}
         gated = None
+        s2plan = self._s2_cv1_plan() if M.THIN_FUSE else {}
+        zfill = None
+
+        def s2_cv1(conv, c2f, xin, gc, gp, key):
+            z = c2f.empty_z(xin.shape[0], (xin.shape[2] + 1) // 2, (xin.shape[3] + 1) // 2, xin.dtype, xin.device)
+            conv.forward_gated(xin, gc, gp, key, out=z[:, :2 * c2f.c], cv1=c2f.cv1)
+            return z
+
         for m in self.model:
             if gated is not None:
                 xg, gc, gp, key = gated
                 gated = None
+                c2f = s2plan.get(m.i)
+                if c2f is not None and m.s2_cv1_ok(xg, c2f, True):
+                    zfill, x = s2_cv1(m, c2f, xg, gc, gp, key), None
+                    y.append(None)
+                    continue
                 x = m.forward_gated(xg, gc, gp, key)
                 y.append(x if m.i in self.save else None)
                 continue
@@ -332,6 +363,14 @@
                     else:
                         x = det.forward_towers([f if f is not None else det.tower_features(k, ins[k])
                                                 for k, f in enumerate(feats)])
+            elif zfill is not None:
+                x, zfill = m(None, z=zfill), None
+            elif (m.i in s2plan and isinstance(inp, torch.Tensor) and inp.device.type == "cuda"
+                  and m.s2_cv1_ok(inp, s2plan[m.i], False)):
+                key = ("conv3x3s2_backbone", tuple(inp.shape), (64, False, False)) if m.s2_backbone else None
+                zfill, x = s2_cv1(m, s2plan[m.i], inp, None, None, key), None
+                y.append(None)
+                continue
             else:
                 x = m(inp)
             if towers is not None and m is not det:
diff --git a/yolo-sod_amd/perf.py b/yolo-sod_amd/perf.py
--- a/yolo-sod_amd/perf.py
+++ b/yolo-sod_amd/perf.py
@@ -37,6 +37,11 @@
 PATH_OPS = frozenset({"se", "cbam", "ca", "a2", "swin", "mamba", "decode", "head", "nms", *FUSED_CONV})
 
 
+def fused_cv1(key) -> bool:
+    extra = key[2]
+    return key[0] in FUSED_CONV and isinstance(extra, tuple) and len(extra) > 2 and extra[-1] == "cv1"
+
+
 def swin_geom(H, W, ws=7):
     if H <= ws and W <= ws:
         return H, W, H, W
@@ -53,11 +58,14 @@
     op, shape, extra = key
     if op in FUSED_CONV:
         B, C, H, W = shape
-        cout, hid = extra
+        cout, hid = extra[:2]
         Ho, Wo = (H + 1) // 2, (W + 1) // 2
         act = B * C * H * W * E + B * cout * Ho * Wo * E + (B * H * W * F32 if op == "cbam_conv" else 0)
         w = (cout * C * 9 + cout + 2 * C * hid + C + hid + (98 if op == "cbam_conv" else 0)) * F32
         flops = 2 * B * Ho * Wo * cout * C * 9 + B * C * H * W * (1 if op == "se_conv" else 2)
+        if fused_cv1(key):
+            w += (cout * cout + cout) * F32
+            flops += 2 * B * Ho * Wo * cout * cout
         return act + w, flops
     if op in ("se", "cbam", "ca"):
         B, C, H, W = shape
@@ -256,12 +264,16 @@
 def _split_fused(key):
     op, shape, extra = key[:3]
     B, C, H, W = shape
-    cout, hid = extra
+    cout, hid = extra[:2]
     E = elem_size(key)
     Ho, Wo = (H + 1) // 2, (W + 1) // 2
     conv_b = (B * C * H * W + B * cout * Ho * Wo) * E + (cout * C * 9 + cout) * F32
     conv_f = 2 * B * Ho * Wo * cout * C * 9
-    t_conv = max(conv_b / (PEAK_HBM_GBS * 1e9), conv_f / (PEAK_BF16_MFMA_TFLOPS / 3 * 1e12)) * 1e3
+    t_mfma = conv_f / (PEAK_BF16_MFMA_TFLOPS / 3 * 1e12)
+    if fused_cv1(key):
+        conv_b += (cout * cout + cout) * F32
+        t_mfma += 2 * B * Ho * Wo * cout * cout / (PEAK_FP32_MFMA_TFLOPS * 1e12)
+    t_conv = max(conv_b / (PEAK_HBM_GBS * 1e9), t_mfma) * 1e3
     return (FUSED_CONV[op], tuple(shape), hid) + tuple(key[3:]), t_conv
 
 
```

Result: no change. 4606, median of 3 (+0.7%).
